# mdangschat/ctc-asr

Measured on AMD Instinct MI355X. Metric: audio-seconds/s training throughput (DS2, 10 s utterances), higher is better.
Workload: dtype f32 tensors / accumulate / own kernels; projection GEMMs: fp16x3 split (22 significand bits) where the layer input is bounded or, behind a ReLU cell, scaled per row / per column on the device - forward projections and their gradient GEMMs - bf16x6 split (24 bits) elsewhere; forward and backward recu

## Files before the change

ctc_asr_amd/csrc/conv16.hip:

```cpp
#include "common.h"

namespace {

constexpr int C16_CIN = 32, C16_KT = 11, C16_KF = 21;
constexpr int C16_CELL = 144;

typedef unsigned int u32x4 __attribute__((ext_vector_type(4)));
typedef unsigned int u32x2 __attribute__((ext_vector_type(2)));
typedef _Float16 f16x8 __attribute__((ext_vector_type(8)));
union Frag16 {
    u32x4 u;
    f16x8 h;
};

__device__ __forceinline__ unsigned f16_pieces(float s) {
    const _Float16 h1 = (_Float16)s;
    const _Float16 h2 = (_Float16)(s - (float)h1);
    return (unsigned)__builtin_bit_cast(unsigned short, h1) |
           ((unsigned)__builtin_bit_cast(unsigned short, h2) << 16);
}

__device__ __forceinline__ float scale_below_f16_max(unsigned max_bits) {
    const int e = (int)((max_bits >> 23) & 0xFF) - 127;
    const int se = max_bits == 0u ? 0 : min(max(14 - e, -60), 60);
// ... 547 lines not shown
    if (tile < tiles) fetch(tile);
    while (tile < tiles) {
        __syncthreads();
        stage();
        __syncthreads();
        const int next = next_valid(tile + nsplit);
        if (next < tiles) fetch(next);
#pragma unroll 1
        for (int q = 0; q < G::KS; ++q) {
            const int slot = 4 * q + g;
            Frag16 a1[2], a2[2];
#pragma unroll
            for (int c = 0; c < 2; ++c) {
                a1[c].u = dzs[(slot * 2 + 0) * 32 + c * 16 + n];
                a2[c].u = dzs[(slot * 2 + 1) * 32 + c * 16 + n];
            }
            const u32x4 *xb = xs + ((2 * slot + kf0) * 2) * 32 + ci_tile * 16 + n;
#pragma unroll
            for (int k = 0; k < TAPS; ++k) {
                if (k < TAPS - 1 || !half) {
                    Frag16 b1, b2;
                    b1.u = xb[k * 64];
                    b2.u = xb[k * 64 + 32];
#pragma unroll
                    for (int c = 0; c < 2; ++c) {
                        acc[k][c] = __builtin_amdgcn_mfma_f32_16x16x32_f16(a1[c].h, b1.h, acc[k][c], 0, 0, 0);
                        acc[k][c] = __builtin_amdgcn_mfma_f32_16x16x32_f16(a1[c].h, b2.h, acc[k][c], 0, 0, 0);
                        acc[k][c] = __builtin_amdgcn_mfma_f32_16x16x32_f16(a2[c].h, b1.h, acc[k][c], 0, 0, 0);
                    }
                }
            }
        }
        tile = next;
    }
    float *out = partial + (((size_t)split * gridDim.z + cg) * C16_KT + kt) * C16_KF * 1024;
#pragma unroll
    for (int k = 0; k < TAPS; ++k) {
        if (k < TAPS - 1 || !half) {
#pragma unroll
            for (int c = 0; c < 2; ++c)
#pragma unroll
                for (int r = 0; r < 4; ++r)
                    out[(size_t)(kf0 + k) * 1024 + (c * 16 + 4 * g + r) * C16_CIN + ci_tile * 16 +
                        n] = acc[k][c][r];
        }
    }
}

__global__ void wrw16_reduce_kernel(const float *__restrict__ partial,
                                    const unsigned *__restrict__ max_bits, float inv_x_scale,
                                    float *__restrict__ dw, int nsplit, int cout) {
    const int j = blockIdx.x * blockDim.x + threadIdx.x;
    const int total = cout * C16_CIN * C16_KT * C16_KF;
    if (j >= total) return;
    const int ci = j & 31, co32 = (j >> 5) & 31, tap = (j >> 10) % (C16_KT * C16_KF);
    const int co = (j >> 10) / (C16_KT * C16_KF) * 32 + co32;
    float sum = 0.f;
#pragma unroll 4
    for (int sp = 0; sp < nsplit; ++sp) sum += partial[(size_t)sp * total + j];
    dw[((size_t)co * C16_CIN + ci) * (C16_KT * C16_KF) + tap] =
        sum * (inv_x_scale / scale_below_f16_max(max_bits[co]));
}

int wrw16_splits(int B, int T, int cout) {
    const int tiles = ((B + 7) / 8) * T;
    const int want = 512 / (C16_KT * (cout / 32));
    return tiles < want ? tiles : want;
}

struct Wrw16Workspace {
    size_t max_bits, x16, dz16, partial, total;
};
Wrw16Workspace wrw16_workspace(int B, int T, int freq_in, int cout) {
    const size_t nblk = (size_t)(B + 7) / 8;
    Wrw16Workspace w;
    w.max_bits = 0;
    w.x16 = 512;
    w.dz16 = w.x16 + nblk * T * freq_in * 1024;
    w.partial = w.dz16 + nblk * T * (freq_in / 2) * 2 * cout * 16;
    w.total = w.partial + (size_t)wrw16_splits(B, T, cout) * cout * C16_CIN * C16_KT * C16_KF * 4;
    return w;
}

bool covered16(int freq_in, int cout) {
    return (freq_in == 40 && cout == 32) || (freq_in == 20 && cout == 96);
}

}

static size_t pack16_order_bytes(int cout) {
    return (size_t)C16_KT * C16_KF * C16_CIN * cout * 4;
}
extern "C" size_t ctcasr_conv_s12_pack16_bytes(int cout) {
    if (cout != 32 && cout != 96) return 0;
    return 16 + 2 * pack16_order_bytes(cout);
}

extern "C" int ctcasr_conv_s12_pack_weights16(const float *w, void *packed, int cout,
                                              ctcasr_stream_t stream) {
    if (!w || !packed || (cout != 32 && cout != 96)) return CTCASR_ERR_BAD_ARGUMENT;
    hipStream_t s = (hipStream_t)stream;
    unsigned *max_bits = reinterpret_cast<unsigned *>(packed);
    if (hipMemsetAsync(max_bits, 0, 16, s) != hipSuccess) return CTCASR_ERR_LAUNCH;
    const int n = cout * C16_CIN * C16_KT * C16_KF;
    conv16_absmax_kernel<<<64, 256, 0, s>>>(w, n, max_bits);
    const int threads = C16_KT * C16_KF * (cout / 16) * 64;
    conv16_pack_fwd_kernel<<<(threads + 255) / 256, 256, 0, s>>>(
        w, max_bits, reinterpret_cast<u32x4 *>(reinterpret_cast<char *>(packed) + 16), cout);
    const int threads_b = C16_KT * C16_KF * (cout / 32) * 2 * 64;
    conv16_pack_bwd_kernel<<<(threads_b + 255) / 256, 256, 0, s>>>(
        w, max_bits,
        reinterpret_cast<u32x4 *>(reinterpret_cast<char *>(packed) + 16 + pack16_order_bytes(cout)),
        cout);
    return ctcasr_launch_status();
}

extern "C" int ctcasr_conv_s12_bwd_data16(const float *dz, const void *packed, float *dx, int B,
                                          int T, int freq_in, int cout, int dz_time_major,
                                          const float *act, float relu_cutoff,
                                          ctcasr_stream_t stream) {
    if (!dz || !packed || !dx || B <= 0 || T <= 0 || (act && relu_cutoff <= 0.f))
        return CTCASR_ERR_BAD_ARGUMENT;
    if (!covered16(freq_in, cout) || B > 65535) return CTCASR_ERR_UNSUPPORTED;
    hipStream_t s = (hipStream_t)stream;
    const unsigned *max_bits = reinterpret_cast<const unsigned *>(packed);
    const void *pieces = reinterpret_cast<const char *>(packed) + 16 + pack16_order_bytes(cout);
    if (cout == 32)
        return launch_bwd16<32, 40>(dz, pieces, max_bits, dx, B, T, dz_time_major, act,
                                    relu_cutoff, s);
    return launch_bwd16<96, 20>(dz, pieces, max_bits, dx, B, T, dz_time_major, act, relu_cutoff, s);
}

extern "C" int ctcasr_conv_s12_fwd16(const float *x, float x_scale, const void *packed,
                                     const float *bias, float *y, int B, int T, int freq_in,
                                     int cout, float relu_cutoff, int y_time_major,
                                     ctcasr_stream_t stream) {
    if (!x || !packed || !y || B <= 0 || T <= 0 || !(x_scale > 0.f)) return CTCASR_ERR_BAD_ARGUMENT;
    if (!covered16(freq_in, cout) || B > 65535) return CTCASR_ERR_UNSUPPORTED;
    hipStream_t s = (hipStream_t)stream;
    const unsigned *max_bits = reinterpret_cast<const unsigned *>(packed);
    const void *pieces = reinterpret_cast<const char *>(packed) + 16;
    if (cout == 32)
        return launch_fwd16<32, 40>(x, x_scale, pieces, max_bits, bias, y, B, T, relu_cutoff,
                                    y_time_major, s);
    return launch_fwd16<96, 20>(x, x_scale, pieces, max_bits, bias, y, B, T, relu_cutoff,
                                y_time_major, s);
}

extern "C" size_t ctcasr_conv_s12_wrw16_workspace_bytes(int B, int T, int freq_in, int cout) {
    if (B <= 0 || T <= 0 || !covered16(freq_in, cout)) return 0;
    return wrw16_workspace(B, T, freq_in, cout).total;
}

extern "C" int ctcasr_conv_s12_wrw16(const float *dz, const float *x, float x_scale, float *dw,
                                     int B, int T, int freq_in, int cout, int dz_time_major,
                                     const float *act, float relu_cutoff, float *dbias,
                                     void *workspace, size_t workspace_bytes,
                                     ctcasr_stream_t stream) {
    if (!dz || !x || !dw || B <= 0 || T <= 0 || (act && relu_cutoff <= 0.f) || !(x_scale > 0.f))
        return CTCASR_ERR_BAD_ARGUMENT;
    if (!covered16(freq_in, cout)) return CTCASR_ERR_UNSUPPORTED;
    const Wrw16Workspace w = wrw16_workspace(B, T, freq_in, cout);
    if (!workspace || workspace_bytes < w.total) return CTCASR_ERR_WORKSPACE;
    hipStream_t s = (hipStream_t)stream;
    char *base = reinterpret_cast<char *>(workspace);
    unsigned *max_bits = reinterpret_cast<unsigned *>(base + w.max_bits);
    u32x4 *x16 = reinterpret_cast<u32x4 *>(base + w.x16);
    u32x4 *dz16 = reinterpret_cast<u32x4 *>(base + w.dz16);
    float *partial = reinterpret_cast<float *>(base + w.partial);
    const int fo = freq_in / 2, nblk = (B + 7) / 8;
    if (hipMemsetAsync(max_bits, 0, 512, s) != hipSuccess) return CTCASR_ERR_LAUNCH;
    const long cells4 = (long)B * T * fo * cout / 4;
    wrw16_colmax_kernel<<<240, 256, 0, s>>>(dz, act, relu_cutoff, cells4, cout, max_bits, dbias);
    const long per_utt = (long)T * freq_in * C16_CIN, xcells = (long)nblk * per_utt;
    wrw16_pack_x_kernel<<<(unsigned)((xcells + 255) / 256), 256, 0, s>>>(x, x_scale, x16, B,
                                                                        per_utt, xcells);
    const long dcells = (long)nblk * T * fo * cout;
    wrw16_pack_dz_kernel<<<(unsigned)((dcells + 255) / 256), 256, 0, s>>>(
        dz, act, relu_cutoff, max_bits, dz16, B, T, fo * cout, cout, dz_time_major, dcells);
    const int nsplit = wrw16_splits(B, T, cout);
    dim3 grid(nsplit, C16_KT, cout / 32);
    if (freq_in == 40) {
        if (hipFuncSetAttribute(reinterpret_cast<const void *>(&wrw16_kernel<40>),
                                hipFuncAttributeMaxDynamicSharedMemorySize,
                                (int)Wrw16Geometry<40>::LDS) != hipSuccess)
            return CTCASR_ERR_LAUNCH;
        wrw16_kernel<40><<<grid, 256, Wrw16Geometry<40>::LDS, s>>>(x16, dz16, partial, nblk, T, cout);
    } else {
        if (hipFuncSetAttribute(reinterpret_cast<const void *>(&wrw16_kernel<20>),
                                hipFuncAttributeMaxDynamicSharedMemorySize,
                                (int)Wrw16Geometry<20>::LDS) != hipSuccess)
            return CTCASR_ERR_LAUNCH;
        wrw16_kernel<20><<<grid, 256, Wrw16Geometry<20>::LDS, s>>>(x16, dz16, partial, nblk, T, cout);
    }
    const int total = cout * C16_CIN * C16_KT * C16_KF;
    wrw16_reduce_kernel<<<(total + 255) / 256, 256, 0, s>>>(partial, max_bits, 1.0f / x_scale, dw,
                                                            nsplit, cout);
    return ctcasr_launch_status();
}

namespace {

constexpr int Z0_KT = 11, Z0_KF = 41, Z0_FI = 80, Z0_FO = 40, Z0_TT = 16;
constexpr int Z0_PW = 128;
constexpr int Z0_PT = 2 * Z0_TT + Z0_KT - 2;
constexpr int Z0_GROUPS = Z0_KT * 6;
constexpr int Z0_QS = (Z0_GROUPS + 3) / 4;
constexpr int Z0_W_CELLS = Z0_QS * 2 * 2 * 64;
constexpr int Z0_DW = 32 * Z0_KT * Z0_KF;
constexpr size_t Z0_FWD_LDS = (size_t)2 * 2 * Z0_PT * Z0_PW * 2 + (size_t)Z0_W_CELLS * 16 + 16;
constexpr size_t Z0_WRW_LDS = ((size_t)Z0_KT * 2 * Z0_PW + (size_t)Z0_FO * 2 * 32) * 16;
constexpr int Z0_WRW_GRID = 256;

__global__ void __launch_bounds__(256)
conv0_pack_w16_kernel(const float *__restrict__ w, const unsigned *__restrict__ max_bits,
                      u32x4 *__restrict__ packed) {
    const int i = blockIdx.x * blockDim.x + threadIdx.x;
    if (i >= Z0_QS * 2 * 64) return;
    const int lane = i & 63, nt = (i >> 6) & 1, q = i >> 7;
    const int n = lane & 15, g = lane >> 4, gi = 4 * q + g, kt = gi / 6, kb = gi % 6;
    const float s_w = scale_below_f16_max(*max_bits);
    unsigned p[8];
#pragma unroll
    for (int e = 0; e < 8; ++e) {
        const int kf = 8 * kb + e;
        p[e] = (gi < Z0_GROUPS && kf < Z0_KF)
                   ? f16_pieces(w[((16 * nt + n) * Z0_KT + kt) * Z0_KF + kf] * s_w) : 0u;
    }
    store_pieces8(packed + ((size_t)(q * 2 + nt) * 2) * 64 + lane, 64, p);
}

__global__ void __launch_bounds__(256)
conv0_fwd16_kernel(const float *__restrict__ x, const u32x4 *__restrict__ packed,
                   const unsigned *__restrict__ w_max_bits, const float *__restrict__ bias,
                   float *__restrict__ y, int T, int t_out, int pt0, float cutoff) {
    extern __shared__ __attribute__((aligned(16))) unsigned char zsm[];
    _Float16 *copies = reinterpret_cast<_Float16 *>(zsm);
    u32x4 *wl = reinterpret_cast<u32x4 *>(zsm + (size_t)2 * 2 * Z0_PT * Z0_PW * 2);
    unsigned *pmax = reinterpret_cast<unsigned *>(wl + Z0_W_CELLS);
    const int tid = threadIdx.x, lane = tid & 63, wave = tid >> 6;
    const int t0 = blockIdx.x * Z0_TT, b = blockIdx.y;
    const int g = lane >> 4, n = lane & 15;
    constexpr int PLANE = Z0_PT * Z0_PW;

    if (tid == 0) *pmax = 0u;
    __syncthreads();
    constexpr int PER = (PLANE + 255) / 256;
    float v[PER];
    float m = 0.f;
#pragma unroll
    for (int j = 0; j < PER; ++j) {
        const int i = tid + j * 256, col = i % Z0_PW, pr = i / Z0_PW;
        const int ts = 2 * t0 - pt0 + pr, fi = col - 19;
        v[j] = (i < PLANE && ts >= 0 && ts < T && fi >= 0 && fi < Z0_FI)
                   ? x[((size_t)b * T + ts) * Z0_FI + fi] : 0.f;
        m = fmaxf(m, fabsf(v[j]));
    }
    m = wave_max(m);
    if (lane == 0) atomicMax(pmax, __float_as_uint(m));
    for (int i = tid; i < Z0_W_CELLS; i += 256) wl[i] = packed[i];
    __syncthreads();
    const float s_x = scale_below_f16_max(*pmax);
    for (int i = tid; i < 2 * Z0_PT; i += 256) {
        _Float16 *tail = copies + (size_t)(2 + i / Z0_PT) * PLANE + (i % Z0_PT) * Z0_PW + Z0_PW - 2;
        tail[0] = (_Float16)0.f;
        tail[1] = (_Float16)0.f;
    }
#pragma unroll
    for (int j = 0; j < PER; ++j) {
        const int i = tid + j * 256, col = i % Z0_PW;
        if (i < PLANE) {
            const unsigned p = f16_pieces(v[j] * s_x);
            const _Float16 h1 = __builtin_bit_cast(_Float16, (unsigned short)(p & 0xFFFFu));
            const _Float16 h2 = __builtin_bit_cast(_Float16, (unsigned short)(p >> 16));
            copies[i] = h1;
            copies[PLANE + i] = h2;
            if (col >= 2) {
                copies[2 * PLANE + i - 2] = h1;
                copies[3 * PLANE + i - 2] = h2;
            }
        }
    }
    __syncthreads();

    int base_a[10];
#pragma unroll
    for (int ti = 0; ti < 10; ++ti) {
        const int rho = ti / 5, mrow = (ti % 5) * 16 + n, tt = mrow / 20, i = mrow % 20;
        base_a[ti] = rho * 2 * PLANE + 2 * (4 * wave + tt) * Z0_PW + 4 * i;
    }
    f32x4 acc[10][2];
#pragma unroll
    for (int ti = 0; ti < 10; ++ti) {
        acc[ti][0] = (f32x4){0.f, 0.f, 0.f, 0.f};
        acc[ti][1] = (f32x4){0.f, 0.f, 0.f, 0.f};
    }
#pragma unroll 1
    for (int q = 0; q < Z0_QS; ++q) {
        const int gi = 4 * q + g, kt = gi / 6, kb = gi - 6 * kt;
        const int off = gi < Z0_GROUPS ? kt * Z0_PW + 8 * kb : 0;
        const unsigned keep0 = kb == 5 ? 0x0000FFFFu : 0xFFFFFFFFu, keep = kb == 5 ? 0u : 0xFFFFFFFFu;
        Frag16 b1[2], b2[2];
#pragma unroll
        for (int nt = 0; nt < 2; ++nt) {
            b1[nt].u = wl[((q * 2 + nt) * 2 + 0) * 64 + lane];
            b2[nt].u = wl[((q * 2 + nt) * 2 + 1) * 64 + lane];
        }
#pragma unroll
        for (int ti = 0; ti < 10; ++ti) {
            const u32x2 *p1 = reinterpret_cast<const u32x2 *>(copies + base_a[ti] + off);
            const u32x2 *p2 = reinterpret_cast<const u32x2 *>(copies + base_a[ti] + off + PLANE);
            const u32x2 lo1 = p1[0], hi1 = p1[1], lo2 = p2[0], hi2 = p2[1];
            Frag16 a1, a2;
            a1.u = (u32x4){lo1.x & keep0, lo1.y & keep, hi1.x & keep, hi1.y & keep};
            a2.u = (u32x4){lo2.x & keep0, lo2.y & keep, hi2.x & keep, hi2.y & keep};
#pragma unroll
            for (int nt = 0; nt < 2; ++nt) {
                acc[ti][nt] = __builtin_amdgcn_mfma_f32_16x16x32_f16(a1.h, b1[nt].h, acc[ti][nt], 0, 0, 0);
                acc[ti][nt] = __builtin_amdgcn_mfma_f32_16x16x32_f16(a1.h, b2[nt].h, acc[ti][nt], 0, 0, 0);
                acc[ti][nt] = __builtin_amdgcn_mfma_f32_16x16x32_f16(a2.h, b1[nt].h, acc[ti][nt], 0, 0, 0);
            }
        }
    }

    const float inv = 1.0f / (s_x * scale_below_f16_max(*w_max_bits));
    const float bias0 = bias ? bias[n] : 0.f, bias1 = bias ? bias[16 + n] : 0.f;
#pragma unroll
    for (int ti = 0; ti < 10; ++ti)
#pragma unroll
        for (int r = 0; r < 4; ++r) {
            const int rho = ti / 5, mrow = (ti % 5) * 16 + 4 * g + r, tt = mrow / 20;
            const int fo = 2 * (mrow % 20) + rho, t = t0 + 4 * wave + tt;
            if (t < t_out) {
                float *out = y + ((size_t)(b * t_out + t) * Z0_FO + fo) * 32 + n;
                float v0 = acc[ti][0][r] * inv + bias0, v1 = acc[ti][1][r] * inv + bias1;
                if (cutoff > 0.f) {
                    v0 = relu_clip(v0, cutoff);
                    v1 = relu_clip(v1, cutoff);
                }
                out[0] = v0;
                out[16] = v1;
            }
        }
}

__global__ void __launch_bounds__(256)
conv0_pack_x_kernel(const float *__restrict__ x, const unsigned *__restrict__ max_bits,
                    u32x4 *__restrict__ x16, int B, long per_utt , long cells) {
    const long i = (long)blockIdx.x * 256 + threadIdx.x;
    if (i >= cells) return;
    const long within = i % per_utt;
    const int b0 = (int)(i / per_utt) * 8;
    const float s = scale_below_f16_max(*max_bits);
// ... 42 lines not shown
        const u32x4 *dsrc = dz16 + ((size_t)bblk * t_out + t) * Z0_FO * 64;
#pragma unroll
        for (int j = 0; j < DZ_PER; ++j) rdz[j] = dsrc[tid + j * 256];
    };
    auto stage = [&]() {
#pragma unroll
        for (int j = 0; j < X_PER; ++j) {
            const int i = tid + j * 256, kt = i / (2 * Z0_FI), rest = i % (2 * Z0_FI);
            if (i < X_CELLS)
                xl[(kt * 2 + rest / Z0_FI) * Z0_PW + 19 + rest % Z0_FI] = rx[j];
        }
#pragma unroll
        for (int j = 0; j < DZ_PER; ++j) dzs[tid + j * 256] = rdz[j];
    };

    int tile = blockIdx.x;
    if (tile < tiles) fetch(tile);
    while (tile < tiles) {
        __syncthreads();
        stage();
        __syncthreads();
        const int next = tile + gridDim.x;
        if (next < tiles) fetch(next);
#pragma unroll 1
        for (int q = 0; q < Z0_FO / 4; ++q) {
            const int slot = 4 * q + g;
            Frag16 a1[2], a2[2];
#pragma unroll
            for (int mt = 0; mt < 2; ++mt) {
                a1[mt].u = dzs[(slot * 2 + 0) * 32 + mt * 16 + n];
                a2[mt].u = dzs[(slot * 2 + 1) * 32 + mt * 16 + n];
            }
#pragma unroll
            for (int k = 0; k < 3; ++k) {
                const int kt = wave + 4 * k;
                if (kt < Z0_KT) {
                    const u32x4 *xb = xl + (kt * 2) * Z0_PW + 2 * slot + n;
#pragma unroll
                    for (int nt = 0; nt < 3; ++nt) {
                        Frag16 b1, b2;
                        b1.u = xb[16 * nt];
                        b2.u = xb[16 * nt + Z0_PW];
#pragma unroll
                        for (int mt = 0; mt < 2; ++mt) {
                            acc[k][nt][mt] = __builtin_amdgcn_mfma_f32_16x16x32_f16(
                                a1[mt].h, b1.h, acc[k][nt][mt], 0, 0, 0);
                            acc[k][nt][mt] = __builtin_amdgcn_mfma_f32_16x16x32_f16(
                                a1[mt].h, b2.h, acc[k][nt][mt], 0, 0, 0);
                            acc[k][nt][mt] = __builtin_amdgcn_mfma_f32_16x16x32_f16(
                                a2[mt].h, b1.h, acc[k][nt][mt], 0, 0, 0);
                        }
                    }
                }
            }
        }
        tile = next;
    }
    float *out = partial + (size_t)blockIdx.x * Z0_DW;
#pragma unroll
    for (int k = 0; k < 3; ++k) {
        const int kt = wave + 4 * k;
        if (kt < Z0_KT) {
#pragma unroll
            for (int nt = 0; nt < 3; ++nt) {
                const int kf = 16 * nt + n;
                if (kf < Z0_KF) {
#pragma unroll
                    for (int mt = 0; mt < 2; ++mt)
#pragma unroll
                        for (int r = 0; r < 4; ++r)
                            out[((16 * mt + 4 * g + r) * Z0_KT + kt) * Z0_KF + kf] =
                                acc[k][nt][mt][r];
                }
            }
        }
    }
}

__global__ void __launch_bounds__(256)
conv0_wrw16_reduce_kernel(const float *__restrict__ partial, const unsigned *__restrict__ ch_bits,
                          const unsigned *__restrict__ x_bits, float *__restrict__ dw, int parts) {
    __shared__ float band_sum[4][64];
    const int e = threadIdx.x & 63, band = threadIdx.x >> 6, i = blockIdx.x * 64 + e;
    float sum = 0.f;
    if (i < Z0_DW) {
#pragma unroll 8
        for (int part = band; part < parts; part += 4) sum += partial[(size_t)part * Z0_DW + i];
    }
    band_sum[band][e] = sum;
    __syncthreads();
    if (band == 0 && i < Z0_DW)
        dw[i] = (band_sum[0][e] + band_sum[1][e] + (band_sum[2][e] + band_sum[3][e])) /
                (scale_below_f16_max(ch_bits[i / (Z0_KT * Z0_KF)]) * scale_below_f16_max(*x_bits));
}

struct Z0Workspace {
    size_t x16, dz16, partial, total;
    int parts;
};
Z0Workspace z0_workspace(int B, int T) {
    const size_t nblk = (size_t)(B + 7) / 8, t_out = (size_t)(T + 1) / 2;
    Z0Workspace w;
    w.x16 = 512;
    w.dz16 = w.x16 + nblk * T * 2 * Z0_FI * 16;
    w.partial = w.dz16 + nblk * t_out * Z0_FO * 64 * 16;
    const size_t tiles = nblk * t_out;
    w.parts = (int)(tiles < (size_t)Z0_WRW_GRID ? tiles : (size_t)Z0_WRW_GRID);
    w.total = w.partial + (size_t)w.parts * Z0_DW * 4;
    return w;
}

int conv0_pt0(int T) {
    const int t_out = (T + 1) / 2;
    const int total = (t_out - 1) * 2 + Z0_KT - T;
    return total > 0 ? total / 2 : 0;
}

}

extern "C" size_t ctcasr_conv0_pack16_bytes(void) { return 16 + (size_t)Z0_W_CELLS * 16; }

extern "C" int ctcasr_conv0_pack_weights16(const float *w, void *packed16, ctcasr_stream_t stream) {
    if (!w || !packed16) return CTCASR_ERR_BAD_ARGUMENT;
    hipStream_t s = (hipStream_t)stream;
    unsigned *max_bits = reinterpret_cast<unsigned *>(packed16);
    if (hipMemsetAsync(max_bits, 0, 16, s) != hipSuccess) return CTCASR_ERR_LAUNCH;
    conv16_absmax_kernel<<<8, 256, 0, s>>>(w, Z0_DW, max_bits);
    conv0_pack_w16_kernel<<<(Z0_QS * 2 * 64 + 255) / 256, 256, 0, s>>>(
        w, max_bits, reinterpret_cast<u32x4 *>(reinterpret_cast<char *>(packed16) + 16));
    return ctcasr_launch_status();
}

extern "C" int ctcasr_conv0_fwd16(const float *x, const void *packed16, const float *bias, float *y,
                                  int B, int T, float relu_cutoff, ctcasr_stream_t stream) {
    if (!x || !packed16 || !y || B <= 0 || T <= 0) return CTCASR_ERR_BAD_ARGUMENT;
    if (B > 65535) return CTCASR_ERR_UNSUPPORTED;
    const int t_out = (T + 1) / 2;
    if (hipFuncSetAttribute(reinterpret_cast<const void *>(&conv0_fwd16_kernel),
                            hipFuncAttributeMaxDynamicSharedMemorySize,
                            (int)Z0_FWD_LDS) != hipSuccess)
        return CTCASR_ERR_LAUNCH;
    dim3 grid((t_out + Z0_TT - 1) / Z0_TT, B);
    conv0_fwd16_kernel<<<grid, 256, Z0_FWD_LDS, (hipStream_t)stream>>>(
        x, reinterpret_cast<const u32x4 *>(reinterpret_cast<const char *>(packed16) + 16),
        reinterpret_cast<const unsigned *>(packed16), bias, y, T, t_out, conv0_pt0(T), relu_cutoff);
    return ctcasr_launch_status();
}

extern "C" size_t ctcasr_conv0_wrw16_workspace_bytes(int B, int T) {
    if (B <= 0 || T <= 0) return 0;
    return z0_workspace(B, T).total;
}

extern "C" int ctcasr_conv0_wrw16(const float *dz, const float *x, float *dw, int B, int T,
                                  const float *act, float relu_cutoff, float *dbias,
                                  void *workspace, size_t workspace_bytes,
                                  ctcasr_stream_t stream) {
    if (!dz || !x || !dw || B <= 0 || T <= 0 || (act && relu_cutoff <= 0.f))
        return CTCASR_ERR_BAD_ARGUMENT;
    const Z0Workspace w = z0_workspace(B, T);
    if (!workspace || workspace_bytes < w.total) return CTCASR_ERR_WORKSPACE;
    hipStream_t s = (hipStream_t)stream;
    char *base = reinterpret_cast<char *>(workspace);
    unsigned *ch_bits = reinterpret_cast<unsigned *>(base);
    unsigned *x_bits = reinterpret_cast<unsigned *>(base + 256);
    u32x4 *x16 = reinterpret_cast<u32x4 *>(base + w.x16);
    u32x4 *dz16 = reinterpret_cast<u32x4 *>(base + w.dz16);
    float *partial = reinterpret_cast<float *>(base + w.partial);
    const int t_out = (T + 1) / 2, nblk = (B + 7) / 8;
    if (hipMemsetAsync(base, 0, 512, s) != hipSuccess) return CTCASR_ERR_LAUNCH;
    const long cells4 = (long)B * t_out * Z0_FO * 32 / 4;
    wrw16_colmax_kernel<<<240, 256, 0, s>>>(dz, act, relu_cutoff, cells4, 32, ch_bits, dbias);
    const long n_x = (long)B * T * Z0_FI;
    conv16_absmax_kernel<<<512, 256, 0, s>>>(x, (int)n_x, x_bits);
    const long per_utt = (long)T * Z0_FI, xcells = (long)nblk * per_utt;
    conv0_pack_x_kernel<<<(unsigned)((xcells + 255) / 256), 256, 0, s>>>(x, x_bits, x16, B, per_utt,
                                                                        xcells);
    const long dcells = (long)nblk * t_out * Z0_FO * 32;
    wrw16_pack_dz_kernel<<<(unsigned)((dcells + 255) / 256), 256, 0, s>>>(
        dz, act, relu_cutoff, ch_bits, dz16, B, t_out, Z0_FO * 32, 32, 0, dcells);
    if (hipFuncSetAttribute(reinterpret_cast<const void *>(&conv0_wrw16_kernel),
                            hipFuncAttributeMaxDynamicSharedMemorySize,
                            (int)Z0_WRW_LDS) != hipSuccess)
        return CTCASR_ERR_LAUNCH;
    conv0_wrw16_kernel<<<w.parts, 256, Z0_WRW_LDS, s>>>(x16, dz16, partial, nblk, T, t_out,
                                                        conv0_pt0(T));
    conv0_wrw16_reduce_kernel<<<(Z0_DW + 63) / 64, 256, 0, s>>>(partial, ch_bits, x_bits, dw,
                                                                  w.parts);
    return ctcasr_launch_status();
}
```

ctc_asr_amd/csrc/elementwise.hip:

```cpp
#include "common.h"

namespace {

__device__ __forceinline__ float uniform01(uint64_t seed, uint64_t idx) {
    return (float)splitmix64_r24(seed, idx) * (1.0f / 16777216.0f);
}

__global__ void __launch_bounds__(256)
bias_act_fwd_kernel(float *__restrict__ y, const float *__restrict__ bias, int64_t n, int cols,
                    float cutoff, float rate, float inv_keep, uint64_t seed) {
    const int64_t stride = (int64_t)gridDim.x * blockDim.x;
    for (int64_t i = (int64_t)blockIdx.x * blockDim.x + threadIdx.x; i < n; i += stride) {
        float v = y[i];
        if (bias) v += bias[i % cols];
        if (cutoff > 0.f) {
            v = relu_clip(v, cutoff);
            if (rate > 0.f) v = uniform01(seed, (uint64_t)i) >= rate ? v * inv_keep : 0.f;
        }
        y[i] = v;
    }
}

__global__ void __launch_bounds__(256)
bias_act_fwd_kernel_v4(float4 *__restrict__ y, const float4 *__restrict__ bias, int64_t n4,
                       int cols4, float cutoff, float rate, float inv_keep, uint64_t seed) {
    const int64_t stride = (int64_t)gridDim.x * blockDim.x;
    for (int64_t i = (int64_t)blockIdx.x * blockDim.x + threadIdx.x; i < n4; i += stride) {
        float4 v = y[i];
        if (bias) {
            float4 bb = bias[i % cols4];
            v.x += bb.x; v.y += bb.y; v.z += bb.z; v.w += bb.w;
        }
        if (cutoff > 0.f) {
            v.x = relu_clip(v.x, cutoff); v.y = relu_clip(v.y, cutoff);
            v.z = relu_clip(v.z, cutoff); v.w = relu_clip(v.w, cutoff);
            if (rate > 0.f) {
                const uint64_t e = (uint64_t)i * 4;
                v.x = uniform01(seed, e + 0) >= rate ? v.x * inv_keep : 0.f;
                v.y = uniform01(seed, e + 1) >= rate ? v.y * inv_keep : 0.f;
                v.z = uniform01(seed, e + 2) >= rate ? v.z * inv_keep : 0.f;
                v.w = uniform01(seed, e + 3) >= rate ? v.w * inv_keep : 0.f;
            }
        }
        y[i] = v;
    }
}

__global__ void __launch_bounds__(256)
dropout_kernel(const float *__restrict__ in, float *__restrict__ out, int64_t n, float rate,
               float inv_keep, uint64_t seed) {
    const int64_t stride = (int64_t)gridDim.x * blockDim.x;
    for (int64_t i = (int64_t)blockIdx.x * blockDim.x + threadIdx.x; i < n; i += stride)
        out[i] = uniform01(seed, (uint64_t)i) >= rate ? in[i] * inv_keep : 0.f;
}

__global__ void __launch_bounds__(256)
bias_act_bwd_kernel(const float *__restrict__ y, const float *__restrict__ dy,
                    float *__restrict__ dz, float *__restrict__ dbias, int64_t rows, int cols,
                    float upper, float inv_keep, int64_t rows_per_block) {
    __shared__ float part[4][64];
    const int lane = threadIdx.x & 63, wave = threadIdx.x >> 6;
    const bool narrow = cols < 64 && 64 % cols == 0;
    const int rpw = narrow ? 64 / cols : 1;
    const int c = narrow ? lane % cols : blockIdx.x * 64 + lane;
    const int64_t r0 = (int64_t)blockIdx.y * rows_per_block;
    const int64_t r1 = r0 + rows_per_block < rows ? r0 + rows_per_block : rows;
    float sum = 0.f;
    if (c < cols) {
        for (int64_t r = r0 + wave * rpw + (narrow ? lane / cols : 0); r < r1; r += 4 * rpw) {
            const int64_t i = r * cols + c;
            float g = dy[i];
            if (y) {
                const float v = y[i];
                g = (v > 0.f && v < upper) ? g * inv_keep : 0.f;
            }
            if (dz) dz[i] = g;
            sum += g;
        }
    }
    if (!dbias) return;
    part[wave][lane] = sum;
    __syncthreads();
    if (wave == 0 && lane < (narrow ? cols : 64) && c < cols) {
        float total = 0.f;
        for (int j = lane; j < 64; j += narrow ? cols : 64)
            total += part[0][j] + part[1][j] + part[2][j] + part[3][j];
        atomicAdd(&dbias[c], total);
    }
}

__global__ void __launch_bounds__(256)
transpose_kernel(const float *__restrict__ in, float *__restrict__ out, int rows, int cols) {
    __shared__ float tile[32][33];
    const size_t base = (size_t)blockIdx.z * rows * cols;
    const int tx = threadIdx.x & 31, ty = threadIdx.x >> 5;
    const int c0 = blockIdx.x * 32, r0 = blockIdx.y * 32;
    for (int j = ty; j < 32; j += 8) {
        int r = r0 + j, c = c0 + tx;
        if (r < rows && c < cols) tile[j][tx] = in[base + (size_t)r * cols + c];
    }
    __syncthreads();
    for (int j = ty; j < 32; j += 8) {
        int c = c0 + j, r = r0 + tx;
        if (r < rows && c < cols) out[base + (size_t)c * rows + r] = tile[tx][j];
    }
}

#define ADAM_LANE(f)                                                      \
        {                                                                 \
            float gr = gg.f * gscale;                                     \
            mm.f = b1 * mm.f + (1.f - b1) * gr;                           \
            vv.f = b2 * vv.f + (1.f - b2) * gr * gr;                      \
            pp.f -= lr_t * mm.f / (sqrtf(vv.f) + eps);                    \
        }

__global__ void __launch_bounds__(256)
adam_kernel(float *__restrict__ p, const float *__restrict__ g, float *__restrict__ m,
            float *__restrict__ v, int64_t n, float lr_t, float b1, float b2, float eps,
            float gscale, const int32_t *__restrict__ skip,
            const float *__restrict__ gfactor) {
    if (skip && *skip) return;
    if (gfactor) gscale *= *gfactor;
    const int64_t stride = (int64_t)gridDim.x * blockDim.x;
    const int64_t n4 = n >> 2;
    float4 *p4 = reinterpret_cast<float4 *>(p);
    const float4 *g4 = reinterpret_cast<const float4 *>(g);
    float4 *m4 = reinterpret_cast<float4 *>(m);
    float4 *v4 = reinterpret_cast<float4 *>(v);
    for (int64_t i = (int64_t)blockIdx.x * blockDim.x + threadIdx.x; i < n4; i += stride) {
        float4 pp = p4[i], gg = g4[i], mm = m4[i], vv = v4[i];
        ADAM_LANE(x) ADAM_LANE(y) ADAM_LANE(z) ADAM_LANE(w)
        p4[i] = pp; m4[i] = mm; v4[i] = vv;
    }
    for (int64_t i = (n4 << 2) + (int64_t)blockIdx.x * blockDim.x + threadIdx.x; i < n;
         i += stride) {
        float gr = g[i] * gscale;
        float mm = b1 * m[i] + (1.f - b1) * gr;
        float vv = b2 * v[i] + (1.f - b2) * gr * gr;
        m[i] = mm; v[i] = vv;
        p[i] -= lr_t * mm / (sqrtf(vv) + eps);
    }
}

__global__ void __launch_bounds__(256)
adam_ema_kernel(float *__restrict__ p, const float *__restrict__ g, float *__restrict__ m,
                float *__restrict__ v, float *__restrict__ e, int64_t n, float lr_t, float b1,
                float b2, float eps, float gscale, const int32_t *__restrict__ skip,
                const float *__restrict__ gfactor, float alpha) {
    if (skip && *skip) return;
    if (gfactor) gscale *= *gfactor;
    const int64_t stride = (int64_t)gridDim.x * blockDim.x;
    const int64_t n4 = n >> 2;
    float4 *p4 = reinterpret_cast<float4 *>(p);
    const float4 *g4 = reinterpret_cast<const float4 *>(g);
    float4 *m4 = reinterpret_cast<float4 *>(m);
    float4 *v4 = reinterpret_cast<float4 *>(v);
    float4 *e4 = reinterpret_cast<float4 *>(e);
#define EMA_LANE(f) ee.f = ee.f + alpha * (pp.f - ee.f);
    for (int64_t i = (int64_t)blockIdx.x * blockDim.x + threadIdx.x; i < n4; i += stride) {
        float4 pp = p4[i], gg = g4[i], mm = m4[i], vv = v4[i], ee = e4[i];
        ADAM_LANE(x) ADAM_LANE(y) ADAM_LANE(z) ADAM_LANE(w)
        EMA_LANE(x) EMA_LANE(y) EMA_LANE(z) EMA_LANE(w)
        p4[i] = pp; m4[i] = mm; v4[i] = vv; e4[i] = ee;
    }
    struct One { float x; };
    for (int64_t i = (n4 << 2) + (int64_t)blockIdx.x * blockDim.x + threadIdx.x; i < n;
         i += stride) {
        One pp{p[i]}, gg{g[i]}, mm{m[i]}, vv{v[i]}, ee{e[i]};
        ADAM_LANE(x)
        EMA_LANE(x)
        m[i] = mm.x; v[i] = vv.x; p[i] = pp.x; e[i] = ee.x;
    }
#undef EMA_LANE
}
#undef ADAM_LANE

__global__ void step_guard_kernel(const int32_t *__restrict__ status,
                                  const float *__restrict__ loss, int batch,
                                  const unsigned *err0, const unsigned *err1,
                                  const int32_t *wgrad, int32_t *__restrict__ skip) {
    int bad = 0;
    for (int b = threadIdx.x; b < batch; b += blockDim.x) {
        if (status && status[b] != 0) bad = 1;
        if (loss && !isfinite(loss[b])) bad = 1;
    }
    bad = __any(bad) ? 1 : 0;
    __shared__ int any_bad[4];
    if ((threadIdx.x & 63) == 0) any_bad[threadIdx.x >> 6] = bad;
    __syncthreads();
    if (threadIdx.x == 0) {
        const unsigned err = (err0 ? *err0 : 0u) | (err1 ? *err1 : 0u) |
                             (wgrad && *wgrad != 0 ? 1u << 30 : 0u);
        skip[0] = (any_bad[0] | any_bad[1] | any_bad[2] | any_bad[3] | (err != 0u)) ? 1 : 0;
        skip[1] = (int32_t)err;
    }
}

__global__ void __launch_bounds__(256)
absmax_kernel(const float *__restrict__ x, int64_t n, unsigned *__restrict__ out) {
    const int64_t stride = (int64_t)gridDim.x * blockDim.x;
    float m = 0.f;
    const float4 *x4 = reinterpret_cast<const float4 *>(x);
    for (int64_t i = (int64_t)blockIdx.x * blockDim.x + threadIdx.x; i < (n >> 2); i += stride) {
        const float4 v = x4[i];
        m = fmaxf(fmaxf(m, fmaxf(fabsf(v.x), fabsf(v.y))), fmaxf(fabsf(v.z), fabsf(v.w)));
    }
    for (int64_t i = ((n >> 2) << 2) + (int64_t)blockIdx.x * blockDim.x + threadIdx.x; i < n;
         i += stride)
        m = fmaxf(m, fabsf(x[i]));
    m = wave_max(m);
    __shared__ float wmax[4];
    if ((threadIdx.x & 63) == 0) wmax[threadIdx.x >> 6] = m;
    __syncthreads();
    if (threadIdx.x == 0)
        atomicMax(out, __float_as_uint(fmaxf(fmaxf(wmax[0], wmax[1]), fmaxf(wmax[2], wmax[3]))));
}

__global__ void __launch_bounds__(256) occupy_kernel(unsigned long long busy_ticks) {
    const unsigned long long start = wall_clock64();
    while (wall_clock64() - start < busy_ticks) __builtin_amdgcn_s_sleep(32);
}

__global__ void __launch_bounds__(256) collective_traffic_kernel(float4 *a, const float4 *b,
                                                                 long long n4, long long total4,
                                                                 unsigned long long busy_ticks) {
    const unsigned long long start = wall_clock64();
    const long long share = total4 / gridDim.x;
    const long long first = (long long)blockIdx.x * share;
    constexpr long long SLAB = 256 * 16;
    for (long long base = 0; base < share; base += SLAB) {
#pragma unroll 4
        for (long long i = base + threadIdx.x; i < min(base + SLAB, share); i += 256) {
            const long long idx = (first + i) % n4;
            const float4 x = a[idx], y = b[idx];
            a[idx] = make_float4(x.x + y.x, x.y + y.y, x.z + y.z, x.w + y.w);
        }
        const unsigned long long due = (unsigned long long)(
            (double)busy_ticks * (double)(base + SLAB) / (double)share);
        while (wall_clock64() - start < due) __builtin_amdgcn_s_sleep(8);
    }
    while (wall_clock64() - start < busy_ticks) __builtin_amdgcn_s_sleep(32);
}

int grid_for(int64_t work_items) {
    int64_t blocks = (work_items + 255) / 256;
    if (blocks > 2048) blocks = 2048;
    if (blocks < 1) blocks = 1;
    return (int)blocks;
}

}

extern "C" int ctcasr_bias_act_fwd(float *y, const float *bias, int64_t rows, int cols,
                                   float cutoff, float dropout_rate, uint64_t seed,
                                   ctcasr_stream_t stream) {
    if (!y || rows < 0 || cols <= 0 || dropout_rate < 0.f || dropout_rate >= 1.f)
        return CTCASR_ERR_BAD_ARGUMENT;
    if (rows == 0) return CTCASR_OK;
    const int64_t n = rows * cols;
    const float inv_keep = 1.f / (1.f - dropout_rate);
    hipStream_t s = (hipStream_t)stream;
    const bool aligned = (reinterpret_cast<uintptr_t>(y) % 16 == 0) &&
                         (!bias || reinterpret_cast<uintptr_t>(bias) % 16 == 0);
    if (cols % 4 == 0 && aligned) {
        bias_act_fwd_kernel_v4<<<grid_for(n / 4), 256, 0, s>>>(
            reinterpret_cast<float4 *>(y), reinterpret_cast<const float4 *>(bias), n / 4,
            cols / 4, cutoff, dropout_rate, inv_keep, seed);
    } else {
        bias_act_fwd_kernel<<<grid_for(n), 256, 0, s>>>(y, bias, n, cols, cutoff, dropout_rate,
                                                        inv_keep, seed);
    }
    return ctcasr_launch_status();
}

static int launch_bwd(const float *y, const float *dy, float *dz, float *dbias, int64_t rows,
                      int cols, float upper, float inv_keep, hipStream_t s) {
    const int col_blocks = (cols + 63) / 64;
    int64_t row_blocks = (2048 + col_blocks - 1) / col_blocks;
    if (row_blocks > (rows + 15) / 16) row_blocks = (rows + 15) / 16;
    if (row_blocks < 1) row_blocks = 1;
    if (row_blocks > 65535) row_blocks = 65535;
    const int64_t rows_per_block = (rows + row_blocks - 1) / row_blocks;
    dim3 grid(col_blocks, (unsigned)((rows + rows_per_block - 1) / rows_per_block));
    bias_act_bwd_kernel<<<grid, 256, 0, s>>>(y, dy, dz, dbias, rows, cols, upper, inv_keep,
                                            rows_per_block);
    return ctcasr_launch_status();
}

extern "C" int ctcasr_bias_act_bwd(const float *y, const float *dy, float *dz, float *dbias,
                                   int64_t rows, int cols, float cutoff, float dropout_rate,
                                   ctcasr_stream_t stream) {
    if (!y || !dy || !dz || rows < 0 || cols <= 0 || cutoff <= 0.f || dropout_rate < 0.f ||
        dropout_rate >= 1.f)
        return CTCASR_ERR_BAD_ARGUMENT;
    if (rows == 0) return CTCASR_OK;
    const float inv_keep = 1.f / (1.f - dropout_rate);
    return launch_bwd(y, dy, dz, dbias, rows, cols, cutoff * inv_keep, inv_keep,
                      (hipStream_t)stream);
}

extern "C" int ctcasr_colsum_accumulate(const float *dz, float *dbias, int64_t rows, int cols,
                                        ctcasr_stream_t stream) {
    if (!dz || !dbias || rows < 0 || cols <= 0) return CTCASR_ERR_BAD_ARGUMENT;
    if (rows == 0) return CTCASR_OK;
    return launch_bwd(nullptr, dz, nullptr, dbias, rows, cols, 0.f, 1.f, (hipStream_t)stream);
}

extern "C" int ctcasr_dropout(const float *in, float *out, int64_t n, float dropout_rate,
                              uint64_t seed, ctcasr_stream_t stream) {
    if (!in || !out || n < 0 || dropout_rate < 0.f || dropout_rate >= 1.f)
        return CTCASR_ERR_BAD_ARGUMENT;
    if (n == 0) return CTCASR_OK;
    dropout_kernel<<<grid_for(n), 256, 0, (hipStream_t)stream>>>(
        in, out, n, dropout_rate, 1.f / (1.f - dropout_rate), seed);
    return ctcasr_launch_status();
}

extern "C" int ctcasr_transpose_batched(const float *in, float *out, int batch, int rows, int cols,
                                        ctcasr_stream_t stream) {
    if (!in || !out || batch <= 0 || rows <= 0 || cols <= 0) return CTCASR_ERR_BAD_ARGUMENT;
    dim3 grid((cols + 31) / 32, (rows + 31) / 32, batch);
    transpose_kernel<<<grid, 256, 0, (hipStream_t)stream>>>(in, out, rows, cols);
    return ctcasr_launch_status();
}

extern "C" int ctcasr_adam_step_clipped(float *param, const float *grad, float *m, float *v,
                                        int64_t n, float lr, float beta1, float beta2,
                                        float epsilon, int64_t step, float grad_scale,
                                        const int32_t *skip, const float *grad_factor,
                                        ctcasr_stream_t stream) {
    if (!param || !grad || !m || !v || n < 0 || step < 1) return CTCASR_ERR_BAD_ARGUMENT;
    if (n == 0) return CTCASR_OK;
    if ((reinterpret_cast<uintptr_t>(param) | reinterpret_cast<uintptr_t>(grad) |
         reinterpret_cast<uintptr_t>(m) | reinterpret_cast<uintptr_t>(v)) % 16 != 0)
        return CTCASR_ERR_BAD_ARGUMENT;
    const double lr_t = (double)lr * sqrt(1.0 - pow((double)beta2, (double)step)) /
                        (1.0 - pow((double)beta1, (double)step));
#ifndef ADAM_BLOCKS
#define ADAM_BLOCKS 65536
#endif
    int64_t want = (n / 4 + 1 + 255) / 256;
    const int blocks = (int)(want > ADAM_BLOCKS ? ADAM_BLOCKS : want < 1 ? 1 : want);
    adam_kernel<<<blocks, 256, 0, (hipStream_t)stream>>>(
        param, grad, m, v, n, (float)lr_t, beta1, beta2, epsilon, grad_scale, skip, grad_factor);
    return ctcasr_launch_status();
}

extern "C" int ctcasr_adam_step_ema(float *param, const float *grad, float *m, float *v,
                                    float *ema, int64_t n, float lr, float beta1, float beta2,
                                    float epsilon, int64_t step, float grad_scale,
                                    const int32_t *skip, const float *grad_factor,
                                    float ema_alpha, ctcasr_stream_t stream) {
    if (!param || !grad || !m || !v || !ema || n < 0 || step < 1) return CTCASR_ERR_BAD_ARGUMENT;
    if (!(ema_alpha >= 0.f && ema_alpha <= 1.f)) return CTCASR_ERR_BAD_ARGUMENT;
    if (n == 0) return CTCASR_OK;
    if ((reinterpret_cast<uintptr_t>(param) | reinterpret_cast<uintptr_t>(grad) |
         reinterpret_cast<uintptr_t>(m) | reinterpret_cast<uintptr_t>(v) |
         reinterpret_cast<uintptr_t>(ema)) % 16 != 0)
        return CTCASR_ERR_BAD_ARGUMENT;
    const double lr_t = (double)lr * sqrt(1.0 - pow((double)beta2, (double)step)) /
                        (1.0 - pow((double)beta1, (double)step));
    int64_t want = (n / 4 + 1 + 255) / 256;
    const int blocks = (int)(want > ADAM_BLOCKS ? ADAM_BLOCKS : want < 1 ? 1 : want);
    adam_ema_kernel<<<blocks, 256, 0, (hipStream_t)stream>>>(
        param, grad, m, v, ema, n, (float)lr_t, beta1, beta2, epsilon, grad_scale, skip,
        grad_factor, ema_alpha);
    return ctcasr_launch_status();
}

extern "C" int ctcasr_adam_step(float *param, const float *grad, float *m, float *v, int64_t n,
                                float lr, float beta1, float beta2, float epsilon, int64_t step,
                                float grad_scale, const int32_t *skip, ctcasr_stream_t stream) {
    return ctcasr_adam_step_clipped(param, grad, m, v, n, lr, beta1, beta2, epsilon, step,
                                    grad_scale, skip, nullptr, stream);
}

extern "C" int ctcasr_step_guard(const int32_t *ctc_status, const float *per_utterance_loss,
                                 int batch, const uint32_t *timeout_word0,
                                 const uint32_t *timeout_word1, const int32_t *wgrad_word,
                                 int32_t *skip, ctcasr_stream_t stream) {
    if (!skip || batch < 0) return CTCASR_ERR_BAD_ARGUMENT;
    step_guard_kernel<<<1, 256, 0, (hipStream_t)stream>>>(ctc_status, per_utterance_loss, batch,
                                                          timeout_word0, timeout_word1, wgrad_word,
                                                          skip);
    return ctcasr_launch_status();
}

extern "C" int ctcasr_occupy_cus(int workgroups, int busy_us, ctcasr_stream_t stream) {
    if (workgroups < 1 || workgroups > 256 || busy_us < 0 || busy_us > 100000)
        return CTCASR_ERR_BAD_ARGUMENT;
    occupy_kernel<<<workgroups, 256, 0, (hipStream_t)stream>>>((unsigned long long)busy_us * 100ull);
    return ctcasr_launch_status();
}

extern "C" int ctcasr_collective_traffic(int workgroups, int busy_us, float *a, const float *b,
                                         int64_t scratch_floats, int64_t payload_bytes,
                                         ctcasr_stream_t stream) {
    if (workgroups < 1 || workgroups > 256 || busy_us < 0 || busy_us > 100000 || !a || !b ||
        scratch_floats < 1024 || scratch_floats % 4 != 0 || payload_bytes < 0 ||
        (reinterpret_cast<uintptr_t>(a) | reinterpret_cast<uintptr_t>(b)) % 16 != 0)
        return CTCASR_ERR_BAD_ARGUMENT;
    const long long total4 = 2 * (payload_bytes / 16);
    collective_traffic_kernel<<<workgroups, 256, 0, (hipStream_t)stream>>>(
        reinterpret_cast<float4 *>(a), reinterpret_cast<const float4 *>(b), scratch_floats / 4,
        total4, (unsigned long long)busy_us * 100ull);
    return ctcasr_launch_status();
}

extern "C" int ctcasr_absmax(const float *x, int64_t n, uint32_t *max_bits,
                             ctcasr_stream_t stream) {
    if (!x || !max_bits || n < 0 || reinterpret_cast<uintptr_t>(x) % 16 != 0)
        return CTCASR_ERR_BAD_ARGUMENT;
    if (n == 0) return CTCASR_OK;
    const int blocks = grid_for(n / 4 + 1);
    absmax_kernel<<<blocks < 1024 ? blocks : 1024, 256, 0, (hipStream_t)stream>>>(x, n, max_bits);
    return ctcasr_launch_status();
}
```

ctc_asr_amd/hip.py:

```python

import ctypes
import functools
import os

import torch

_PKG_DIR = os.path.dirname(os.path.abspath(__file__))
LIB_PATH = os.path.join(_PKG_DIR, 'libctcasr.so')

ABI_VERSION = 8
BUILD_PROBE_WRONG_RESULTS, BUILD_NONDEFAULT_TUNING = 1, 2
RNN_DEFAULT, RNN_HALF_CHIP, RNN_WHOLE_CHIP, RNN_ONE_BARRIER = 0, 1, 2, 4
RNN_F16 = 16
RNN_XCD_SPLIT = 32
RNN_STAGGER = 64
RNN_KPAIR = 128
RESIDENT_GATE_MAX_US = 100000
GRAD_NORM_CHUNK = 8192
GRAD_NORM_MAX_SEGMENTS = 64
SPEC_AUGMENT_MAX_MASKS = 16
NOISE_MIX_CHUNK = 8192
NOISE_MIX_SNR_DB = (-20, 60)
REVERB_CHUNK = 2048
REVERB_TAP_BLOCK = 32
REVERB_TAP_ALIGN = 8
REVERB_MAX_TAPS = 8192
VAD_HOP = 160
VAD_LEVELS = 160
VAD_CHUNK = 40960
RESAMPLE_MAX_TABLE = 16640
RESAMPLE_RATES = (4000, 192000)
RESAMPLE_MAX_CHANNELS = 8
SEQ_BN_ROWS = 64
ALIGN_LONG_TILE_STATES = 1024
ALIGN_LONG_TILE_FRAMES = 256
ALIGN_LONG_MAX = (1 << 22, 1 << 20, 64)
SEARCH_MAX_LABEL_LEN = 576
SEARCH_MAX_HITS = 1024
SEARCH_WAVES = 4
CELL_IDS = {'rnn_relu': 0, 'rnn_tanh': 1, 'lstm': 2, 'gru': 3}
CELL_GATES = {'rnn_relu': 1, 'rnn_tanh': 1, 'lstm': 4, 'gru': 3}

_c_int, _c_i64, _c_u64 = ctypes.c_int, ctypes.c_int64, ctypes.c_uint64
_c_f, _c_p, _c_sz = ctypes.c_float, ctypes.c_void_p, ctypes.c_size_t
_c_d = ctypes.c_double

SIGNATURES = {
    'ctcasr_abi_version': (_c_int, []),
    'ctcasr_build_flags': (ctypes.c_uint, []),
    'ctcasr_error_string': (ctypes.c_char_p, [_c_int]),
    'ctcasr_set_option': (_c_int, [ctypes.c_char_p, _c_int]),
    'ctcasr_rnn_kernel_events': (_c_int, [_c_p, _c_p]),
    'ctcasr_log_softmax_fwd': (_c_int, [_c_p, _c_p, _c_int, _c_int, _c_p]),
    'ctcasr_log_softmax_bwd': (_c_int, [_c_p, _c_p, _c_p, _c_int, _c_int, _c_p]),
    'ctcasr_ctc_loss_workspace_bytes': (_c_sz, [_c_int] * 4),
    'ctcasr_ctc_loss_fwd_bwd': (_c_int, [_c_p] * 4 + [_c_int] * 5 + [_c_f] + [_c_p] * 4 +
                                [_c_sz, _c_p]),
    'ctcasr_ctc_greedy_decode': (_c_int, [_c_p, _c_p] + [_c_int] * 4 + [_c_p, _c_p, _c_p]),
    'ctcasr_ctc_beam_workspace_bytes': (_c_sz, [_c_int] * 4),
    'ctcasr_ctc_beam_decode': (_c_int, [_c_p, _c_p] + [_c_int] * 6 + [_c_p] * 4 + [_c_sz, _c_p]),
    'ctcasr_ctc_beam_lm_workspace_bytes': (_c_sz, [_c_int] * 4),
    'ctcasr_ctc_beam_decode_lm': (_c_int, [_c_p, _c_p] + [_c_int] * 6 + [_c_p] * 3 + [_c_int] +
                                  [_c_p] * 4 + [_c_sz, _c_p]),
    'ctcasr_ctc_beam_nbest_workspace_bytes': (_c_sz, [_c_int] * 4),
    'ctcasr_ctc_beam_decode_nbest': (_c_int, [_c_p, _c_p] + [_c_int] * 7 + [_c_p] * 3 + [_c_int] +
                                     [_c_p] * 5 + [_c_sz, _c_p]),
    'ctcasr_ctc_score_workspace_bytes': (_c_sz, [_c_int] * 5),
    'ctcasr_ctc_score': (_c_int, [_c_p, _c_p] + [_c_int] * 4 + [_c_p] * 3 + [_c_int] * 2 +
                         [_c_p] * 3 + [_c_sz, _c_p]),
    'ctcasr_ctc_mwer_workspace_bytes': (_c_sz, [_c_int] * 5),
    'ctcasr_ctc_mwer': (_c_int, [_c_p, _c_p] + [_c_int] * 4 + [_c_p] * 4 + [_c_int, _c_int, _c_f,
                                                                              _c_int] +
                        [_c_p] * 6 + [_c_sz, _c_p]),
    'ctcasr_ctc_align_workspace_bytes': (_c_sz, [_c_int] * 4),
    'ctcasr_ctc_align': (_c_int, [_c_p] * 4 + [_c_int] * 5 + [_c_p] * 5 + [_c_sz, _c_p]),
    'ctcasr_ctc_align_long_workspace_bytes': (_c_sz, [_c_i64, _c_int, _c_i64, _c_int]),
    'ctcasr_ctc_align_long': (_c_int, [_c_p, _c_p, _c_i64, _c_int, _c_int, _c_i64, _c_int] +
                              [_c_p] * 6 + [_c_sz, _c_p]),
    'ctcasr_ctc_search_workspace_bytes': (_c_sz, [_c_int] * 3),
    'ctcasr_ctc_search': (_c_int, [_c_p, _c_p] + [_c_int] * 4 + [_c_p, _c_p, _c_int, _c_int] +
                          [_c_p] * 3 + [_c_int, _c_int] + [_c_p] * 9 + [_c_sz, _c_p]),
    'ctcasr_edit_distance_workspace_bytes': (_c_sz, [_c_int] * 3),
    'ctcasr_edit_distance': (_c_int, [_c_p] * 6 + [_c_int] * 3 + [_c_p] * 6 + [_c_sz, _c_p]),
    'ctcasr_rnn_reserve_bytes': (_c_sz, [_c_int] * 4),
    'ctcasr_rnn_workspace_bytes': (_c_sz, [_c_int] * 4),
    'ctcasr_rnn_persistent_supported': (_c_int, [_c_int] * 4),
    'ctcasr_rnn_poll_error': (_c_int, [_c_p, _c_sz] + [_c_int] * 4 + [_c_p]),
    'ctcasr_rnn_resident_gate': (_c_int, [_c_p, _c_sz] + [_c_int] * 4 + [ctypes.c_uint, _c_int,
                                                                          _c_p]),
    'ctcasr_rnn_gru_drec_offset': (_c_sz, [_c_int] * 3),
    'ctcasr_rnn_fwd': (_c_int, [_c_int] + [_c_p] * 5 + [_c_int] * 3 + [_c_p] * 3 + [_c_sz, _c_p]),
    'ctcasr_rnn_bwd': (_c_int, [_c_int] + [_c_p] * 5 + [_c_int] * 3 + [_c_p] * 4 + [_c_sz, _c_p]),
    'ctcasr_rnn_fwd_steps': (_c_int, [_c_int] + [_c_p] * 5 + [_c_int] * 3 + [_c_p] * 4 +
                             [_c_sz, _c_int, _c_int, _c_int, _c_p]),
    'ctcasr_rnn_fwd_f16_supported': (_c_int, [_c_int] * 5),
    'ctcasr_rnn_bwd_steps': (_c_int, [_c_int] + [_c_p] * 5 + [_c_int] * 3 + [_c_p] * 5 +
                             [_c_sz, _c_int, _c_int, _c_int, _c_p]),
    'ctcasr_rnn_bwd_f16_supported': (_c_int, [_c_int] * 5),
    'ctcasr_bias_act_fwd': (_c_int, [_c_p, _c_p, _c_i64, _c_int, _c_f, _c_f, _c_u64, _c_p]),
    'ctcasr_bias_act_bwd': (_c_int, [_c_p] * 4 + [_c_i64, _c_int, _c_f, _c_f, _c_p]),
    'ctcasr_dropout': (_c_int, [_c_p, _c_p, _c_i64, _c_f, _c_u64, _c_p]),
    'ctcasr_colsum_accumulate': (_c_int, [_c_p, _c_p, _c_i64, _c_int, _c_p]),
    'ctcasr_conv_s12_supported': (_c_int, [_c_int, _c_int]),
    'ctcasr_conv_s12_pack_weights': (_c_int, [_c_p, _c_p, _c_int, _c_p]),
    'ctcasr_conv_s12_fwd': (_c_int, [_c_p, _c_p, _c_p, _c_p] + [_c_int] * 4 + [_c_f, _c_int, _c_p]),
    'ctcasr_conv_s12_pack16_bytes': (_c_sz, [_c_int]),
    'ctcasr_conv_s12_pack_weights16': (_c_int, [_c_p, _c_p, _c_int, _c_p]),
    'ctcasr_conv_s12_fwd16': (_c_int, [_c_p, _c_f, _c_p, _c_p, _c_p] + [_c_int] * 4 +
                              [_c_f, _c_int, _c_p]),
    'ctcasr_conv_s12_bwd_data16': (_c_int, [_c_p, _c_p, _c_p] + [_c_int] * 5 + [_c_p, _c_f, _c_p]),
    'ctcasr_conv0_pack16_bytes': (_c_sz, []),
    'ctcasr_conv0_pack_weights16': (_c_int, [_c_p, _c_p, _c_p]),
    'ctcasr_conv0_fwd16': (_c_int, [_c_p] * 4 + [_c_int, _c_int, _c_f, _c_p]),
    'ctcasr_conv0_wrw16_workspace_bytes': (_c_sz, [_c_int, _c_int]),
    'ctcasr_conv0_wrw16': (_c_int, [_c_p] * 3 + [_c_int, _c_int, _c_p, _c_f, _c_p, _c_p, _c_sz,
                                                 _c_p]),
    'ctcasr_conv_s12_wrw16_workspace_bytes': (_c_sz, [_c_int] * 4),
    'ctcasr_conv_s12_wrw16': (_c_int, [_c_p, _c_p, _c_f, _c_p] + [_c_int] * 5 +
                              [_c_p, _c_f, _c_p, _c_p, _c_sz, _c_p]),
    'ctcasr_conv_s12_bwd_data': (_c_int, [_c_p, _c_p, _c_p] + [_c_int] * 5 + [_c_p, _c_f, _c_p]),
    'ctcasr_conv_s12_wrw_workspace_bytes': (_c_sz, [_c_int] * 4),
    'ctcasr_conv_s12_wrw': (_c_int, [_c_p] * 3 + [_c_int] * 5 + [_c_p, _c_f, _c_p] +
                            [_c_p, _c_sz, _c_p]),
    'ctcasr_conv0_fwd': (_c_int, [_c_p, _c_p, _c_p, _c_p, _c_int, _c_int, _c_f, _c_p]),
    'ctcasr_conv0_wrw_workspace_bytes': (_c_sz, [_c_int, _c_int]),
    'ctcasr_conv0_wrw': (_c_int, [_c_p, _c_p, _c_p, _c_int, _c_int, _c_p, _c_f, _c_p, _c_p, _c_sz,
                                  _c_p]),
    'ctcasr_transpose_batched': (_c_int, [_c_p, _c_p, _c_int, _c_int, _c_int, _c_p]),
    'ctcasr_split_bf16': (_c_int, [_c_p, _c_i64, _c_int, _c_i64, _c_p, _c_int, _c_p, _c_i64, _c_i64,
                                   _c_p]),
    'ctcasr_split_f16': (_c_int, [_c_p, _c_i64, _c_int, _c_i64, _c_f, _c_p, _c_int, _c_p, _c_i64,
                                  _c_i64, _c_p]),
    'ctcasr_colmax_scale': (_c_int, [_c_p, _c_i64, _c_int, _c_i64, _c_p, _c_p, _c_p, _c_p]),
    'ctcasr_colscale_from_max': (_c_int, [_c_p, _c_int, _c_p, _c_p, _c_p]),
    'ctcasr_split_f16_cols': (_c_int, [_c_p, _c_i64, _c_int, _c_i64, _c_p, _c_f, _c_p, _c_int, _c_p,
                                       _c_i64, _c_i64, _c_p]),
    'ctcasr_split_f16_rows': (_c_int, [_c_p, _c_i64, _c_int, _c_i64, _c_p, _c_int, _c_p, _c_i64,
                                       _c_i64, _c_p, _c_p]),
    'ctcasr_rescale_rows': (_c_int, [_c_p, _c_i64, _c_p, _c_f, _c_p, _c_i64, _c_i64, _c_int, _c_int,
                                     _c_p]),
    'ctcasr_gemm_split_nt': (_c_int, [_c_p, _c_i64, _c_p, _c_i64, _c_p, _c_i64, _c_int, _c_int, _c_int,
                                      _c_int, _c_p]),
    'ctcasr_gemm_split_tn': (_c_int, [_c_p, _c_i64, _c_p, _c_i64, _c_p, _c_i64, _c_int, _c_int, _c_int,
                                      _c_int, _c_p]),
    'ctcasr_rnn_f16_recurrence': (_c_int, [_c_int] * 7),
    'ctcasr_collective_traffic': (_c_int, [_c_int, _c_int, _c_p, _c_p, _c_i64, _c_i64, _c_p]),
    'ctcasr_wgrad16_packed_bytes': (_c_sz, [_c_int, _c_int]),
    'ctcasr_wgrad16_pack': (_c_int, [_c_p, _c_i64, _c_i64, _c_int, _c_i64, _c_int, _c_p, _c_f, _c_p,
                                     _c_p]),
    'ctcasr_wgrad16_gemm': (_c_int, [_c_p, _c_int, _c_int, _c_p, _c_p, _c_int, _c_int, _c_f, _c_p,
                                     _c_i64, _c_p, _c_int, _c_int, _c_f, _c_p, _c_i64, _c_int, _c_p,
                                     _c_p]),
    'ctcasr_wgrad16_sync_ints': (_c_sz, [_c_int, _c_int, _c_int]),
    'ctcasr_dgrad16_packed_bytes': (_c_sz, [_c_int]),
    'ctcasr_dgrad16_pack_weights': (_c_int, [_c_p, _c_i64, _c_int, _c_int, _c_f, _c_p, _c_p]),
    'ctcasr_dgrad16_supported': (_c_int, [_c_int] * 4),
    'ctcasr_dgrad16_published_offsets': (_c_int, [_c_int, _c_int, _c_int, _c_p, _c_p]),
    'ctcasr_dgrad16_blockscaled': (_c_int, [_c_p, _c_int, _c_int, _c_int, _c_p, _c_f, _c_int, _c_p,
                                            _c_i64] + [_c_int] * 5 + [_c_p]),
    'ctcasr_features_num_frames': (_c_int, [_c_int]),
    'ctcasr_features_tables_bytes': (_c_sz, []),
    'ctcasr_features_init_tables': (_c_int, [_c_p, _c_int, _c_p]),
    'ctcasr_features_workspace_bytes': (_c_sz, [_c_int, _c_int]),
    'ctcasr_features': (_c_int, [_c_p, _c_p] + [_c_int] * 5 + [_c_p, _c_p, _c_int, _c_p, _c_p,
                                 _c_sz, _c_p]),
    'ctcasr_spec_augment': (_c_int, [_c_p, _c_p, _c_int, _c_int, _c_u64] + [_c_int] * 5 +
                            [_c_p, _c_p]),
    'ctcasr_resample_num_samples': (_c_int, [_c_int, _c_int]),
    'ctcasr_speed_perturb': (_c_int, [_c_p, _c_p, _c_p, _c_int, _c_int, _c_p, _c_int, _c_p, _c_p]),
    'ctcasr_noise_mix_workspace_bytes': (_c_sz, [_c_int]),
    'ctcasr_noise_mix': (_c_int, [_c_p, _c_p, _c_int, _c_int, _c_p, _c_p, _c_int, _c_u64] +
                         [_c_int] * 3 + [_c_p] * 5 + [_c_sz, _c_p]),
    'ctcasr_reverb': (_c_int, [_c_p, _c_p, _c_int, _c_int] + [_c_p] * 4 + [_c_int, _c_u64, _c_int] +
                      [_c_p] * 3),
    'ctcasr_vad_energy': (_c_int, [_c_p, _c_i64, _c_p, _c_p, _c_p]),
    'ctcasr_gather_segments': (_c_int, [_c_p, _c_i64, _c_p, _c_p, _c_int, _c_int] + [_c_p] * 3),
    'ctcasr_resample_plan': (_c_int, [_c_int, _c_int] + [_c_p] * 4),
    'ctcasr_resample_chunk': (_c_int, [_c_int, _c_int]),
    'ctcasr_resample_out_samples': (_c_i64, [_c_i64, _c_int, _c_int]),
    'ctcasr_resample_table_bytes': (_c_sz, [_c_int, _c_int]),
    'ctcasr_resample_table': (_c_int, [_c_int, _c_int, _c_p, _c_p]),
    'ctcasr_resample': (_c_int, [_c_p, _c_int, _c_int, _c_i64, _c_int, _c_int, _c_p, _c_p, _c_i64,
                                 _c_p, _c_p]),
    'ctcasr_adam_step': (_c_int, [_c_p] * 4 + [_c_i64] + [_c_f] * 4 + [_c_i64, _c_f, _c_p, _c_p]),
    'ctcasr_adam_step_clipped': (_c_int, [_c_p] * 4 + [_c_i64] + [_c_f] * 4 +
                                 [_c_i64, _c_f, _c_p, _c_p, _c_p]),
    'ctcasr_adam_step_ema': (_c_int, [_c_p] * 5 + [_c_i64] + [_c_f] * 4 +
                             [_c_i64, _c_f, _c_p, _c_p, _c_f, _c_p]),
    'ctcasr_grad_norm_workspace_bytes': (_c_sz, [_c_i64, _c_int]),
    'ctcasr_grad_norm': (_c_int, [_c_p, _c_i64, _c_p, _c_int, _c_f, _c_f] + [_c_p] * 4 +
                         [_c_sz, _c_p]),
    'ctcasr_seq_bn_workspace_bytes': (_c_sz, [_c_i64, _c_int]),
    'ctcasr_seq_bn_fwd': (_c_int, [_c_p, _c_p, _c_int, _c_int, _c_int] + [_c_p] * 4 +
                          [_c_d, _c_d] + [_c_p] * 4 + [_c_sz, _c_p]),
    'ctcasr_seq_bn_infer': (_c_int, [_c_p, _c_p, _c_int, _c_int, _c_int] + [_c_p] * 4 +
                            [_c_d, _c_p, _c_p]),
    'ctcasr_seq_bn_bwd': (_c_int, [_c_p, _c_p, _c_p, _c_int, _c_int, _c_int] + [_c_p] * 7 +
                          [_c_sz, _c_p]),
    'ctcasr_step_guard': (_c_int, [_c_p, _c_p, _c_int, _c_p, _c_p, _c_p, _c_p, _c_p]),
    'ctcasr_rnn_timeout_word_offset': (_c_sz, [_c_int] * 5),
    'ctcasr_absmax': (_c_int, [_c_p, _c_i64, _c_p, _c_p]),
    'ctcasr_occupy_cus': (_c_int, [_c_int, _c_int, _c_p]),
}

_lib = None

EVENTS = None
TIMED = ('rnn_fwd', 'rnn_bwd', 'ctc_loss_fwd_bwd', 'dgrad16')


class _Timed:
    def __init__(self, name):
        self.name = name

    def __enter__(self):
        if EVENTS is not None and self.name in TIMED:
            self.start = torch.cuda.Event(enable_timing=True)
            self.stop = torch.cuda.Event(enable_timing=True)
            self.start.record()
        return self

    def __exit__(self, *exc):
        if EVENTS is not None and self.name in TIMED:
            self.stop.record()
            EVENTS.setdefault(self.name, []).append((self.start, self.stop))
        return False


def drain_events():
    global EVENTS
    out = {}
    for name, pairs in (EVENTS or {}).items():
        out[name] = (len(pairs), sum(a.elapsed_time(b) for a, b in pairs))
    if EVENTS is not None:
        EVENTS = {}
    return out


class CtcAsrError(RuntimeError):
    """Non-zero status from the C ABI."""


def load(path=None):
    global _lib
    if _lib is not None and path is None:
        return _lib
    path = path or os.environ.get('CTCASR_LIB') or LIB_PATH
    if not os.path.exists(path):
        raise CtcAsrError('{} is missing - build it with `python -m ctc_asr_amd.build`; the '
                          'MI355X path has no CPU fallback.'.format(path))
    lib = ctypes.CDLL(path)
    for name, (restype, argtypes) in SIGNATURES.items():
        fn = getattr(lib, name)
        fn.restype, fn.argtypes = restype, argtypes
    if lib.ctcasr_abi_version() != ABI_VERSION:
        raise CtcAsrError('libctcasr ABI version mismatch')
    if lib.ctcasr_build_flags() & BUILD_PROBE_WRONG_RESULTS and \
            os.environ.get('CTCASR_ALLOW_PROBE_BUILD') != '1':
        raise CtcAsrError('{} is a timing-probe build (ctcasr_build_flags() = {:#x}: results are '
                          'wrong on purpose); set CTCASR_ALLOW_PROBE_BUILD=1 to load it anyway.'
                          .format(path, lib.ctcasr_build_flags()))
    _lib = lib
    return lib


def _check(code, what):
    if code != 0:
        raise CtcAsrError('{} failed: {} ({})'.format(
            what, load().ctcasr_error_string(code).decode(), code))


def _dev(tensor, dtype=torch.float32, name='tensor'):
# ... 1028 lines not shown
        raise CtcAsrError('{}: x_scale must be a positive finite number (got {}).'
                          .format(what, x_scale))
    return x_scale


def _conv_mask(what, dz, act, relu_cutoff, dbias, cout):
    if act is not None:
        if tuple(act.shape) != tuple(dz.shape):
            raise CtcAsrError('{}: act must be shaped like dz {} (got {}).'
                              .format(what, tuple(dz.shape), tuple(act.shape)))
        if not float(relu_cutoff) > 0.0:
            raise CtcAsrError('{}: act needs relu_cutoff > 0 (got {}).'.format(what, relu_cutoff))
    _expect_numel(what, 'dbias', dbias, cout)


@_on_tensor_device
def conv_s12_pack_weights(weight, packed=None):
    cout = weight.shape[0] if weight.dim() == 4 else 0
    if tuple(weight.shape[1:]) != (32, 11, 21) or cout not in (32, 96):
        raise CtcAsrError('the conv_s12 kernels cover w [32|96, 32, 11, 21] only.')
    _expect_numel('conv_s12_pack_weights', 'packed', packed, conv_s12_packed_floats(cout))
    packed = torch.empty(conv_s12_packed_floats(cout), dtype=torch.float32,
                         device=weight.device) if packed is None else packed
    _check(load().ctcasr_conv_s12_pack_weights(_dev(weight, name='weight'),
                                               _dev(packed, name='packed'), cout, _stream()),
           'conv_s12_pack_weights')
    return packed


@_on_tensor_device
def conv_s12_fwd(x, packed, cout, bias=None, out=None, relu_cutoff=0.0, time_major=False):
    batch, frames, freq, cin = _conv_dims('conv_s12_fwd', 'x', x, 4)
    if cin != 32 or not conv_s12_supported(freq, cout):
        raise CtcAsrError('conv_s12_fwd: unsupported layer shape {} -> {} channels'.format(
            tuple(x.shape), cout))
    _expect_numel('conv_s12_fwd', 'packed', packed, conv_s12_packed_floats(cout))
    _expect_numel('conv_s12_fwd', 'bias', bias, cout)
    _expect_numel('conv_s12_fwd', 'out', out, batch * frames * (freq // 2) * cout)
    shape = (frames, batch, freq // 2, cout) if time_major else (batch, frames, freq // 2, cout)
    out = torch.empty(shape, dtype=torch.float32, device=x.device) if out is None else out
    with _Timed('conv_s12_fwd'):
        _check(load().ctcasr_conv_s12_fwd(_dev(x, name='x'), _dev(packed, name='packed'),
                                          _dev(bias, name='bias'), _dev(out, name='y'), batch,
                                          frames, freq, cout, float(relu_cutoff),
                                          1 if time_major else 0, _stream()), 'conv_s12_fwd')
    return out


@_on_tensor_device
def conv_s12_pack_weights16(weight, packed=None):
    cout = weight.shape[0] if weight.dim() == 4 else 0
    nbytes = load().ctcasr_conv_s12_pack16_bytes(int(cout))
    if nbytes == 0 or tuple(weight.shape[1:]) != (32, 11, 21):
        raise CtcAsrError('conv_s12_pack_weights16: unsupported kernel shape {}'.format(
            tuple(weight.shape)))
    if packed is None or packed.numel() != nbytes:
        packed = torch.empty(nbytes, dtype=torch.uint8, device=weight.device)
    _check(load().ctcasr_conv_s12_pack_weights16(_dev(weight, name='weight'),
                                                 _dev(packed, torch.uint8, 'packed'), int(cout),
                                                 _stream()), 'conv_s12_pack_weights16')
    return packed


@_on_tensor_device
def conv_s12_fwd16(x, x_scale, packed16, cout, bias=None, out=None, relu_cutoff=0.0,
                   time_major=False):
    batch, frames, freq, cin = _conv_dims('conv_s12_fwd16', 'x', x, 4)
    if cin != 32 or not conv_s12_supported(freq, cout):
        raise CtcAsrError('conv_s12_fwd16: unsupported layer shape {} -> {} channels'.format(
            tuple(x.shape), cout))
    x_scale = _conv_scale('conv_s12_fwd16', x_scale)
    _expect_numel('conv_s12_fwd16', 'packed16', packed16,
                  load().ctcasr_conv_s12_pack16_bytes(int(cout)))
    _expect_numel('conv_s12_fwd16', 'bias', bias, cout)
    _expect_numel('conv_s12_fwd16', 'out', out, batch * frames * (freq // 2) * cout)
    shape = (frames, batch, freq // 2, cout) if time_major else (batch, frames, freq // 2, cout)
    out = torch.empty(shape, dtype=torch.float32, device=x.device) if out is None else out
    with _Timed('conv_s12_fwd'):
        _check(load().ctcasr_conv_s12_fwd16(_dev(x, name='x'), x_scale,
                                            _dev(packed16, torch.uint8, 'packed16'),
                                            _dev(bias, name='bias'), _dev(out, name='y'), batch,
                                            frames, freq, cout, float(relu_cutoff),
                                            1 if time_major else 0, _stream()), 'conv_s12_fwd16')
    return out


def _conv_s12_dz(what, dz, time_major):
    dims = _conv_dims(what, 'dz', dz, 4)
    frames, batch = (dims[0], dims[1]) if time_major else (dims[1], dims[0])
    if not conv_s12_supported(2 * dims[2], dims[3]):
        raise CtcAsrError('{}: unsupported layer shape {}'.format(what, tuple(dz.shape)))
    return batch, frames, dims[2], dims[3]


@_on_tensor_device
def conv_s12_bwd_data(dz, packed, out=None, time_major=False, act=None, relu_cutoff=0.0):
    batch, frames, freq_out, cout = _conv_s12_dz('conv_s12_bwd_data', dz, time_major)
    _conv_mask('conv_s12_bwd_data', dz, act, relu_cutoff, None, cout)
    _expect_numel('conv_s12_bwd_data', 'packed', packed, conv_s12_packed_floats(cout))
    _expect_numel('conv_s12_bwd_data', 'out', out, batch * frames * 2 * freq_out * 32)
    out = torch.empty((batch, frames, 2 * freq_out, 32), dtype=torch.float32, device=dz.device) \
        if out is None else out
    with _Timed('conv_s12_bwd_data'):
        _check(load().ctcasr_conv_s12_bwd_data(_dev(dz, name='dz'), _dev(packed, name='packed'),
                                               _dev(out, name='dx'), batch, frames,
                                               2 * freq_out, cout, 1 if time_major else 0,
                                               _dev(act, name='act'), float(relu_cutoff),
                                               _stream()), 'conv_s12_bwd_data')
    return out


@_on_tensor_device
def conv_s12_bwd_data16(dz, packed16, out=None, time_major=False, act=None, relu_cutoff=0.0):
    batch, frames, freq_out, cout = _conv_s12_dz('conv_s12_bwd_data16', dz, time_major)
    _conv_mask('conv_s12_bwd_data16', dz, act, relu_cutoff, None, cout)
    _expect_numel('conv_s12_bwd_data16', 'packed16', packed16,
                  load().ctcasr_conv_s12_pack16_bytes(int(cout)))
    _expect_numel('conv_s12_bwd_data16', 'out', out, batch * frames * 2 * freq_out * 32)
    out = torch.empty((batch, frames, 2 * freq_out, 32), dtype=torch.float32, device=dz.device) \
        if out is None else out
    with _Timed('conv_s12_bwd_data'):
        _check(load().ctcasr_conv_s12_bwd_data16(_dev(dz, name='dz'),
                                                 _dev(packed16, torch.uint8, 'packed16'),
                                                 _dev(out, name='dx'), batch, frames,
                                                 2 * freq_out, cout, 1 if time_major else 0,
                                                 _dev(act, name='act'), float(relu_cutoff),
                                                 _stream()), 'conv_s12_bwd_data16')
    return out


@_on_tensor_device
def conv_s12_wrw(dz, x, out=None, time_major=False, act=None, relu_cutoff=0.0, dbias=None):
    batch, frames, freq_out, cout = _conv_s12_dz('conv_s12_wrw', dz, time_major)
    if tuple(x.shape) != (batch, frames, 2 * freq_out, 32):
        raise CtcAsrError('conv_s12_wrw: unsupported layer shape {} / {}'.format(
            tuple(dz.shape), tuple(x.shape)))
    _conv_mask('conv_s12_wrw', dz, act, relu_cutoff, dbias, cout)
    _expect_numel('conv_s12_wrw', 'out', out, cout * 32 * 11 * 21)
    out = torch.empty((cout, 32, 11, 21), dtype=torch.float32, device=x.device) if out is None \
        else out
    workspace = _workspace(load().ctcasr_conv_s12_wrw_workspace_bytes(batch, frames,
                                                                      2 * freq_out, cout),
                           x.device)
    with _Timed('conv_s12_wrw'):
        _check(load().ctcasr_conv_s12_wrw(_dev(dz, name='dz'), _dev(x, name='x'),
                                          _dev(out, name='dw'), batch, frames, 2 * freq_out, cout,
                                          1 if time_major else 0, _dev(act, name='act'),
                                          float(relu_cutoff), _dev(dbias, name='dbias'),
                                          _dev(workspace, torch.uint8, 'workspace'),
                                          workspace.numel(), _stream()), 'conv_s12_wrw')
    return out


@_on_tensor_device
def conv_s12_wrw16(dz, x, x_scale, out=None, time_major=False, act=None, relu_cutoff=0.0,
                   dbias=None):
    batch, frames, freq_out, cout = _conv_s12_dz('conv_s12_wrw16', dz, time_major)
    if tuple(x.shape) != (batch, frames, 2 * freq_out, 32):
        raise CtcAsrError('conv_s12_wrw16: unsupported layer shape {} / {}'.format(
            tuple(dz.shape), tuple(x.shape)))
    x_scale = _conv_scale('conv_s12_wrw16', x_scale)
    _conv_mask('conv_s12_wrw16', dz, act, relu_cutoff, dbias, cout)
    _expect_numel('conv_s12_wrw16', 'out', out, cout * 32 * 11 * 21)
    out = torch.empty((cout, 32, 11, 21), dtype=torch.float32, device=x.device) if out is None \
        else out
    workspace = _workspace(load().ctcasr_conv_s12_wrw16_workspace_bytes(batch, frames,
                                                                        2 * freq_out, cout),
                           x.device)
    with _Timed('conv_s12_wrw'):
        _check(load().ctcasr_conv_s12_wrw16(_dev(dz, name='dz'), _dev(x, name='x'),
                                            x_scale, _dev(out, name='dw'), batch, frames,
                                            2 * freq_out, cout, 1 if time_major else 0,
                                            _dev(act, name='act'), float(relu_cutoff),
                                            _dev(dbias, name='dbias'),
                                            _dev(workspace, torch.uint8, 'workspace'),
                                            workspace.numel(), _stream()), 'conv_s12_wrw16')
    return out


def _conv0_x(what, x):
    batch, frames, freq = _conv_dims(what, 'x', x, 3)
    if freq != 80:
        raise CtcAsrError('{} covers x [B,T,80] only (got {}).'.format(what, tuple(x.shape)))
    return batch, frames


@_on_tensor_device
def conv0_fwd(x, weight, bias=None, out=None, relu_cutoff=0.0):
    batch, frames = _conv0_x('conv0_fwd', x)
    if tuple(weight.shape) != (32, 1, 11, 41):
        raise CtcAsrError('conv0_fwd covers x [B,T,80] and w [32,1,11,41] only.')
    _expect_numel('conv0_fwd', 'bias', bias, 32)
    _expect_numel('conv0_fwd', 'out', out, batch * ((frames + 1) // 2) * 40 * 32)
    out = torch.empty((batch, (frames + 1) // 2, 40, 32), dtype=torch.float32,
                      device=x.device) if out is None else out
    with _Timed('conv0_fwd'):
        _check(load().ctcasr_conv0_fwd(_dev(x, name='x'), _dev(weight, name='weight'),
                                       _dev(bias, name='bias'), _dev(out, name='y'), batch,
                                       frames, float(relu_cutoff), _stream()), 'conv0_fwd')
    return out


@_on_tensor_device
def conv0_pack_weights16(weight, out=None):
    if tuple(weight.shape) != (32, 1, 11, 41):
        raise CtcAsrError('conv0_pack_weights16 covers w [32,1,11,41] only.')
    nbytes = load().ctcasr_conv0_pack16_bytes()
    _expect_numel('conv0_pack_weights16', 'out', out, nbytes)
    out = torch.empty(nbytes, dtype=torch.uint8, device=weight.device) if out is None else out
    _check(load().ctcasr_conv0_pack_weights16(_dev(weight, name='weight'),
                                              _dev(out, torch.uint8, 'packed16'), _stream()),
           'conv0_pack_weights16')
    return out


@_on_tensor_device
def conv0_fwd16(x, packed16, bias=None, out=None, relu_cutoff=0.0):
    batch, frames = _conv0_x('conv0_fwd16', x)
    _expect_numel('conv0_fwd16', 'packed16', packed16, load().ctcasr_conv0_pack16_bytes())
    _expect_numel('conv0_fwd16', 'bias', bias, 32)
    _expect_numel('conv0_fwd16', 'out', out, batch * ((frames + 1) // 2) * 40 * 32)
    out = torch.empty((batch, (frames + 1) // 2, 40, 32), dtype=torch.float32,
                      device=x.device) if out is None else out
    with _Timed('conv0_fwd'):
        _check(load().ctcasr_conv0_fwd16(_dev(x, name='x'), _dev(packed16, torch.uint8, 'packed16'),
                                         _dev(bias, name='bias'), _dev(out, name='y'), batch,
                                         frames, float(relu_cutoff), _stream()), 'conv0_fwd16')
    return out


@_on_tensor_device
def conv0_wrw16(dz, x, out=None, act=None, relu_cutoff=0.0, dbias=None):
    batch, frames = _conv0_x('conv0_wrw16', x)
    if tuple(dz.shape) != (batch, (frames + 1) // 2, 40, 32):
        raise CtcAsrError('conv0_wrw16 covers x [B,T,80], dz [B,ceil(T/2),40,32] only.')
    _conv_mask('conv0_wrw16', dz, act, relu_cutoff, dbias, 32)
    _expect_numel('conv0_wrw16', 'out', out, 32 * 11 * 41)
    out = torch.empty((32, 1, 11, 41), dtype=torch.float32, device=x.device) if out is None \
        else out
    workspace = _workspace(load().ctcasr_conv0_wrw16_workspace_bytes(batch, frames), x.device)
    with _Timed('conv0_wrw'):
        _check(load().ctcasr_conv0_wrw16(_dev(dz, name='dz'), _dev(x, name='x'),
                                         _dev(out, name='dw'), batch, frames,
                                         _dev(act, name='act'), float(relu_cutoff),
                                         _dev(dbias, name='dbias'),
                                         _dev(workspace, torch.uint8, 'workspace'),
                                         workspace.numel(), _stream()), 'conv0_wrw16')
    return out


@_on_tensor_device
def conv0_wrw(dz, x, out=None, act=None, relu_cutoff=0.0, dbias=None):
    batch, frames = _conv0_x('conv0_wrw', x)
    if tuple(dz.shape) != (batch, (frames + 1) // 2, 40, 32):
        raise CtcAsrError('conv0_wrw covers x [B,T,80], dz [B,ceil(T/2),40,32] only.')
    _conv_mask('conv0_wrw', dz, act, relu_cutoff, dbias, 32)
    _expect_numel('conv0_wrw', 'out', out, 32 * 11 * 41)
    out = torch.empty((32, 1, 11, 41), dtype=torch.float32, device=x.device) if out is None \
        else out
    workspace = _workspace(load().ctcasr_conv0_wrw_workspace_bytes(batch, frames), x.device)
    with _Timed('conv0_wrw'):
        _check(load().ctcasr_conv0_wrw(_dev(dz, name='dz'), _dev(x, name='x'),
                                       _dev(out, name='dw'), batch, frames, _dev(act, name='act'),
                                       float(relu_cutoff), _dev(dbias, name='dbias'),
                                       _dev(workspace, torch.uint8, 'workspace'),
                                       workspace.numel(), _stream()), 'conv0_wrw')
    return out


@_on_tensor_device
def transpose_batched(src, out=None):
    if src.dim() != 3:
        raise CtcAsrError('transpose_batched: src must be [N, R, C] (got {} dimensions).'
                          .format(src.dim()))
    batch, rows, cols = src.shape
    out = torch.empty((batch, cols, rows), dtype=torch.float32, device=src.device) \
        if out is None else out
    if tuple(out.shape) != (batch, cols, rows):
        raise CtcAsrError('transpose_batched: out must be [N, C, R] = {} (got {}).'
                          .format((batch, cols, rows), tuple(out.shape)))
    _check(load().ctcasr_transpose_batched(_dev(src, name='src'), _dev(out, name='out'), batch,
                                           rows, cols, _stream()), 'transpose_batched')
    return out


@_on_tensor_device
def adam_step(param, grad, m, v, step, lr=1e-5, beta1=0.9, beta2=0.999, epsilon=1e-8,
              grad_scale=1.0, skip=None, grad_factor=None, ema=None, ema_alpha=None):
    for name, tensor in (('grad', grad), ('m', m), ('v', v)):
        _expect_numel('adam_step', name, tensor, param.numel())
    if skip is not None and skip.numel() < 1:
        raise CtcAsrError('adam_step: skip holds no word.')
    if ema is not None:
        _expect_numel('adam_step', 'ema', ema, param.numel())
        if ema_alpha is None:
            raise CtcAsrError('adam_step: ema needs ema_alpha.')
        if grad_factor is not None:
            _expect_numel('adam_step', 'grad_factor', grad_factor, 1)
        _check(load().ctcasr_adam_step_ema(
            _dev(param, name='param'), _dev(grad, name='grad'), _dev(m, name='m'),
            _dev(v, name='v'), _dev(ema, name='ema'), param.numel(), float(lr), float(beta1),
            float(beta2), float(epsilon), int(step), float(grad_scale),
            _dev(skip, torch.int32, 'skip'), _dev(grad_factor, name='grad_factor'),
            float(ema_alpha), _stream()), 'adam_step')
        return
    if ema_alpha is not None:
        raise CtcAsrError('adam_step: ema_alpha without ema.')
    if grad_factor is not None:
        _expect_numel('adam_step', 'grad_factor', grad_factor, 1)
        _check(load().ctcasr_adam_step_clipped(
            _dev(param, name='param'), _dev(grad, name='grad'), _dev(m, name='m'),
            _dev(v, name='v'), param.numel(), float(lr), float(beta1), float(beta2),
            float(epsilon), int(step), float(grad_scale), _dev(skip, torch.int32, 'skip'),
            _dev(grad_factor, name='grad_factor'), _stream()), 'adam_step')
        return
    _check(load().ctcasr_adam_step(_dev(param, name='param'), _dev(grad, name='grad'),
                                   _dev(m, name='m'), _dev(v, name='v'), param.numel(), float(lr),
                                   float(beta1), float(beta2), float(epsilon), int(step),
                                   float(grad_scale), _dev(skip, torch.int32, 'skip'), _stream()),
           'adam_step')


def grad_norm_workspace_bytes(n, segments):
    return load().ctcasr_grad_norm_workspace_bytes(int(n), int(segments))


@_on_tensor_device
def grad_norm(grad, seg_offsets, grad_scale=1.0, max_norm=0.0, skip=None, out=None,
              workspace=None):
    segments = seg_offsets.numel() - 1
    if segments < 1:
        raise CtcAsrError('grad_norm: seg_offsets holds {} offsets, at least 2 needed.'
                          .format(seg_offsets.numel()))
    if segments > GRAD_NORM_MAX_SEGMENTS:
        raise CtcAsrError('grad_norm: {} segments, at most {} supported.'
                          .format(segments, GRAD_NORM_MAX_SEGMENTS))
    if skip is not None and skip.numel() < 1:
        raise CtcAsrError('grad_norm: skip holds no word.')
    if out is None:
        out = torch.empty(segments + 2, dtype=torch.float32, device=grad.device)
    _expect_numel('grad_norm', 'out', out, segments + 2)
    need = grad_norm_workspace_bytes(grad.numel(), segments)
    if workspace is None:
        workspace = _workspace(need, grad.device)
    elif workspace.numel() < need:
        raise CtcAsrError('grad_norm: workspace holds {} bytes, {} needed.'
                          .format(workspace.numel(), need))
    out_ptr = _dev(out, name='out')
    _check(load().ctcasr_grad_norm(_dev(grad, name='grad'), grad.numel(),
                                   _dev(seg_offsets, torch.int64, 'seg_offsets'), segments,
                                   float(grad_scale), float(max_norm), out_ptr,
                                   out_ptr + 4 * (segments + 1), _dev(skip, torch.int32, 'skip'),
                                   _dev(workspace, torch.uint8, 'workspace'), workspace.numel(),
                                   _stream()), 'grad_norm')
    return out[:segments + 1], out[segments + 1:]


def seq_bn_workspace_bytes(rows, channels):
    return load().ctcasr_seq_bn_workspace_bytes(int(rows), int(channels))


def _seq_bn_shape(what, x, lengths, per_channel):
    if x.dim() != 3:
        raise CtcAsrError('{}: x must be [T, B, C] (got {} dimensions).'.format(what, x.dim()))
    steps, batch, channels = x.shape
    if channels < 4 or channels % 4 != 0:
        raise CtcAsrError('{}: {} channels; a multiple of 4 is needed.'.format(what, channels))
    if steps < 1 or batch < 1:
        raise CtcAsrError('{}: x is empty (shape {}).'.format(what, tuple(x.shape)))
    if lengths is not None:
        _expect_numel(what, 'lengths', lengths, batch)
    for name, tensor in per_channel:
        _expect_numel(what, name, tensor, channels)
    return steps, batch, channels


def _seq_bn_workspace(what, workspace, rows, channels, device):
    need = seq_bn_workspace_bytes(rows, channels)
    if workspace is None:
        return _workspace(need, device)
    if workspace.numel() < need:
        raise CtcAsrError('{}: workspace holds {} bytes, {} needed.'
                          .format(what, workspace.numel(), need))
    return workspace


@_on_tensor_device
def seq_bn_fwd(x, lengths, gamma, beta, running_mean, running_var, decay, eps, workspace=None):
    steps, batch, channels = _seq_bn_shape(
        'seq_bn_fwd', x, lengths, (('gamma', gamma), ('beta', beta),
                                   ('running_mean', running_mean), ('running_var', running_var)))
    workspace = _seq_bn_workspace('seq_bn_fwd', workspace, steps * batch, channels, x.device)
    y = torch.empty_like(x)
    mean = torch.empty(channels, dtype=torch.float32, device=x.device)
    rstd = torch.empty(channels, dtype=torch.float32, device=x.device)
    _check(load().ctcasr_seq_bn_fwd(
        _dev(x, name='x'), _dev(lengths, torch.int32, 'lengths'), steps, batch, channels,
        _dev(gamma, name='gamma'), _dev(beta, name='beta'),
        _dev(running_mean, name='running_mean'), _dev(running_var, name='running_var'),
        float(decay), float(eps), _dev(y, name='y'), _dev(mean, name='mean'),
# ... 397 lines not shown
```

ctc_asr_amd/model.py:

```python

import contextlib
import math
import os

import numpy as np
import torch

from ctc_asr_amd import hip, metrics, split_gemm
from ctc_asr_amd.labels import num_classes
from ctc_asr_amd.params import check_mwer_settings, ema_alpha_at

CONV_KERNEL_SIZES = ((11, 41), (11, 21), (11, 21))
CONV_STRIDES = ((2, 2), (1, 2), (1, 2))
GATES = {'lstm': 4, 'gru': 3, 'rnn_relu': 1, 'rnn_tanh': 1}
BN_EPS = 1e-5


class InfeasibleAlignmentError(ValueError):
    """Raised where ``tf.nn.ctc_loss`` raises InvalidArgumentError ("Not enough time for target
    transition sequence"), ``ignore_longer_outputs_than_inputs=False`` (``asr/model.py:259``)."""


class ModelConfig:

# ... 214 lines not shown

    def touch(self):
        self.version += 1

    def load(self, flat_params):
        for name in self.offsets:
            value = torch.as_tensor(np.asarray(flat_params[name]), dtype=torch.float32)
            if name.startswith('conv') and name.endswith('kernel'):
                value = value.permute(3, 2, 0, 1)
            self.p[name].copy_(value.contiguous().to(self.device))
        self.version += 1
        self.seed_ema()

    def seed_ema(self):
        if self.ema is not None:
            self.ema.copy_(self.param)

    def export(self, which='param'):
        if which == 'ema':
            if self.ema is None:
                raise ValueError('export: this arena keeps no averaged parameters.')
            views = {n: self._view(self.ema, n) for n in self.offsets}
        else:
            views = self.p if which == 'param' else self.g
        out = {}
        for name, view in views.items():
            value = view.detach().cpu()
            if name.startswith('conv') and name.endswith('kernel'):
                value = value.permute(2, 3, 1, 0)
            out[name] = value.contiguous().numpy().copy()
        return out


def predicted_input_bounds(cfg, training):
    if cfg.used_model == 'ds2':
        bound = cfg.relu_cutoff / (1.0 - cfg.conv_dropout_rate)
    else:
        bound = cfg.relu_cutoff / (1.0 - (cfg.dense_dropout_rate if training else 0.0))
    rate = cfg.rnn_dropout_rate if training else 0.0
    bounds = []
    for i in range(cfg.num_layers_rnn):
        if cfg.rnn_batch_norm and i > 0:
            bound = None
        if rate > 0.0 and (i > 0 or not cfg.cudnn) and bound is not None:
            bound = bound / (1.0 - rate)
        bounds.append(bound)
        bound = None if cfg.cell == 'rnn_relu' else 1.0
        if rate > 0.0 and not cfg.cudnn and bound is not None:
            bound = bound / (1.0 - rate)
    return bounds + [bound]


class _WeightPieces:

    def __init__(self, model, name, matrix, training):
        self.model, self.name, self.matrix, self.training = model, name, matrix, training
        self.fwd16 = self.tr16 = None
        self.dg16 = None
        self.rows_form = False
        self._fwd = self._tr = None

    def make_fwd(self, out=None):
        if self.name == 'dense4':
            stacked = split_gemm.split_rows_stacked(self.matrix, split_gemm.B_ORDER, out=out)
            self._fwd = stacked.view(-1, self.matrix.shape[1])
        else:
            self._fwd = split_gemm.split(self.matrix, split_gemm.B_ORDER, out=out)
        return self._fwd

    def make_tr(self, out=None, scratch=None):
        if self.name == 'dense4':
            self._tr = split_gemm.split(self.matrix, split_gemm.A_ORDER, out=out)
        else:
            rows, cols = self.matrix.shape
            if scratch is None:
                scratch = torch.empty((cols, rows), dtype=torch.float32,
                                      device=self.matrix.device)
            hip.transpose_batched(self.matrix.view(1, rows, cols), out=scratch.view(1, cols, rows))
            self._tr = split_gemm.split(scratch, split_gemm.A_ORDER, out=out)
        return self._tr

    def make_tr16(self, out=None, scratch=None):
        rows, cols = self.matrix.shape
        if scratch is None:
            scratch = torch.empty((cols, rows), dtype=torch.float32, device=self.matrix.device)
        hip.transpose_batched(self.matrix.view(1, rows, cols), out=scratch.view(1, cols, rows))
        self.tr16 = split_gemm.split16(scratch, split_gemm.W_SCALE, split_gemm.H_B, out=out)
        return self.tr16

    def __getitem__(self, index):
        if index == 0:
            return self._fwd if self._fwd is not None else self.make_fwd()
        if index == 1:
            return self._tr if self._tr is not None else self.make_tr()
        return (self.fwd16, self.tr16)[index - 2]


class CTCModel:

    def __init__(self, cfg, device='cuda', seed=0, params=None, conv_autotune=None, ema=False):
        side_gate_max_us = int(os.environ.get('CTCASR_SIDE_GATE_US', '300'))
        if side_gate_max_us > hip.RESIDENT_GATE_MAX_US:
            raise ValueError('CTCASR_SIDE_GATE_US={}: a residency gate waits {} us at the most '
                             '(0 disables the gates).'.format(side_gate_max_us,
                                                              hip.RESIDENT_GATE_MAX_US))
        hip.load()
        if conv_autotune is None:
            conv_autotune = os.environ.get('CTCASR_CONV_AUTOTUNE', '0') == '1'
        if conv_autotune:
            torch.backends.cudnn.benchmark = True
        else:
            os.environ.setdefault('MIOPEN_FIND_MODE', 'FAST')
            torch.backends.cudnn.benchmark = False
        self.cfg = cfg
        self.device = torch.device(device)
        if self.device.type != 'cuda':
            raise hip.CtcAsrError('CTCModel runs on the MI355X only; there is no CPU path.')
        self.arena = ParamArena(cfg, self.device, ema=ema)
        self._grad_norm_state = None
        self.arena.load(params if params is not None else init_params(cfg, seed))
        self.step_count = 0
        self.overlap_wgrad = os.environ.get('CTCASR_OVERLAP_WGRAD', '1') == '1'
        self.own_conv = os.environ.get('CTCASR_OWN_CONV', '1') == '1'
        self._conv_packed = {}
        self._conv_packed16 = {}
        self.conv_f16 = os.environ.get('CTCASR_CONV_F16', '1') == '1'
        self.conv_wrw_f16 = os.environ.get('CTCASR_CONV_WRW_F16', '1') == '1'
        self.conv_fused_bwd = os.environ.get('CTCASR_CONV_FUSED_BWD', '1') == '1'
        self.side_gate_max_us = side_gate_max_us
        self._ticket = 0
        self.bwd_chunks = max(0, int(os.environ.get('CTCASR_BWD_CHUNKS', '0')))
        self.fwd_chunks = max(1, int(os.environ.get('CTCASR_FWD_CHUNKS', '4')))
        self.fwd_pipeline_max_batch = int(os.environ.get('CTCASR_FWD_PIPELINE_MAX_BATCH', '16'))
        self.split_gemm = os.environ.get('CTCASR_SPLIT_GEMM', '1') == '1'
        self.split_dense4 = os.environ.get('CTCASR_SPLIT_DENSE4', '1') == '1'
        self.fwd_f16 = os.environ.get('CTCASR_FWD_F16', '1') == '1'
        self.bwd_f16 = os.environ.get('CTCASR_BWD_F16', '1') == '1'
        self.split_wgrad = os.environ.get('CTCASR_SPLIT_WGRAD', '1') == '1'
        self.own_dgrad = os.environ.get('CTCASR_OWN_DGRAD', '1') == '1'
        self.own_wgrad = os.environ.get('CTCASR_OWN_WGRAD', '1') == '1'
        self.own_wgrad_parts = int(os.environ.get('CTCASR_WGRAD_PARTS', '2'))
        self.unbounded_f16 = os.environ.get('CTCASR_UNBOUNDED_F16', '1') == '1'
        self.rnn_fwd_f16 = os.environ.get('CTCASR_RNN_FWD_F16', '1') == '1'
        self.rnn_bwd_f16 = os.environ.get('CTCASR_RNN_BWD_F16', '1') == '1'
        self.rnn_xcd_flag = hip.RNN_XCD_SPLIT \
            if os.environ.get('CTCASR_RNN_XCD_SPLIT', '1') == '1' else 0
        self.rnn_stagger_flag = hip.RNN_STAGGER \
            if os.environ.get('CTCASR_RNN_STAGGER', '1') == '1' else 0
        self.rnn_kpair_wide = os.environ.get('CTCASR_RNN_KPAIR_2048', '1') == '1'
        self.rnn_fwd_pieces = os.environ.get('CTCASR_RNN_FWD_PIECES', '1') == '1'
        self._w_split, self._w_split_ready, self._w_split_bufs = {}, None, {}
        self._w_guard = None
        self._side_stream = None
        self.early_hooks = False
        self.rnn_bwd_flags = int(os.environ.get('CTCASR_RNN_BWD_FLAGS', str(hip.RNN_DEFAULT)))
        self.gpu_metrics = os.environ.get('CTCASR_GPU_METRICS', '1') == '1'
        self._rnn_ws = {}
        self.dropout_seed = int(seed) * 0x9E3779B1 + 1
        self.bn_state = None
        if cfg.rnn_batch_norm and cfg.num_layers_rnn > 1:
            self.bn_state = torch.zeros((cfg.num_layers_rnn - 1, 2, 2 * cfg.num_units_rnn),
                                        dtype=torch.float32, device=self.device)
            self.bn_state[:, 1].fill_(1.0)
        self._bn_ws = None
        self._acts = None
        self._w_hh_t = [torch.empty((2, cfg.num_units_rnn, GATES[cfg.cell] * cfg.num_units_rnn),
                                    dtype=torch.float32, device=self.device)
                        for _ in range(cfg.num_layers_rnn)]

    def _upcoming_ticket(self):
        return self._ticket % 0xFFFFFF + 1

    def _take_ticket(self):
        self._ticket = self._upcoming_ticket()
        return self._ticket

    def _gate_side_stream(self, cell, workspace, t_out, batch, hidden):
        if self.side_gate_max_us > 0:
            hip.rnn_resident_gate(cell, workspace, t_out, batch, hidden, self._upcoming_ticket(),
                                  self.side_gate_max_us)

    def _predicted_bounds(self, training):
        return predicted_input_bounds(self.cfg, training)

    def _weights_in_f16_range(self, names, views, side):
        fresh = self._w_guard is None or self._w_guard['version'] != self.arena.version or \
            self._w_guard['names'] != names
        if fresh:
            self._w_guard = {
                'version': self.arena.version, 'names': names, 'event': None,
                'dev': torch.zeros(len(names), dtype=torch.int32, device=self.device),
                'host': torch.zeros(len(names), dtype=torch.int32).pin_memory(),
                'max': None}
        guard = self._w_guard

        def measure():
            with torch.cuda.stream(side):
                guard['dev'].zero_()
                for k, view in enumerate(views):
                    hip.absmax(view, guard['dev'][k:k + 1])
                guard['host'].copy_(guard['dev'], non_blocking=True)
                guard['event'] = torch.cuda.Event()
                guard['event'].record(side)

        if fresh:
            measure()
            guard['event'].synchronize()
        if guard['event'] is not None and guard['event'].query():
            guard['max'] = guard['host'].view(torch.float32).clone().numpy()
            guard['event'] = None
        if guard['event'] is None:
            measure()
        limit = 0.5 * split_gemm.F16_MAX / split_gemm.W_SCALE
        return {name: bool(guard['max'][k] <= limit) for k, name in enumerate(names)}

    def _prepare_weight_splits(self, rows, training, batch=None):
        cfg, p = self.cfg, self.arena.p
        self._w_split, self._w_split_ready = {}, None
        if not self.split_gemm:
            return
        gh2 = 2 * GATES[cfg.cell] * cfg.num_units_rnn
        jobs = []
        for i in range(cfg.num_layers_rnn):
            w_ih = p['rnn{}/w_ih'.format(i)].view(gh2, -1)
            if split_gemm.worthwhile(rows, w_ih.shape[1], gh2):
                jobs.append((i, 'rnn{}'.format(i), w_ih))
        k4 = p['dense4/kernel']
        dense4 = self.split_dense4 and split_gemm.worthwhile(rows, k4.shape[0], k4.shape[1])
        if not jobs and not dense4:
            return
        main = torch.cuda.current_stream(self.device)
        if self._side_stream is None:
            self._side_stream = torch.cuda.Stream(self.device)
        side = self._side_stream
        bufs = self._w_split_bufs
        start = torch.cuda.Event()
        start.record(main)
        side.wait_event(start)
        bounds = self._predicted_bounds(training)
        in_range = {}
        if self.fwd_f16:
            names = tuple(name for _, name, _ in jobs) + (('dense4',) if dense4 else ())
            views = [w for _, _, w in jobs] + ([k4] if dense4 else [])
            in_range = self._weights_in_f16_range(names, views, side)

        def rows_form(layer, name):
            return (self.fwd_f16 and self.unbounded_f16 and in_range.get(name, False) and
                    bounds[layer] is None)

        def f16_form(layer, name):
            return (self.fwd_f16 and in_range.get(name, False) and
                    split_gemm.f16_scale(bounds[layer]) is not None) or rows_form(layer, name)

        def buf(key, make):
            if key not in bufs:
                bufs[key] = make()
            return bufs[key]

        dense4_f16 = dense4 and f16_form(cfg.num_layers_rnn, 'dense4')
        hidden = cfg.num_units_rnn
        own_dgrad = bool(
            training and batch and self.own_dgrad and self.bwd_f16 and self.rnn_bwd_f16 and
            cfg.cell == 'lstm' and cfg.cudnn and rows % batch == 0 and
            hip.dgrad16_supported(cfg.cell, rows // batch, batch, hidden) and
            hip.rnn_bwd_f16_supported(cfg.cell, rows // batch, batch, hidden,
                                      self.rnn_bwd_flags | hip.RNN_F16))
        with torch.cuda.stream(side):
            for i, name, w_ih in jobs:
                cols = w_ih.shape[1]
                pieces = _WeightPieces(self, name, w_ih, training)
                pieces.rows_form = rows_form(i, name)
                if f16_form(i, name):
                    pieces.fwd16 = split_gemm.split16(
                        w_ih, split_gemm.W_SCALE, split_gemm.H_B,
                        out=buf(name + '/f16', lambda: split_gemm.empty16(
                            gh2, cols, split_gemm.H_B, self.device)))
                    above_f16 = f16_form(i + 1, 'rnn{}'.format(i + 1)) \
                        if i + 1 < cfg.num_layers_rnn else dense4_f16
                    bn_above = self.bn_state is not None and i + 1 < cfg.num_layers_rnn
                    above_f16 = above_f16 and not bn_above
                    if training and self.bwd_f16 and above_f16 and own_dgrad:
                        pieces.dg16 = hip.dgrad16_pack_weights(
                            w_ih, hidden, split_gemm.W_SCALE,
                            out=buf(name + '/dg16', lambda: torch.empty(
                                hip.dgrad16_packed_bytes(cols), dtype=torch.uint8,
                                device=self.device)))
                    elif training and self.bwd_f16 and above_f16:
                        pieces.make_tr16(
                            buf(name + '/t16', lambda: split_gemm.empty16(
                                cols, gh2, split_gemm.H_B, self.device)),
                            buf(name + '/t', lambda: torch.empty(
                                (cols, gh2), dtype=torch.float32, device=self.device)))
                    elif training and bn_above:
                        pieces.make_tr(
                            buf(name + '/tbf16', lambda: split_gemm.empty(
                                cols, gh2, split_gemm.A_ORDER, self.device)),
                            buf(name + '/t', lambda: torch.empty(
                                (cols, gh2), dtype=torch.float32, device=self.device)))
                else:
                    pieces.make_fwd(buf(name + '/bf16', lambda: split_gemm.empty(
                        gh2, cols, split_gemm.B_ORDER, self.device)))
                    if training:
                        pieces.make_tr(
                            buf(name + '/tbf16', lambda: split_gemm.empty(
                                cols, gh2, split_gemm.A_ORDER, self.device)),
                            buf(name + '/t', lambda: torch.empty(
                                (cols, gh2), dtype=torch.float32, device=self.device)))
                self._w_split[name] = pieces
            if dense4:
                pieces = _WeightPieces(self, 'dense4', k4, training)
                pieces.rows_form = rows_form(cfg.num_layers_rnn, 'dense4')
                if dense4_f16:
                    stacked16 = buf('dense4/f16', lambda: torch.empty(
                        (3,) + tuple(k4.shape), dtype=torch.float16, device=self.device))
                    split_gemm.split16_rows_stacked(k4, split_gemm.W_SCALE, split_gemm.H_B,
                                                    out=stacked16)
                    pieces.fwd16 = stacked16.view(-1, k4.shape[1])
                else:
                    pieces.make_fwd(buf('dense4/bf16', lambda: torch.empty(
                        (6,) + tuple(k4.shape), dtype=torch.bfloat16, device=self.device)))
                if training and dense4_f16 and self.bwd_f16:
                    pieces.tr16 = split_gemm.split16(
                        k4, split_gemm.W_SCALE, split_gemm.H_B,
                        out=buf('dense4/t16', lambda: split_gemm.empty16(
                            k4.shape[0], k4.shape[1], split_gemm.H_B, self.device)))
                elif training:
                    pieces.make_tr(buf('dense4/tbf16', lambda: split_gemm.empty(
                        k4.shape[0], k4.shape[1], split_gemm.A_ORDER, self.device)), None)
                self._w_split['dense4'] = pieces
            self._w_split_ready = torch.cuda.Event()
            self._w_split_ready.record(side)

    def _weight_split(self, name, backward=False, acts=None):
        pieces, ready = (self._w_split, self._w_split_ready) if acts is None else \
            (acts['w_split'], acts['w_split_ready'])
        got = pieces.get(name)
        if got is None:
            return None
        if ready is not None:
            torch.cuda.current_stream(self.device).wait_event(ready)
        return got

    def _next_seed(self):
        self.dropout_seed = (self.dropout_seed * 6364136223846793005 + 1442695040888963407) \
            & 0xFFFFFFFFFFFFFFFF
        return self.dropout_seed

    def _dense_act(self, x2d, name, rate, training, xs=None):
        p = self.arena.p
        if xs is not None:
            out = split_gemm.mm_nn_stacked(xs, self._weight_split(name)[0])
        else:
            out = torch.mm(x2d, p[name + '/kernel'])
        hip.bias_act_fwd(out, p[name + '/bias'], self.cfg.relu_cutoff,
                         rate if training else 0.0, self._next_seed())
        return out

    def inference_fn(self, sequences, seq_length, training=True):
        cfg, p = self.cfg, self.arena.p
        sequences = sequences.to(self.device, torch.float32).contiguous()
        batch, frames, _ = sequences.shape
        acts = {'training': training, 'batch': batch, 'conv_f16': {}}
        acts['input_poison'] = torch.where(
            torch.isfinite(sequences).view(batch, -1).all(dim=1), 0.0, float('nan')).to(torch.float32)
        self._prepare_weight_splits(cfg.output_time(frames) * batch, training, batch)
        if cfg.used_model == 'ds2':
            x = sequences.unsqueeze(1).contiguous(memory_format=torch.channels_last)
            conv_in, conv_out, pads, own_kind = [], [], [], []
            layers = len(cfg.conv_filters)
            fused = cfg.conv_dropout_rate == 0.0
            last_time_major = False
            for i in range(layers):
                k_t, k_f = CONV_KERNEL_SIZES[i]
                s_t, s_f = CONV_STRIDES[i]
                _, pt0, pt1 = same_padding(x.shape[2], k_t, s_t)
                _, pf0, pf1 = same_padding(x.shape[3], k_f, s_f)
                own_kind.append('conv0' if self._own_conv0_layer(i, x.shape[3]) else
                                's12' if self._own_conv_layer(i, x.shape[3]) else None)
                cutoff = cfg.relu_cutoff if fused else 0.0
                if own_kind[i] == 'conv0':
                    if self.conv_f16:
                        self._conv_packed16[0] = hip.conv0_pack_weights16(
                            p['conv0/kernel'], self._conv_packed16.get(0))
                        y = hip.conv0_fwd16(sequences, self._conv_packed16[0], p['conv0/bias'],
                                            relu_cutoff=cutoff).permute(0, 3, 1, 2)
                    else:
                        y = hip.conv0_fwd(sequences, p['conv0/kernel'], p['conv0/bias'],
                                          relu_cutoff=cutoff).permute(0, 3, 1, 2)
                    acts.setdefault('arithmetic_front', {})['conv0/forward'] = \
                        'fp16x3' if self.conv_f16 else 'fp32'
                    conv_in.append(None)
                    acts['features'] = sequences
                elif own_kind[i] == 's12':
                    kernel = p['conv{}/kernel'.format(i)]
                    last_time_major = fused and i == layers - 1
                    x_scale = split_gemm.f16_scale(cfg.relu_cutoff) \
                        if (self.conv_f16 and fused and i > 0) else None
                    if x_scale is not None:
                        self._conv_packed16[i] = hip.conv_s12_pack_weights16(
                            kernel, self._conv_packed16.get(i))
                        y = hip.conv_s12_fwd16(x.permute(0, 2, 3, 1), x_scale,
                                               self._conv_packed16[i], kernel.shape[0],
                                               p['conv{}/bias'.format(i)], relu_cutoff=cutoff,
                                               time_major=last_time_major)
                    else:
                        self._conv_packed[i] = hip.conv_s12_pack_weights(
                            kernel, self._conv_packed.get(i))
                        y = hip.conv_s12_fwd(x.permute(0, 2, 3, 1), self._conv_packed[i],
                                             kernel.shape[0], p['conv{}/bias'.format(i)],
                                             relu_cutoff=cutoff, time_major=last_time_major)
                    acts.setdefault('arithmetic_front', {})['conv{}/forward'.format(i)] = \
                        'fp16x3' if x_scale is not None else 'fp32'
                    acts.setdefault('conv_f16', {})[i] = x_scale
                    if not last_time_major:
                        y = y.permute(0, 3, 1, 2)
                    conv_in.append(x)
                else:
                    xp = torch.nn.functional.pad(x, (pf0, pf1, pt0, pt1)) \
                        .contiguous(memory_format=torch.channels_last)
                    y = torch.ops.aten.convolution(xp, self._conv_kernel_cl(i),
                                                   p['conv{}/bias'.format(i)], [s_t, s_f],
                                                   [0, 0], [1, 1], False, [0, 0], 1)
                    y = y.contiguous(memory_format=torch.channels_last)
                    conv_in.append(xp)
                if own_kind[i] is None or not fused:
                    hip.bias_act_fwd(y.permute(0, 2, 3, 1), None, cfg.relu_cutoff,
                                     cfg.conv_dropout_rate, self._next_seed())
                conv_out.append(y)
                pads.append((pt0, pt1, pf0, pf1))
                x = y
            if last_time_major:
                t_out = x.shape[0]
                rnn_in = x.view(t_out, batch, -1)
            else:
                t_out = x.shape[2]
                rnn_in = x.permute(2, 0, 3, 1).reshape(t_out, batch, -1)
            acts.update(conv_in=conv_in, conv_out=conv_out, pads=pads, conv_own=own_kind,
                        last_time_major=last_time_major)
            seq_length = torch.full((batch,), t_out, dtype=torch.int32, device=self.device)
            in_bound = cfg.relu_cutoff / (1.0 - cfg.conv_dropout_rate)
        else:
            t_out = frames
            x2d = sequences.transpose(0, 1).reshape(t_out * batch, -1)
            dense_in, dense_out = [], []
            for i in range(3):
                dense_in.append(x2d)
                x2d = self._dense_act(x2d, 'dense{}'.format(i), cfg.dense_dropout_rate, training)
                dense_out.append(x2d)
            rnn_in = x2d.view(t_out, batch, -1)
            in_bound = cfg.relu_cutoff / (1.0 - (cfg.dense_dropout_rate if training else 0.0))
            acts.update(dense_in=dense_in, dense_out=dense_out)
            seq_length = torch.as_tensor(seq_length).to(self.device, torch.int32).contiguous()

        cell, hidden, gates = cfg.cell, cfg.num_units_rnn, GATES[cfg.cell]
        rnn_len = None if cfg.cudnn else seq_length
        layer_in, layer_out, reserves, drop_seeds = [], [], [], []
        arithmetic = acts['arithmetic'] = dict(acts.get('arithmetic_front', {}))
        f16_rec = (self.rnn_fwd_f16 and cell in ('lstm', 'gru') and
                   hip.rnn_persistent_supported(cell, t_out, batch, hidden))
        rnn_flags = (hip.RNN_F16 | self.rnn_xcd_flag) if f16_rec else hip.RNN_DEFAULT
        rnn_form = 'fp16x3' if f16_rec else 'fp32'
        in_split = []
        in_split16 = []
        pipelined_xw = None
        y16_of = None
        x = rnn_in.contiguous()
        workspace = self._rnn_workspace(cell, t_out, batch, hidden)
        rnn_rate = cfg.rnn_dropout_rate if training else 0.0
        bn_on = self.bn_state is not None
        bn_saved = []
        for i in range(cfg.num_layers_rnn):
            seeds = [None, None]
            bn_saved.append(None)
            if bn_on and i > 0:
                bn_name = 'rnn{}/bn_'.format(i)
                state = self.bn_state[i - 1]
                if training:
                    x_bn, bn_mean, bn_rstd = hip.seq_bn_fwd(
                        x, rnn_len, p[bn_name + 'gamma'], p[bn_name + 'beta'], state[0],
                        state[1], cfg.rnn_bn_decay, BN_EPS,
                        workspace=self._bn_workspace(t_out * batch, 2 * hidden))
                    bn_saved[i] = (x, bn_mean, bn_rstd)
                else:
                    x_bn = hip.seq_bn_infer(x, rnn_len, p[bn_name + 'gamma'],
                                            p[bn_name + 'beta'], state[0], state[1], BN_EPS)
                x, in_bound = x_bn, None
            if rnn_rate > 0.0 and (i > 0 or not cfg.cudnn):
                seeds[0] = self._next_seed()
                x = hip.dropout(x, rnn_rate, seeds[0])
                in_bound = in_bound / (1.0 - rnn_rate) if in_bound is not None else None
            w_ih = p['rnn{}/w_ih'.format(i)].view(2 * gates * hidden, -1)
            xs = ws = pieces16 = None
            form = 'fp32'
            if pipelined_xw is not None:
                xw, pipelined_xw = pipelined_xw, None
            elif self._weight_split('rnn{}'.format(i)) is not None:
                w_pieces = self._weight_split('rnn{}'.format(i))
                scale = split_gemm.f16_scale(in_bound) if w_pieces[2] is not None else None
                if scale is None and w_pieces[2] is not None and w_pieces.rows_form:
                    x2d = x.view(t_out * batch, -1)
                    xw = split_gemm.mm_rows16(x2d, w_pieces[2], split_gemm.W_SCALE)
                    pieces16 = split_gemm.ColScaled(x2d)
                    form = 'fp16x3 (row / column scales)'
                elif scale is not None:
                    if y16_of is not None and y16_of[0] is x and y16_of[2] == scale:
                        x16 = y16_of[1]
                    else:
                        x16 = split_gemm.split16(x.view(t_out * batch, -1), scale, split_gemm.H_A)
                    xw = split_gemm.mm_nt16(x16, w_pieces[2], scale * split_gemm.W_SCALE)
                    pieces16 = (x16, scale)
                    form = 'fp16x3'
                else:
                    xs = split_gemm.split(x.view(t_out * batch, -1), split_gemm.A_ORDER)
                    xw = split_gemm.mm_nt(xs, w_pieces[0])
                    form = 'bf16x6'
            else:
                xw = torch.mm(x.view(t_out * batch, -1), w_ih.t())
            in_split.append(xs)
            in_split16.append(pieces16)
            arithmetic['rnn{}/input_projection'.format(i)] = form
            if self._pipeline_forward(i, cell, t_out, batch, hidden, rnn_len, rnn_rate):
                y16_of = None
                y, reserve, workspace, pipelined_xw = self._rnn_fwd_pipelined(
                    i, xw, t_out, batch, hidden, gates, workspace)
            else:
                y16 = None
                consumer = 'rnn{}'.format(i + 1) if i + 1 < cfg.num_layers_rnn else 'dense4'
                if (f16_rec and self.rnn_fwd_pieces and rnn_len is None and
                        not (rnn_rate > 0.0 and (not cfg.cudnn or i + 1 < cfg.num_layers_rnn)) and
                        not (bn_on and i + 1 < cfg.num_layers_rnn) and
                        hip.rnn_fwd_f16_supported(cell, t_out, batch, hidden, rnn_flags)):
                    pieces = self._weight_split(consumer)
                    if pieces is not None and pieces[2] is not None:
                        y16 = split_gemm.empty16(t_out * batch, 2 * hidden, split_gemm.H_A,
                                                 self.device)
                y, reserve, workspace = hip.rnn_fwd(
                    cell, xw.view(t_out, batch, 2, gates * hidden), p['rnn{}/w_hh'.format(i)],
                    rnn_len, b_hh_n=p['rnn{}/b_hh'.format(i)] if cell == 'gru' else None,
                    workspace=workspace, xw_bias=self._rnn_bias(i), flags=rnn_flags,
                    y16=None if y16 is None else y16.buf)
                y16_of = None if y16 is None else (y, y16, split_gemm.RNN_F16_H_SCALE)
            arithmetic['rnn{}/recurrence_fwd'.format(i)] = rnn_form
            layer_in.append(x)
            layer_out.append(y)
            reserves.append(reserve)
            x = y
            in_bound = None if cell == 'rnn_relu' else 1.0
            if rnn_rate > 0.0 and not cfg.cudnn:
                seeds[1] = self._next_seed()
                x = hip.dropout(x, rnn_rate, seeds[1])
                in_bound = in_bound / (1.0 - rnn_rate) if in_bound is not None else None
            drop_seeds.append(seeds)
        acts.update(layer_in=layer_in, layer_out=layer_out, reserves=reserves, rnn_ws=workspace,
# ... 174 lines not shown
        else:
            flat, offsets, max_len, _ = self.pack_labels(labels, self.device)
        batch = logits.shape[1]
        per_utt, grad, status = hip.ctc_loss_fwd_bwd(logits, flat, offsets, seq_length, max_len,
                                                     grad_scale=1.0 / batch)
        if self._acts is not None:
            self._acts['dlogits'] = grad
            if self._acts.get('input_poison') is not None and \
                    self._acts['input_poison'].shape == per_utt.shape:
                per_utt = per_utt + self._acts['input_poison']
        self.last_status, self.last_per_utterance_loss = status, per_utt
        if check:
            self.check_status(status)
        return per_utt.mean()

    def mwer_loss_fn(self, logits, seq_length, labels, originals=None, nbest=4, beam_width=64,
                     ctc_weight=0.01, risk='word', check=True):
        from ctc_asr_amd.labels import decode
        check_mwer_settings(nbest, beam_width, ctc_weight, risk)
        nbest = int(nbest)
        if nbest < 2:
            raise ValueError('mwer_loss_fn(): nbest={} is not in 2..64.'.format(nbest))
        if isinstance(labels, tuple) and len(labels) == 4 and torch.is_tensor(labels[0]):
            flat, offsets, max_len, rows = labels
        else:
            flat, offsets, max_len, rows = self.pack_labels(labels, self.device)
        num_steps, batch = int(logits.shape[0]), int(logits.shape[1])
        per_utt, grad, status = hip.ctc_loss_fwd_bwd(logits, flat, offsets, seq_length, max_len,
                                                     grad_scale=float(ctc_weight) / batch)
        out, out_len, _, n_paths = hip.ctc_beam_decode_nbest(logits, seq_length, beam_width,
                                                            nbest)
        dev = out.device
        lengths = out_len.reshape(-1).clamp(0, num_steps)
        hyp_flat, hyp_offsets = self._pack_rows(out, lengths)
        if risk == 'label':
            ref_len = (offsets[1:] - offsets[:-1]).repeat_interleave(nbest).contiguous()
            distance = hip.edit_distance(
                out, torch.arange(batch * nbest, device=dev, dtype=torch.int32) * num_steps,
                lengths, flat, offsets[:-1].repeat_interleave(nbest).contiguous(), ref_len)[0]
            risks = distance.to(torch.float32)
            longest = int(lengths.max())
        else:
            host = torch.cat([out.reshape(-1), lengths, n_paths]).cpu().numpy()
            host_out = host[:batch * nbest * num_steps].reshape(batch, nbest, num_steps)
            host_len = host[batch * nbest * num_steps:-batch].reshape(batch, nbest)
            if originals is None or len(originals) == 0:
                originals = [decode(row) for row in rows]
            if len(originals) != batch:
                raise ValueError('mwer_loss_fn(): {} transcripts for a batch of {}.'.format(
                    len(originals), batch))
            used = [(b, k) for b in range(batch) for k in range(int(host[-batch + b]))]
            texts = [decode(host_out[b, k, :host_len[b, k]].tolist()) for b, k in used]
            ref_words, hyp_words = metrics.word_ids([originals[b] for b, _ in used], texts)
            counts = metrics.error_counts(hyp_words, ref_words, self.device)
            host_risk = np.zeros((batch, nbest), dtype=np.float32)
            for (b, k), count in zip(used, counts[:, 0]):
                host_risk[b, k] = count
            risks = torch.from_numpy(host_risk.reshape(-1)).to(dev)
            longest = int(host_len.max())
        grad, expected, score, posterior, hyp_status = hip.ctc_mwer(
            logits, seq_length, hyp_flat, hyp_offsets, n_paths, risks,
            max_label_len=max(longest, 0), scale=1.0 / batch, accumulate=True, grad=grad)
        total = expected + float(ctc_weight) * per_utt
        if self._acts is not None:
            self._acts['dlogits'] = grad
            if self._acts.get('input_poison') is not None and \
                    self._acts['input_poison'].shape == total.shape:
                total = total + self._acts['input_poison']
        self.last_status, self.last_per_utterance_loss = status, total
        self.last_mwer = {'labels': hyp_flat, 'label_offsets': hyp_offsets, 'n_hyps': n_paths,
                          'risk': risks, 'expected_risk': expected, 'score': score,
                          'posterior': posterior, 'status': hyp_status, 'out': out,
                          'out_len': out_len, 'ctc_loss': per_utt}
        if check:
            self.check_status(status)
        return total.mean()

    def align_fn(self, logits, seq_len, labels):
        if isinstance(labels, tuple) and len(labels) == 4 and torch.is_tensor(labels[0]):
            flat, offsets, max_len, _ = labels
        else:
            flat, offsets, max_len, _ = self.pack_labels(labels, self.device)
        return hip.ctc_align(logits, flat, offsets, seq_len, max_len)

    def align_long_fn(self, logits, labels):
        if not torch.is_tensor(labels):
            labels = torch.tensor([int(v) for v in labels], dtype=torch.int32,
                                  device=self.device)
        return hip.ctc_align_long(logits, labels)

    def search_fn(self, logits, seq_len, phrases, min_score_per_label, max_hits=16, pairs=None):
        rows = [[int(v) for v in phrase] for phrase in phrases]
        batch = int(logits.shape[1])
        if pairs is None:
            pairs = [(b, p) for b in range(batch) for p in range(len(rows))]
        pairs = [(int(b), int(p)) for b, p in pairs]
        count, max_hits = len(pairs), int(max_hits)
        offsets = np.zeros(len(rows) + 1, dtype=np.int32)
        offsets[1:] = np.cumsum([len(r) for r in rows])
        flat = np.array([v for r in rows for v in r] or [0], dtype=np.int32)
        lengths = np.array([len(r) for r in rows], dtype=np.float64)
        min_score = np.float64(min_score_per_label) * lengths
        dev = logits.device
        host = [torch.as_tensor(flat), torch.as_tensor(offsets), torch.as_tensor(min_score),
                torch.tensor([b for b, _ in pairs], dtype=torch.int32),
                torch.tensor([p for _, p in pairs], dtype=torch.int32)]
        flat_d, offsets_d, min_score_d, utt_d, phrase_d = (t.to(dev) for t in host)
        hits, hit_score, n_hits, best_score, best_span, _, _, status = hip.ctc_search(
            logits, seq_len, flat_d, offsets_d, utt_d, phrase_d, min_score_d, max_hits=max_hits)
        packed = torch.cat([hits.reshape(count, 2 * max_hits).double(), hit_score,
                            n_hits[:, None].double(), best_score[:, None], best_span.double(),
                            status[:, None].double()], dim=1).cpu().numpy()
        spans = packed[:, :2 * max_hits].astype(np.int32).reshape(count, max_hits, 2)
        scores = packed[:, 2 * max_hits:3 * max_hits]
        tail = packed[:, 3 * max_hits:]
        per_pair = {'utt': np.array([b for b, _ in pairs], dtype=np.int32),
                    'phrase': np.array([p for _, p in pairs], dtype=np.int32),
                    'n_hits': tail[:, 0].astype(np.int32), 'best_score': tail[:, 1].copy(),
                    'best_span': tail[:, 2:4].astype(np.int32),
                    'status': tail[:, 4].astype(np.int32)}
        found = []
        for h, (b, p) in enumerate(pairs):
            for k in range(min(int(per_pair['n_hits'][h]), max_hits)):
                score = float(scores[h, k])
                found.append({'phrase': p, 'utt': b, 'start': int(spans[h, k, 0]),
                              'end': int(spans[h, k, 1]), 'score': score,
                              'score_per_label': score / len(rows[p])})
        return found, per_pair

    @staticmethod
    def check_status(status):
        bad = status.cpu().numpy()
        if (bad == 1).any():
            raise InfeasibleAlignmentError(
                'Not enough time for target transition sequence (batch rows {})'
                .format(np.nonzero(bad == 1)[0].tolist()))
        if (bad == 2).any():
            raise ValueError('CTC labels out of range or sequence_length > max_time (rows {})'
                             .format(np.nonzero(bad == 2)[0].tolist()))

    def backward(self, reduce_hook=None, accumulate=False):
        cfg, p, g, acts = self.cfg, self.arena.p, self.arena.g, self._acts
        if acts is None or 'dlogits' not in acts:
            raise RuntimeError('backward() needs inference_fn() and loss_fn() first.')
        if self.bn_state is not None and not acts['training']:
            raise RuntimeError('backward() through rnn_batch_norm needs a training-mode forward '
                               'pass: the batch statistics it normalised with.')
        slices = {name: (start, stop) for name, start, stop in self.arena.layer_slices}

        def done(layer):
            if reduce_hook is not None:
                reduce_hook(layer, *slices[layer])

        if not accumulate:
            self.arena.grad.zero_()

        def write(view, fn):
            if not accumulate:
                fn(view)
                return
            scratch = torch.empty_like(view)
            fn(scratch)
            view.add_(scratch)

        arith = acts.setdefault('arithmetic', {})
        training = acts['training']
        t_out, batch = acts['t_out'], acts['batch']
        hidden, gates, cell = cfg.num_units_rnn, GATES[cfg.cell], cfg.cell
        rows = t_out * batch
        dlogits = acts['dlogits'].view(rows, cfg.num_classes)
        main = torch.cuda.current_stream(self.device)
        side = main
        if self.overlap_wgrad:
            if self._side_stream is None:
                self._side_stream = torch.cuda.Stream(self.device)
            side = self._side_stream
        deferred = []

        whole_chip_rnn = (cfg.cell in ('lstm', 'gru') and cfg.num_units_rnn == 2048 and
                          hip.rnn_persistent_supported(cfg.cell, acts['t_out'], acts['batch'],
                                                       cfg.num_units_rnn))

        persistent = hip.rnn_persistent_supported(cfg.cell, acts['t_out'], acts['batch'],
                                                  cfg.num_units_rnn)

        def on_side(tensors, fn, gate=False, beside_recurrence=True):
            if side is main or (whole_chip_rnn and beside_recurrence):
                fn()
                return
            ready = torch.cuda.Event()
            ready.record(main)
            with torch.cuda.stream(side):
                side.wait_event(ready)
                if gate and persistent:
                    self._gate_side_stream(cfg.cell, acts['rnn_ws'], acts['t_out'], acts['batch'],
                                           cfg.num_units_rnn)
                fn()
            for tensor in tensors:
                tensor.record_stream(side)

        for i in range(cfg.num_layers_rnn):
            hip.transpose_batched(p['rnn{}/w_hh'.format(i)], out=self._w_hh_t[i])

        write(g['logits/kernel'], lambda out: torch.mm(acts['dense4'].t(), dlogits, out=out))
        hip.colsum_accumulate(dlogits, g['logits/bias'])
        d_dense4 = torch.mm(dlogits, p['logits/kernel'].t())
        done('logits')
        dz = hip.bias_act_bwd(acts['dense4'], d_dense4, cfg.relu_cutoff,
                              cfg.dense_dropout_rate if training else 0.0, g['dense4/bias'])
        k4_split = self._weight_split('dense4', True, acts) if acts['flat_uses_split'] else None
        dz_split = None
        if k4_split is not None and k4_split[3] is not None:
            dy = split_gemm.dgrad16(dz, k4_split[3], split_gemm.W_SCALE) \
                .view(t_out, batch, 2 * hidden)
            acts['arithmetic']['dense4/data_gradient'] = 'fp16x3'
        elif k4_split is not None:
            dz_split = split_gemm.split(dz, split_gemm.B_ORDER)
            dy = split_gemm.mm_nt(dz_split, k4_split[1]).view(t_out, batch, 2 * hidden)
        else:
            dy = torch.mm(dz, p['dense4/kernel'].t()).view(t_out, batch, 2 * hidden)
        early = self.early_hooks

        flat16 = acts.get('flat16')
        k4_f16 = (self.bwd_f16 and k4_split is not None and flat16 is not None and
                  self.split_wgrad and os.environ.get('CTCASR_DENSE4_WGRAD_F16', '1') == '1')
        acts['arithmetic']['dense4/kernel_gradient'] = \
            'fp16x3' if k4_f16 else ('bf16x6' if k4_split is not None else 'fp32')

        def dense4_weight_grad(dz_split=dz_split):
            if k4_f16:
                dz16, dz_inv = split_gemm.wgrad16_operand(dz)
                pieces, scale = flat16[0], flat16[1]
                inv = getattr(flat16, 'col_inv', None)
                if inv is None:
                    inv = torch.ones(pieces.cols, dtype=torch.float32, device=dz.device)
                if not accumulate:
                    g['dense4/kernel'].zero_()
                split_gemm.wgrad16(g['dense4/kernel'], pieces.buf, inv,
                                   split_gemm.Split(dz16, split_gemm.H_B), scale, 0,
                                   x_col_inv=dz_inv)
            elif k4_split is not None:
                if dz_split is None:
                    dz_split = split_gemm.split(dz, split_gemm.B_ORDER)
                if acts['flat_split'] is None:
                    acts['flat_split'] = split_gemm.split(acts['rnn_flat'], split_gemm.A_ORDER)
                split_gemm.mm_tn_rows(g['dense4/kernel'], acts['flat_split'], dz_split, 0, rows,
                                      accumulate=accumulate)
            else:
                write(g['dense4/kernel'], lambda out: torch.mm(acts['rnn_flat'].t(), dz, out=out))
            if early:
                done('dense4')

        on_side([dz] + ([dz_split.buf] if dz_split is not None else []) +
                ([acts['flat_split'].buf] if acts['flat_split'] is not None else []),
                dense4_weight_grad, gate=True)
        if not early:
            deferred.append('dense4')

        need_dx_first = True
        rnn_rate = acts['rnn_rate']
        for i in range(cfg.num_layers_rnn - 1, -1, -1):
            name = 'rnn{}'.format(i)
            x, y = acts['layer_in'][i], acts['layer_out'][i]
            seeds = acts['drop_seeds'][i]
            if seeds[1] is not None:
                dy = hip.dropout(dy.contiguous(), rnn_rate, seeds[1])
            gh = gates * hidden
            chunks = 1
            if (side is not main and acts['rnn_len'] is None and not whole_chip_rnn and
                    persistent):
                chunks = self.bwd_chunks or 2
                if t_out < 8 * chunks:
                    chunks = 1
            dy = dy.contiguous()
            dxw = torch.empty((t_out, batch, 2, gh), dtype=torch.float32, device=dy.device)

            drec = hip.rnn_gru_drec(acts['reserves'][i], t_out, batch, hidden) if cell == 'gru' \
                else dxw
            dxw2d = dxw.view(rows, 2 * gh)
            w_ih = p[name + '/w_ih'].view(2 * gh, -1)

            w_pieces = self._weight_split(name, True, acts)
            use_split = w_pieces is not None
            x16 = acts['in_split16'][i]
            if i + 1 < cfg.num_layers_rnn:
                y16 = acts['in_split16'][i + 1] if acts['layer_in'][i + 1] is y else None
            else:
                y16 = acts['flat16'] if acts['flat_of'] is y else None
            g16 = (self.bwd_f16 and use_split and x16 is not None and y16 is not None and
                   (w_pieces[3] is not None or w_pieces.dg16 is not None) and
                   2 * gh <= 16384 and self.split_wgrad)
            ds = drs = None
            if use_split and not g16:
                ds = split_gemm.empty(rows, 2 * gh, split_gemm.B_ORDER, dy.device)
                drs = ds if cell != 'gru' else \
                    split_gemm.empty(rows, 2 * gh, split_gemm.B_ORDER, dy.device)

            def input_pieces(layer=i, x=x):
                if acts['in_split'][layer] is None:
                    acts['in_split'][layer] = split_gemm.split(x.view(rows, -1),
                                                               split_gemm.A_ORDER)
                return acts['in_split'][layer]

            def output_pieces(layer=i, y=y):
                if layer + 1 < cfg.num_layers_rnn and acts['layer_in'][layer + 1] is y and \
                        acts['in_split'][layer + 1] is not None:
                    return acts['in_split'][layer + 1]
                if layer + 1 == cfg.num_layers_rnn and acts['flat_of'] is y and \
                        acts['flat_split'] is not None:
                    return acts['flat_split']
                if acts['out_split'][layer] is None:
                    acts['out_split'][layer] = split_gemm.split(y.view(rows, 2 * hidden),
                                                                split_gemm.A_ORDER)
                return acts['out_split'][layer]

            side_tensors = [dxw] + [t.buf for t in (ds, drs, acts['in_split'][i],
                                                    acts['flat_split']) if t is not None] + \
                [t[0].buf for t in (x16, y16)
                 if t is not None and not isinstance(t, split_gemm.ColScaled)]

            def split_steps(lo, hi, ds=ds, drs=drs, dxw2d=dxw2d, drec=drec):
                for d, (a, b) in enumerate(((lo, hi), (t_out - hi, t_out - lo))):
                    rng, cols = slice(a * batch, b * batch), slice(d * gh, (d + 1) * gh)
                    hip.split_bf16(dxw2d[rng, cols], split_gemm.B_ORDER, out=ds.buf[rng, :, cols])
                    if drs is not ds:
                        hip.split_bf16(drec.view(rows, 2 * gh)[rng, cols], split_gemm.B_ORDER,
                                       out=drs.buf[rng, :, cols])

            x_packs = {}

            def partial_weight_grads_f16(lo, hi, name=name, dxw2d=dxw2d, drec=drec, x16=x16,
                                         y16=y16, x=x, y=y, colmax=None, x_packs=x_packs):
                own = (self.own_wgrad and cell != 'gru' and
                       not isinstance(x16, split_gemm.ColScaled) and
                       not isinstance(y16, split_gemm.ColScaled))
                for d, (a, b) in enumerate(((lo, hi), (t_out - hi, t_out - lo))):
                    cols = slice(d * gh, (d + 1) * gh)
                    if own:
                        n_rows = (b - a) * batch
                        stages = (n_rows + 31) // 32
                        d_rows = dxw2d[a * batch:b * batch, cols]
                        scale, inv = hip.colmax_scale(d_rows) if colmax is None else \
                            hip.colscale_from_max(colmax[d * gh:(d + 1) * gh])
                        d_pk = hip.wgrad16_pack(d_rows, n_rows, 0, stages, 1.0, col_scale=scale)
                        x_pk = x_packs.pop((a, n_rows), None)
                        if x_pk is None:
                            x_pk = hip.wgrad16_pack(x.view(rows, -1), rows, a * batch, stages,
                                                    x16[1])
                            x_packs[(a, n_rows)] = x_pk
                        y_pk = hip.wgrad16_pack(
                            y.view(rows, 2 * hidden)[:, d * hidden:(d + 1) * hidden], rows,
                            (a + (1 if d else -1)) * batch, stages, y16[1])
                        hip.wgrad16_gemm(d_pk, gh, stages, inv, x_pk, 0, x16[1],
                                         g[name + '/w_ih'][d], y_packed=y_pk, y_scale=y16[1],
                                         dw_y=g[name + '/w_hh'][d], parts=self.own_wgrad_parts)
# ... 42 lines not shown
                    if b <= a:
                        continue
                    if ds is not None:
                        split_gemm.mm_tn_rows(g[name + '/w_hh'][d], drs, ys, a * batch, b * batch,
                                              a_cols=cols, b_cols=hcols, b_shift=shift * batch)
                    else:
                        g[name + '/w_hh'][d].addmm_(
                            drec[a:b, :, d, :].reshape((b - a) * batch, gh).t(),
                            y[a + shift:b + shift, :, hcols].reshape((b - a) * batch, hidden))

            b_start = self.arena.offsets[name + '/b_ih']
            b_count = 2 * gh * (2 if cell == 'gru' else 1)
            assert self.arena.offsets[name + '/b_hh'] == b_start + 2 * gh
            dbias = self.arena.grad[b_start:b_start + b_count]
            bounds = [t_out * (chunks - c) // chunks for c in range(chunks + 1)]
            split_done = []
            bwd_flags = self.rnn_bwd_flags | ((hip.RNN_F16 | self.rnn_xcd_flag |
                                               self.rnn_stagger_flag |
                                               (hip.RNN_KPAIR if hidden == 2048 and
                                                self.rnn_kpair_wide else 0))
                                              if self.rnn_bwd_f16 else 0)
            f16_rec = hip.rnn_f16_recurrence(cell, t_out, batch, hidden, bwd_flags, backward=True,
                                             ragged=acts['rnn_len'] is not None)
            arith['rnn{}/recurrence_bwd'.format(i)] = 'fp16x3' if f16_rec else 'fp32'
            colmax = torch.zeros((chunks, 2 * gh), dtype=torch.int32, device=dy.device) \
                if f16_rec and g16 else None
            if colmax is not None:
                side_tensors.append(colmax)
            need_dx = i > 0 or need_dx_first
            own_dg = (need_dx and g16 and w_pieces.dg16 is not None and f16_rec and
                      acts['rnn_len'] is None and
                      hip.dgrad16_supported(cell, t_out, batch, hidden))
            for c in range(chunks):
                hip.rnn_bwd(cell, dy, y, self._w_hh_t[i], acts['reserves'][i], acts['rnn_len'],
                            dxw=dxw, dbias=dbias, workspace=acts['rnn_ws'],
                            steps=(bounds[c + 1], bounds[c]), flags=bwd_flags,
                            ticket=self._take_ticket() if persistent and not whole_chip_rnn
                            else 0, colmax=None if colmax is None else colmax[c])
                if c + 1 < chunks:
                    def finished_steps(lo=bounds[c + 1], hi=bounds[c],
                                       colmax=None if colmax is None else colmax[c]):
                        if ds is not None:
                            split_steps(lo, hi)
                            split_done.append(torch.cuda.Event())
                            split_done[-1].record(torch.cuda.current_stream(self.device))
                        partial_weight_grads(lo, hi, colmax=colmax)
                    on_side(side_tensors, finished_steps, gate=True)
            if ds is not None:
                split_steps(0, bounds[-2])
                for event in split_done:
                    main.wait_event(event)
            dy_below = None
            if need_dx:
                arith['rnn{}/data_gradient'.format(i)] = \
                    'fp16x3 block-scaled (own kernel)' if own_dg else \
                    'fp16x3' if g16 else 'bf16x6' if use_split else 'fp32'
                if own_dg:
                    dy_below = hip.dgrad16_blockscaled(
                        acts['rnn_ws'], t_out, batch, hidden, w_pieces.dg16, split_gemm.W_SCALE,
                        w_ih.shape[1]).view(t_out, batch, -1)
                elif g16:
                    if w_pieces[3] is None:
                        w_pieces.make_tr16()
                    dy_below = split_gemm.dgrad16(
                        dxw2d, w_pieces[3], split_gemm.W_SCALE,
                        before_gemm=(lambda: main.wait_stream(side)) if side is not main
                        else None).view(t_out, batch, -1)
                elif side is not main:
                    main.wait_stream(side)
                if g16:
                    pass
                elif use_split:
                    dy_below = torch.empty((rows, x.shape[-1]), dtype=torch.float32,
                                           device=dy.device)
                    split_gemm.mm_nt_by_order(dy_below, ds, w_pieces[1])
                    dy_below = dy_below.view(t_out, batch, -1)
                else:
                    dy_below = torch.mm(dxw2d, w_ih).view(t_out, batch, -1)
                if seeds[0] is not None:
                    dy_below = hip.dropout(dy_below, rnn_rate, seeds[0])
                if acts['bn_saved'][i] is not None:
                    bn_in, bn_mean, bn_rstd = acts['bn_saved'][i]
                    dy_below = hip.seq_bn_bwd(
                        dy_below.contiguous(), bn_in, acts['rnn_len'], bn_mean, bn_rstd,
                        p[name + '/bn_gamma'], g[name + '/bn_gamma'], g[name + '/bn_beta'],
                        workspace=self._bn_workspace(rows, 2 * hidden))

            def weight_grads(name=name, x=x, y=y, dxw=dxw, dxw2d=dxw2d, i=i, chunks=chunks,
                             last=bounds[-2], partial_weight_grads=partial_weight_grads,
                             drec=drec, use_split=use_split,
                             colmax=None if colmax is None else colmax[chunks - 1]):
                if cell != 'gru':
                    g[name + '/b_hh'].copy_(g[name + '/b_ih'])
                if chunks > 1 or use_split:
                    partial_weight_grads(0, last, colmax=colmax)
                    return
                write(g[name + '/w_ih'].view(2 * gates * hidden, -1),
                      lambda out: torch.mm(dxw2d.t(), x.view(rows, -1), out=out))
                if t_out > 1:
                    gh = gates * hidden
                    write(g[name + '/w_hh'][0], lambda out: torch.mm(
                        drec[1:, :, 0, :].reshape((t_out - 1) * batch, gh).t(),
                        y[:-1, :, :hidden].reshape((t_out - 1) * batch, hidden), out=out))
                    write(g[name + '/w_hh'][1], lambda out: torch.mm(
                        drec[:-1, :, 1, :].reshape((t_out - 1) * batch, gh).t(),
                        y[1:, :, hidden:].reshape((t_out - 1) * batch, hidden), out=out))

            def layer_weight_grads(name=name, weight_grads=weight_grads):
                weight_grads()
                if early:
                    done(name)

            on_side(side_tensors, layer_weight_grads, gate=i > 0, beside_recurrence=i > 0)
            if not early:
                deferred.append(name)
            if dy_below is not None:
                dy = dy_below
        with torch.cuda.stream(side):
            for name in deferred:
                done(name)
            if hasattr(reduce_hook, 'flush'):
                reduce_hook.flush()

        if cfg.used_model == 'ds2':
            conv_out = acts['conv_out']
            last = conv_out[-1]
            if acts['last_time_major']:
                dact = dy.contiguous().view(last.shape)
            else:
                b_, c_, tt, ff = last.shape
                dact = dy.view(tt, b_, ff, c_).permute(1, 0, 2, 3).contiguous()
            if side is not main and any(kind is None for kind in acts['conv_own']):
                main.wait_stream(side)
            for i in range(len(cfg.conv_filters) - 1, -1, -1):
                name = 'conv{}'.format(i)
                tm = acts['last_time_major'] and i == len(cfg.conv_filters) - 1
                out_phys = conv_out[i] if tm else conv_out[i].permute(0, 2, 3, 1)
                own = acts['conv_own'][i]
                fused_bwd = (self.conv_fused_bwd and own is not None and
                             cfg.conv_dropout_rate == 0.0)
                if fused_bwd:
                    dz = dact if tm else dact.permute(0, 3, 1, 2)
                    mask = dict(act=out_phys, relu_cutoff=cfg.relu_cutoff)
                else:
                    dz = hip.bias_act_bwd(out_phys, dact, cfg.relu_cutoff,
                                          cfg.conv_dropout_rate, g[name + '/bias'])
                    if not tm:
                        dz = dz.permute(0, 3, 1, 2)
                    mask = {}
                pt0, pt1, pf0, pf1 = acts['pads'][i]
                if own == 'conv0':
                    wrw0 = hip.conv0_wrw16 if (self.conv_f16 and self.conv_wrw_f16) \
                        else hip.conv0_wrw
                    write(g[name + '/kernel'], lambda out: wrw0(
                        dz.permute(0, 2, 3, 1), acts['features'], out=out,
                        dbias=g[name + '/bias'] if fused_bwd else None, **mask))
                    done(name)
                    continue
                conv_in = acts['conv_in'][i]
                if own == 's12':
                    dz_phys = dz if tm else dz.permute(0, 2, 3, 1)
                    if acts['conv_f16'].get(i) and self.conv_wrw_f16:
                        write(g[name + '/kernel'], lambda out: hip.conv_s12_wrw16(
                            dz_phys, conv_in.permute(0, 2, 3, 1), acts['conv_f16'][i], out=out,
                            time_major=tm, dbias=g[name + '/bias'] if fused_bwd else None,
                            **mask))
                    else:
                        write(g[name + '/kernel'], lambda out: hip.conv_s12_wrw(
                            dz_phys, conv_in.permute(0, 2, 3, 1), out=out, time_major=tm,
                            dbias=g[name + '/bias'] if fused_bwd else None, **mask))
                    if i > 0 and acts['conv_f16'].get(i):
                        dact = hip.conv_s12_bwd_data16(dz_phys, self._conv_packed16[i],
                                                       time_major=tm, **mask)
                    elif i > 0:
                        dact = hip.conv_s12_bwd_data(dz_phys, self._conv_packed[i],
                                                     time_major=tm, **mask)
                    done(name)
                    continue
                need_dx = i > 0
                dxp, dw, _ = torch.ops.aten.convolution_backward(
                    dz, conv_in, self._conv_kernel_cl(i), [p[name + '/bias'].shape[0]],
                    list(CONV_STRIDES[i]), [0, 0], [1, 1], False, [0, 0], 1,
                    [need_dx, True, False])
                if accumulate:
                    g[name + '/kernel'].add_(dw)
                else:
                    g[name + '/kernel'].copy_(dw)
                if need_dx:
                    dact = dxp[:, :, pt0:dxp.shape[2] - pt1, pf0:dxp.shape[3] - pf1] \
                        .permute(0, 2, 3, 1).contiguous()
                done(name)
        else:
            if side is not main:
                main.wait_stream(side)
            dact = dy.reshape(rows, -1)
            for i in range(2, -1, -1):
                name = 'dense{}'.format(i)
                dz = hip.bias_act_bwd(acts['dense_out'][i], dact.contiguous(), cfg.relu_cutoff,
                                      cfg.dense_dropout_rate if training else 0.0,
                                      g[name + '/bias'])
                write(g[name + '/kernel'],
                      lambda out: torch.mm(acts['dense_in'][i].t(), dz, out=out))
                if i > 0:
                    dact = torch.mm(dz, p[name + '/kernel'].t())
                done(name)
        if side is not main:
            main.wait_stream(side)

    def forward_backward(self, features, feature_len, labels, reduce_hook=None, check=True,
                         accumulate=False, mwer=None, originals=None):
        logits, seq_length = self.inference_fn(features, feature_len, training=True)
        if mwer:
            loss = self.mwer_loss_fn(logits, seq_length, labels, originals=originals,
                                     check=check, **mwer)
        else:
            loss = self.loss_fn(logits, seq_length, labels, check=check)
        if accumulate:
            self.backward(reduce_hook, accumulate=True)
        else:
            self.backward(reduce_hook)
        return loss

    def step_guard(self):
        acts, cfg = self._acts, self.cfg
        words = (0, 0)
        if acts is not None and hip.rnn_persistent_supported(cfg.cell, acts['t_out'],
                                                             acts['batch'], cfg.num_units_rnn):
            words = hip.rnn_timeout_words(cfg.cell, acts['rnn_ws'], acts['t_out'], acts['batch'],
                                          cfg.num_units_rnn)
        return hip.step_guard(self.last_status, self.last_per_utterance_loss, words)

    @property
    def grad_norm_names(self):
        return [name for name, _, _ in self.arena.layer_slices]

    def grad_norms(self, grad_scale=1.0, max_norm=0.0, skip=None):
        if self._grad_norm_state is None:
            slices = self.arena.layer_slices
            offsets = torch.tensor([slices[0][1]] + [stop for _, _, stop in slices],
                                   dtype=torch.int64, device=self.device)
            workspace = torch.empty(
                max(hip.grad_norm_workspace_bytes(self.arena.size, len(slices)), 256),
                dtype=torch.uint8, device=self.device)
            out = torch.zeros(len(slices) + 2, dtype=torch.float32, device=self.device)
            self._grad_norm_state = (offsets, workspace, out)
        offsets, workspace, out = self._grad_norm_state
        return hip.grad_norm(self.arena.grad, offsets, grad_scale, max_norm, skip=skip, out=out,
                             workspace=workspace)

    def apply_gradients(self, learning_rate=1e-5, beta1=0.9, beta2=0.999, epsilon=1e-8,
                        grad_scale=1.0, skip=None, grad_factor=None, ema_decay=0.0):
        a = self.arena
        if ema_decay > 0.0 and a.ema is None:
            raise hip.CtcAsrError('apply_gradients: ema_decay needs a model built with ema=True.')
        alpha = ema_alpha_at(ema_decay, self.step_count) if ema_decay > 0.0 else None
        self.step_count += 1
        if alpha is None:
            hip.adam_step(a.param, a.grad, a.m, a.v, self.step_count, learning_rate, beta1, beta2,
                          epsilon, grad_scale, skip=skip, grad_factor=grad_factor)
        else:
            hip.adam_step(a.param, a.grad, a.m, a.v, self.step_count, learning_rate, beta1, beta2,
                          epsilon, grad_scale, skip=skip, grad_factor=grad_factor, ema=a.ema,
                          ema_alpha=alpha)

    @contextlib.contextmanager
    def ema_weights(self):
        a = self.arena
        if a.ema is None:
            raise hip.CtcAsrError('ema_weights: the model was built without an average.')

        def swap():
            scratch = a.param.clone()
            a.param.copy_(a.ema)
            a.ema.copy_(scratch)
            a.touch()

        swap()
        try:
            yield self
        finally:
            swap()

    def model_fn(self, features, labels, mode, learning_rate=1e-5, adam=(0.9, 0.999, 1e-8)):
        if mode not in ('train', 'eval', 'infer'):
            raise RuntimeError('Invalid mode.')
        logits, seq_length = self.inference_fn(features['spectrogram'],
                                               features['spectrogram_length'],
                                               training=(mode == 'train'))
        self.check_rnn_error()
        if mode == 'infer':
            decoded, plaintext, _ = self.decode_fn(logits, seq_length, None)
            return {'decoded': decoded, 'plaintext': plaintext}
        loss = self.loss_fn(logits, seq_length, labels)
        if mode == 'train':
            self.backward()
            self.apply_gradients(learning_rate, *adam)
        originals = features['label_plaintext']
        decoded, plaintext, summary = self.decode_fn(
            logits, seq_length, np.array([t.encode('utf-8') if isinstance(t, str) else t
                                          for t in originals], dtype=object))
        score = self.error_counts_fn if self.gpu_metrics else self.error_rates_fn
        _, mean_ed, _, wer = score(labels, [t.decode('utf-8') if isinstance(t, bytes) else t
                                            for t in originals], decoded, plaintext)[:4]
        return {'loss': loss, 'decoded': decoded, 'plaintext': plaintext, 'summary': summary,
                'mean_edit_distance': mean_ed, 'word_error_rate': wer}

    def decode_fn(self, logits, seq_len, originals=None, beam_width=None, greedy=False,
                  scorer=None):
        beam_width = self.cfg.beam_width if beam_width is None else beam_width
        if greedy:
            out, out_len = hip.ctc_greedy_decode(logits, seq_len)
        elif scorer is not None:
            out, out_len, _ = hip.ctc_beam_decode_lm(logits, seq_len, beam_width, scorer)
        else:
            out, out_len, _ = hip.ctc_beam_decode(logits, seq_len, beam_width)
        return self._decoded_to_text(out.cpu().numpy(), out_len.cpu().numpy(), originals)

    @staticmethod
    def _decoded_to_text(out, out_len, originals):
        decoded = [out[b, :out_len[b]].tolist() for b in range(out.shape[0])]
        return CTCModel._lists_to_text(decoded, originals)

    @staticmethod
    def _lists_to_text(decoded, originals):
        width = max([len(d) for d in decoded] + [0])
        dense = np.zeros((len(decoded), width), dtype=np.int32)
        for b, row in enumerate(decoded):
            dense[b, :len(row)] = row
        plaintext, summary = metrics.dense_to_text(dense, originals if originals is not None
                                                   else np.array([], dtype=np.int32))
        return decoded, plaintext, summary

    def decode_group_size(self, num_steps, batch, beam_width=None, budget_bytes=48 << 30,
                          max_utterances=256, scorer=None):
        beam_width = self.cfg.beam_width if beam_width is None else beam_width
        sizer = hip.ctc_beam_workspace_bytes if scorer is None else \
            hip.ctc_beam_lm_workspace_bytes
        per_utt = max(1, sizer(num_steps, 1, self.cfg.num_classes, beam_width))
        utterances = max(batch, min(max_utterances, budget_bytes // per_utt))
        return max(1, int(utterances // batch))

    def decode_many(self, batches, beam_width=None, scorer=None):
        beam_width = self.cfg.beam_width if beam_width is None else beam_width
        if not batches:
            return []
        steps = max(int(logits.shape[0]) for logits, _, _ in batches)
        total = sum(int(logits.shape[1]) for logits, _, _ in batches)
        classes = int(batches[0][0].shape[2])
        joint = torch.zeros((steps, total, classes), dtype=torch.float32, device=self.device)
        lengths = torch.empty(total, dtype=torch.int32, device=self.device)
        start = 0
        for logits, seq_len, _ in batches:
            stop = start + int(logits.shape[1])
            joint[:logits.shape[0], start:stop] = logits
            lengths[start:stop] = seq_len
            start = stop
        if scorer is not None:
            out, out_len, _ = hip.ctc_beam_decode_lm(joint, lengths, beam_width, scorer)
        else:
            out, out_len, _ = hip.ctc_beam_decode(joint, lengths, beam_width)
        out, out_len = out.cpu().numpy(), out_len.cpu().numpy()
        results, start = [], 0
        for logits, _, originals in batches:
            stop = start + int(logits.shape[1])
# ... 147 lines not shown
```

include/ctcasr.h:

```cpp
#ifndef CTCASR_H_
#define CTCASR_H_

#include <stddef.h>
#include <stdint.h>

#ifdef __cplusplus
extern "C" {
#endif

#define CTCASR_ABI_VERSION 8

enum {
    CTCASR_OK = 0,
    CTCASR_ERR_BAD_ARGUMENT = -1,
    CTCASR_ERR_UNSUPPORTED = -2,
    CTCASR_ERR_WORKSPACE = -3,
    CTCASR_ERR_LAUNCH = -4,
    CTCASR_ERR_TIMEOUT = -5
};

enum {
    CTCASR_CELL_RNN_RELU = 0,
    CTCASR_CELL_RNN_TANH = 1,
    CTCASR_CELL_LSTM = 2,
// ... 3 lines not shown
typedef void *ctcasr_stream_t;

int ctcasr_abi_version(void);
#define CTCASR_BUILD_PROBE_WRONG_RESULTS 1u
#define CTCASR_BUILD_NONDEFAULT_TUNING   2u
unsigned ctcasr_build_flags(void);
int ctcasr_set_option(const char *name, int value);
int ctcasr_rnn_kernel_events(int launches[2], double total_ms[2]);
const char *ctcasr_error_string(int code);

int ctcasr_log_softmax_fwd(const float *x, float *y, int rows, int C, ctcasr_stream_t stream);
int ctcasr_log_softmax_bwd(const float *y, const float *dy, float *dx, int rows, int C,
                           ctcasr_stream_t stream);

size_t ctcasr_ctc_loss_workspace_bytes(int T, int B, int C, int max_label_len);
int ctcasr_ctc_loss_fwd_bwd(const float *logits, const int32_t *labels,
                            const int32_t *label_offsets, const int32_t *seq_len, int T, int B,
                            int C, int blank, int max_label_len, float grad_scale, float *loss,
                            float *grad_logits, int32_t *status, void *workspace,
                            size_t workspace_bytes, ctcasr_stream_t stream);

int ctcasr_ctc_greedy_decode(const float *logits, const int32_t *seq_len, int T, int B, int C,
                             int blank, int32_t *out, int32_t *out_len, ctcasr_stream_t stream);

size_t ctcasr_ctc_beam_workspace_bytes(int T, int B, int C, int beam_width);
int ctcasr_ctc_beam_decode(const float *logits, const int32_t *seq_len, int T, int B, int C,
                           int blank, int beam_width, int norm_mode, int32_t *out,
                           int32_t *out_len, float *logp, void *workspace,
                           size_t workspace_bytes, ctcasr_stream_t stream);

size_t ctcasr_ctc_beam_lm_workspace_bytes(int T, int B, int C, int beam_width);
int ctcasr_ctc_beam_decode_lm(const float *logits, const int32_t *seq_len, int T, int B, int C,
                              int blank, int beam_width, int norm_mode, const int32_t *lm_next,
                              const float *lm_score, const float *lm_final, int lm_states,
                              int32_t *out, int32_t *out_len, float *logp, void *workspace,
                              size_t workspace_bytes, ctcasr_stream_t stream);

size_t ctcasr_ctc_beam_nbest_workspace_bytes(int T, int B, int C, int beam_width);
int ctcasr_ctc_beam_decode_nbest(const float *logits, const int32_t *seq_len, int T, int B, int C,
                                 int blank, int beam_width, int norm_mode, int top_paths,
                                 const int32_t *lm_next, const float *lm_score,
                                 const float *lm_final, int lm_states, int32_t *out,
                                 int32_t *out_len, float *logp, int32_t *n_paths, void *workspace,
                                 size_t workspace_bytes, ctcasr_stream_t stream);

size_t ctcasr_ctc_score_workspace_bytes(int T, int B, int C, int H, int max_label_len);
int ctcasr_ctc_score(const float *logits, const int32_t *seq_len, int T, int B, int C, int blank,
                     const int32_t *labels, const int32_t *label_offsets, const int32_t *utt,
                     int H, int max_label_len, float *score, int32_t *status, void *workspace,
                     size_t workspace_bytes, ctcasr_stream_t stream);

size_t ctcasr_ctc_mwer_workspace_bytes(int T, int B, int C, int N, int max_label_len);
int ctcasr_ctc_mwer(const float *logits, const int32_t *seq_len, int T, int B, int C, int blank,
                    const int32_t *labels, const int32_t *label_offsets, const int32_t *n_hyps,
                    const float *risk, int N, int max_label_len, float scale, int accumulate,
                    float *grad, float *expected_risk, float *score, float *posterior,
                    int32_t *status, void *workspace, size_t workspace_bytes,
                    ctcasr_stream_t stream);

size_t ctcasr_ctc_align_workspace_bytes(int T, int B, int C, int max_label_len);
int ctcasr_ctc_align(const float *logits, const int32_t *labels, const int32_t *label_offsets,
                     const int32_t *seq_len, int T, int B, int C, int blank, int max_label_len,
                     int32_t *path, float *score, float *frame_logp, int32_t *status,
                     void *workspace, size_t workspace_bytes, ctcasr_stream_t stream);

#define CTCASR_ALIGN_LONG_TILE_STATES 1024
#define CTCASR_ALIGN_LONG_TILE_FRAMES 256
size_t ctcasr_ctc_align_long_workspace_bytes(int64_t T, int C, int64_t L, int tile_frames);
int ctcasr_ctc_align_long(const float *logits, const int32_t *labels, int64_t T, int C, int blank,
                          int64_t L, int tile_frames, int32_t *path, double *score,
                          float *frame_logp, float *logp, int32_t *status, void *workspace,
                          size_t workspace_bytes, ctcasr_stream_t stream);

size_t ctcasr_ctc_search_workspace_bytes(int T, int B, int C);
int ctcasr_ctc_search(const float *logits, const int32_t *seq_len, int T, int B, int C, int blank,
                      const int32_t *labels, const int32_t *label_offsets, int P, int max_label_len,
                      const double *min_score, const int32_t *pair_utt, const int32_t *pair_phrase,
                      int H, int max_hits, int32_t *hits, double *hit_score, int32_t *n_hits,
                      double *best_score, int32_t *best_span, double *end_score,
                      int32_t *end_start, int32_t *status, void *workspace, size_t workspace_bytes,
                      ctcasr_stream_t stream);

size_t ctcasr_edit_distance_workspace_bytes(int B, int max_hyp_len, int max_ref_len);
int ctcasr_edit_distance(const int32_t *hyp, const int32_t *hyp_offsets, const int32_t *hyp_len,
                         const int32_t *ref, const int32_t *ref_offsets, const int32_t *ref_len,
                         int B, int max_hyp_len, int max_ref_len, int32_t *distance,
                         int32_t *substitutions, int32_t *deletions, int32_t *insertions,
                         int32_t *status, void *workspace, size_t workspace_bytes,
                         ctcasr_stream_t stream);

size_t ctcasr_rnn_gru_drec_offset(int T, int B, int H);
size_t ctcasr_rnn_reserve_bytes(int cell, int T, int B, int H);
size_t ctcasr_rnn_workspace_bytes(int cell, int T, int B, int H);
int ctcasr_rnn_fwd(int cell, const float *xw, const float *xw_bias, const float *w_hh,
                   const float *b_hh_n, const int32_t *seq_len, int T, int B, int H, float *y,
                   void *reserve, void *workspace, size_t workspace_bytes, ctcasr_stream_t stream);
#define CTCASR_RNN_DEFAULT 0
#define CTCASR_RNN_HALF_CHIP 1
#define CTCASR_RNN_WHOLE_CHIP 2
#define CTCASR_RNN_ONE_BARRIER 4
#define CTCASR_RNN_F16 16
#define CTCASR_RNN_XCD_SPLIT 32
#define CTCASR_RNN_STAGGER 64
#define CTCASR_RNN_KPAIR 128
#define CTCASR_RNN_TICKET(ticket) ((int)(((unsigned)(ticket) & 0xFFFFFFu) << 8))
int ctcasr_rnn_fwd_steps(int cell, const float *xw, const float *xw_bias, const float *w_hh,
                         const float *b_hh_n, const int32_t *seq_len, int T, int B, int H,
                         float *y, void *y_pieces, void *reserve, void *workspace,
                         size_t workspace_bytes, int step_begin, int step_end, int flags,
                         ctcasr_stream_t stream);
int ctcasr_rnn_fwd_f16_supported(int cell, int T, int B, int H, int flags);
int ctcasr_rnn_persistent_supported(int cell, int T, int B, int H);
int ctcasr_rnn_poll_error(void *workspace, size_t workspace_bytes, int cell, int T, int B,
                          int H, ctcasr_stream_t stream);
int ctcasr_rnn_resident_gate(void *workspace, size_t workspace_bytes, int cell, int T, int B,
                             int H, unsigned ticket, int max_wait_us, ctcasr_stream_t stream);
int ctcasr_rnn_bwd(int cell, const float *dy, const float *y, const float *w_hh_t,
                   const float *b_hh_n, const int32_t *seq_len, int T, int B, int H,
                   const void *reserve, float *dxw, float *dbias, void *workspace,
                   size_t workspace_bytes, ctcasr_stream_t stream);
int ctcasr_rnn_bwd_steps(int cell, const float *dy, const float *y, const float *w_hh_t,
                         const float *b_hh_n, const int32_t *seq_len, int T, int B, int H,
                         const void *reserve, float *dxw, float *dbias, uint32_t *colmax,
                         void *workspace, size_t workspace_bytes, int step_begin, int step_end,
                         int flags, ctcasr_stream_t stream);
int ctcasr_rnn_bwd_f16_supported(int cell, int T, int B, int H, int flags);
int ctcasr_rnn_f16_recurrence(int cell, int T, int B, int H, int flags, int backward, int ragged);

int ctcasr_bias_act_fwd(float *y, const float *bias, int64_t rows, int cols, float cutoff,
                        float dropout_rate, uint64_t seed, ctcasr_stream_t stream);
int ctcasr_bias_act_bwd(const float *y, const float *dy, float *dz, float *dbias, int64_t rows,
                        int cols, float cutoff, float dropout_rate, ctcasr_stream_t stream);
int ctcasr_dropout(const float *in, float *out, int64_t n, float dropout_rate, uint64_t seed,
                   ctcasr_stream_t stream);
int ctcasr_colsum_accumulate(const float *dz, float *dbias, int64_t rows, int cols,
                             ctcasr_stream_t stream);

int ctcasr_conv_s12_supported(int freq_in, int cout);
int ctcasr_conv_s12_pack_weights(const float *w, float *packed, int cout, ctcasr_stream_t stream);
size_t ctcasr_conv_s12_pack16_bytes(int cout);
int ctcasr_conv_s12_pack_weights16(const float *w, void *packed16, int cout,
                                   ctcasr_stream_t stream);
int ctcasr_conv_s12_fwd16(const float *x, float x_scale, const void *packed16, const float *bias,
                          float *y, int B, int T, int freq_in, int cout, float relu_cutoff,
                          int y_time_major, ctcasr_stream_t stream);
int ctcasr_conv_s12_bwd_data16(const float *dz, const void *packed16, float *dx, int B, int T,
                               int freq_in, int cout, int dz_time_major, const float *act,
                               float relu_cutoff, ctcasr_stream_t stream);
size_t ctcasr_conv_s12_wrw16_workspace_bytes(int B, int T, int freq_in, int cout);
int ctcasr_conv_s12_wrw16(const float *dz, const float *x, float x_scale, float *dw, int B, int T,
                          int freq_in, int cout, int dz_time_major, const float *act,
                          float relu_cutoff, float *dbias, void *workspace,
                          size_t workspace_bytes, ctcasr_stream_t stream);
int ctcasr_conv_s12_fwd(const float *x, const float *packed, const float *bias, float *y, int B,
                        int T, int freq_in, int cout, float relu_cutoff, int y_time_major,
                        ctcasr_stream_t stream);
int ctcasr_conv_s12_bwd_data(const float *dz, const float *packed, float *dx, int B, int T,
                             int freq_in, int cout, int dz_time_major, const float *act,
                             float relu_cutoff, ctcasr_stream_t stream);
size_t ctcasr_conv_s12_wrw_workspace_bytes(int B, int T, int freq_in, int cout);
int ctcasr_conv_s12_wrw(const float *dz, const float *x, float *dw, int B, int T, int freq_in,
                        int cout, int dz_time_major, const float *act, float relu_cutoff,
                        float *dbias, void *workspace, size_t workspace_bytes,
                        ctcasr_stream_t stream);

int ctcasr_conv0_fwd(const float *x, const float *w, const float *bias, float *y, int B, int T,
                     float relu_cutoff, ctcasr_stream_t stream);
size_t ctcasr_conv0_wrw_workspace_bytes(int B, int T);
int ctcasr_conv0_wrw(const float *dz, const float *x, float *dw, int B, int T, const float *act,
                     float relu_cutoff, float *dbias, void *workspace, size_t workspace_bytes,
                     ctcasr_stream_t stream);

size_t ctcasr_conv0_pack16_bytes(void);
int ctcasr_conv0_pack_weights16(const float *w, void *packed16, ctcasr_stream_t stream);
int ctcasr_conv0_fwd16(const float *x, const void *packed16, const float *bias, float *y, int B,
                       int T, float relu_cutoff, ctcasr_stream_t stream);
size_t ctcasr_conv0_wrw16_workspace_bytes(int B, int T);
int ctcasr_conv0_wrw16(const float *dz, const float *x, float *dw, int B, int T, const float *act,
                       float relu_cutoff, float *dbias, void *workspace, size_t workspace_bytes,
                       ctcasr_stream_t stream);

int ctcasr_transpose_batched(const float *in, float *out, int batch, int rows, int cols,
                             ctcasr_stream_t stream);

#define CTCASR_SPLIT_MAX_BLOCKS 6
int ctcasr_split_bf16(const float *x, int64_t rows, int cols, int64_t ld_x, const int *order,
                      int blocks, void *out, int64_t ld_out, int64_t block_stride,
                      ctcasr_stream_t stream);

int ctcasr_split_f16(const float *x, int64_t rows, int cols, int64_t ld_x, float scale,
                     const int *order, int blocks, void *out, int64_t ld_out,
                     int64_t block_stride, ctcasr_stream_t stream);

int ctcasr_colmax_scale(const float *x, int64_t rows, int cols, int64_t ld_x, void *workspace,
                        float *scale, float *inv_scale, ctcasr_stream_t stream);
int ctcasr_colscale_from_max(const uint32_t *max_bits, int cols, float *scale, float *inv_scale,
                             ctcasr_stream_t stream);
int ctcasr_split_f16_cols(const float *x, int64_t rows, int cols, int64_t ld_x,
                          const float *col_scale, float scale, const int *order, int blocks,
                          void *out, int64_t ld_out, int64_t block_stride, ctcasr_stream_t stream);
int ctcasr_split_f16_rows(const float *x, int64_t rows, int cols, int64_t ld_x, const int *order,
                          int blocks, void *out, int64_t ld_out, int64_t block_stride,
                          float *inv_scale, ctcasr_stream_t stream);
int ctcasr_rescale_rows(const float *t, int64_t ld_t, const float *row_factor, float alpha,
                        float *out, int64_t ld_out, int64_t rows, int cols, int accumulate,
                        ctcasr_stream_t stream);

int ctcasr_gemm_split_nt(const float *a, int64_t lda, const float *b, int64_t ldb, float *c,
                         int64_t ldc, int m, int n, int k, int accumulate, ctcasr_stream_t stream);
int ctcasr_gemm_split_tn(const float *a, int64_t lda, const float *b, int64_t ldb, float *c,
                         int64_t ldc, int m, int n, int k, int accumulate, ctcasr_stream_t stream);

size_t ctcasr_dgrad16_packed_bytes(int n);
int ctcasr_dgrad16_published_offsets(int T, int B, int hidden, size_t *exchange,
                                     size_t *inverse_scales);
int ctcasr_dgrad16_pack_weights(const float *w_ih, int64_t ld_w, int hidden, int n, float scale,
                                void *packed, ctcasr_stream_t stream);
int ctcasr_dgrad16_supported(int cell, int T, int B, int hidden);
int ctcasr_dgrad16_blockscaled(void *workspace, int T, int B, int hidden, const void *packed,
                               float scale, int n, float *dx, int64_t ld_dx, int t_lo, int t_hi,
                               int dir_lo, int dir_hi, int accumulate, ctcasr_stream_t stream);

size_t ctcasr_wgrad16_packed_bytes(int stages, int cols);
size_t ctcasr_wgrad16_sync_ints(int m, int nx, int ny);
int ctcasr_wgrad16_pack(const float *x, int64_t ld_x, int64_t rows_total, int cols, int64_t row0,
                        int stages, const float *col_scale, float scale, void *packed,
                        ctcasr_stream_t stream);
int ctcasr_wgrad16_gemm(const void *d_packed, int m, int stages, const float *inv_scale,
                        const void *x_packed, int x_stage0, int nx, float x_scale, float *dw_x,
                        int64_t ld_x, const void *y_packed, int y_stage0, int ny, float y_scale,
                        float *dw_y, int64_t ld_y, int parts, int32_t *sync, ctcasr_stream_t stream);

int ctcasr_adam_step(float *param, const float *grad, float *m, float *v, int64_t n, float lr,
                     float beta1, float beta2, float epsilon, int64_t step, float grad_scale,
                     const int32_t *skip, ctcasr_stream_t stream);
int ctcasr_step_guard(const int32_t *ctc_status, const float *per_utterance_loss, int batch,
                      const uint32_t *timeout_word0, const uint32_t *timeout_word1,
                      const int32_t *wgrad_word, int32_t *skip, ctcasr_stream_t stream);
int ctcasr_adam_step_clipped(float *param, const float *grad, float *m, float *v, int64_t n,
                             float lr, float beta1, float beta2, float epsilon, int64_t step,
                             float grad_scale, const int32_t *skip, const float *grad_factor,
                             ctcasr_stream_t stream);
int ctcasr_adam_step_ema(float *param, const float *grad, float *m, float *v, float *ema,
                         int64_t n, float lr, float beta1, float beta2, float epsilon,
                         int64_t step, float grad_scale, const int32_t *skip,
                         const float *grad_factor, float ema_alpha, ctcasr_stream_t stream);

#define CTCASR_GRAD_NORM_CHUNK 8192
#define CTCASR_GRAD_NORM_MAX_SEGMENTS 64
size_t ctcasr_grad_norm_workspace_bytes(int64_t n, int segments);
int ctcasr_grad_norm(const float *grad, int64_t n, const int64_t *seg_offsets, int segments,
                     float grad_scale, float max_norm, float *norms, float *clip_factor,
                     int32_t *skip, void *workspace, size_t workspace_bytes,
                     ctcasr_stream_t stream);
size_t ctcasr_rnn_timeout_word_offset(int cell, int T, int B, int H, int block);
int ctcasr_occupy_cus(int workgroups, int busy_us, ctcasr_stream_t stream);
int ctcasr_collective_traffic(int workgroups, int busy_us, float *a, const float *b,
                              int64_t scratch_floats, int64_t payload_bytes,
                              ctcasr_stream_t stream);
int ctcasr_absmax(const float *x, int64_t n, uint32_t *max_bits, ctcasr_stream_t stream);

int ctcasr_features_num_frames(int num_samples);
size_t ctcasr_features_tables_bytes(void);
int ctcasr_features_init_tables(void *tables, int sampling_rate, ctcasr_stream_t stream);
size_t ctcasr_features_workspace_bytes(int B, int max_samples);
int ctcasr_features(const int16_t *pcm, const int32_t *num_samples, int B, int max_samples,
                    int feature_type, int normalization, int drop_every_second_frame,
                    const void *tables, float *out, int out_frames, int32_t *out_len,
                    void *workspace, size_t workspace_bytes, ctcasr_stream_t stream);

#define CTCASR_SPEC_AUGMENT_MAX_MASKS 16
int ctcasr_spec_augment(float *features, const int32_t *lengths, int B, int out_frames,
                        uint64_t seed, int n_freq, int freq_width, int n_time, int time_width,
                        int time_permille, int32_t *intervals, ctcasr_stream_t stream);
int ctcasr_resample_num_samples(int num_samples, int percent);
int ctcasr_speed_perturb(const int16_t *pcm, const int32_t *num_samples, const int32_t *percent,
                         int B, int max_in, int16_t *out, int max_out, int32_t *out_samples,
                         ctcasr_stream_t stream);

#define CTCASR_NOISE_MIX_CHUNK 8192
#define CTCASR_NOISE_MIX_MIN_SNR_DB (-20)
#define CTCASR_NOISE_MIX_MAX_SNR_DB 60
size_t ctcasr_noise_mix_workspace_bytes(int B);
int ctcasr_noise_mix(const int16_t *pcm, const int32_t *num_samples, int B, int max_samples,
                     const int16_t *bank, const int64_t *clip_offsets, int num_clips,
                     uint64_t seed, int snr_lo_db, int snr_hi_db, int prob_permille,
                     int16_t *out, int32_t *draws, int64_t *powers, float *gain,
                     void *workspace, size_t workspace_bytes, ctcasr_stream_t stream);

#define CTCASR_REVERB_CHUNK 2048
#define CTCASR_REVERB_TAP_BLOCK 32
#define CTCASR_REVERB_TAP_ALIGN 8
#define CTCASR_REVERB_MAX_TAPS 8192
int ctcasr_reverb(const int16_t *pcm, const int32_t *num_samples, int B, int max_samples,
                  const int16_t *taps, const int64_t *rir_offsets, const int32_t *rir_delay,
                  const float *rir_scale, int num_rirs, uint64_t seed, int prob_permille,
                  int16_t *out, int32_t *draws, ctcasr_stream_t stream);

#define CTCASR_VAD_HOP 160
#define CTCASR_VAD_LEVELS 160
#define CTCASR_VAD_CHUNK 40960
int ctcasr_vad_energy(const int16_t *pcm, int64_t n, int64_t *energy, uint32_t *hist,
                      ctcasr_stream_t stream);
int ctcasr_gather_segments(const int16_t *pcm, int64_t n, const int64_t *seg_start,
                           const int32_t *seg_len, int B, int max_samples, int16_t *out,
                           int32_t *num_samples, ctcasr_stream_t stream);

#define CTCASR_RESAMPLE_MAX_TABLE 16640
#define CTCASR_PCM_S16 0
#define CTCASR_PCM_U8 1
#define CTCASR_PCM_S32 2
#define CTCASR_PCM_F32 3
int ctcasr_resample_plan(int rate_in, int rate_out, int *M, int *L, int *radius, int *taps);
int ctcasr_resample_chunk(int rate_in, int rate_out);
int64_t ctcasr_resample_out_samples(int64_t n, int rate_in, int rate_out);
size_t ctcasr_resample_table_bytes(int rate_in, int rate_out);
int ctcasr_resample_table(int rate_in, int rate_out, float *table, ctcasr_stream_t stream);
int ctcasr_resample(const void *in, int format, int channels, int64_t n, int rate_in, int rate_out,
                    const float *table, int16_t *out, int64_t n_out, int32_t *status,
                    ctcasr_stream_t stream);

#define CTCASR_SEQ_BN_ROWS 64
size_t ctcasr_seq_bn_workspace_bytes(int64_t rows, int C);
int ctcasr_seq_bn_fwd(const float *x, const int32_t *lengths, int T, int B, int C,
                      const float *gamma, const float *beta, float *running_mean,
                      float *running_var, double decay, double eps, float *y, float *mean,
                      float *rstd, void *workspace, size_t workspace_bytes,
                      ctcasr_stream_t stream);
int ctcasr_seq_bn_infer(const float *x, const int32_t *lengths, int T, int B, int C,
                        const float *gamma, const float *beta, const float *running_mean,
                        const float *running_var, double eps, float *y, ctcasr_stream_t stream);
int ctcasr_seq_bn_bwd(const float *dy, const float *x, const int32_t *lengths, int T, int B, int C,
                      const float *mean, const float *rstd, const float *gamma, float *dgamma,
// ... 8 lines not shown
```

Measured before the change: 6686.

## Pack conv weight-gradient inputs and run backward prologue early on side stream

Splits the conv weight-gradient entry points so the fp16 packing of the layer input x runs during the forward pass, on a side stream, into a retained workspace. The backward pass then waits on an event and reuses the packed buffer. The grad-zeroing and w_hh transposes also move into an early prologue on the side stream, overlapping the loss computation. The torch isfinite/where input poison check becomes a single custom kernel. In exchange, per-layer workspaces stay alive from forward to backward, which raises memory use and adds event synchronisation.

Measured after the change: 6762, median of 5. 1.1% higher.

```diff
diff --git a/ctc_asr_amd/csrc/conv16.hip b/ctc_asr_amd/csrc/conv16.hip
--- a/ctc_asr_amd/csrc/conv16.hip
+++ b/ctc_asr_amd/csrc/conv16.hip
@@ -723,12 +723,27 @@
     return wrw16_workspace(B, T, freq_in, cout).total;
 }
 
-extern "C" int ctcasr_conv_s12_wrw16(const float *dz, const float *x, float x_scale, float *dw,
-                                     int B, int T, int freq_in, int cout, int dz_time_major,
-                                     const float *act, float relu_cutoff, float *dbias,
-                                     void *workspace, size_t workspace_bytes,
-                                     ctcasr_stream_t stream) {
-    if (!dz || !x || !dw || B <= 0 || T <= 0 || (act && relu_cutoff <= 0.f) || !(x_scale > 0.f))
+extern "C" int ctcasr_conv_s12_wrw16_pack_x(const float *x, float x_scale, int B, int T,
+                                            int freq_in, int cout, void *workspace,
+                                            size_t workspace_bytes, ctcasr_stream_t stream) {
+    if (!x || B <= 0 || T <= 0 || !(x_scale > 0.f)) return CTCASR_ERR_BAD_ARGUMENT;
+    if (!covered16(freq_in, cout)) return CTCASR_ERR_UNSUPPORTED;
+    const Wrw16Workspace w = wrw16_workspace(B, T, freq_in, cout);
+    if (!workspace || workspace_bytes < w.total) return CTCASR_ERR_WORKSPACE;
+    u32x4 *x16 = reinterpret_cast<u32x4 *>(reinterpret_cast<char *>(workspace) + w.x16);
+    const int nblk = (B + 7) / 8;
+    const long per_utt = (long)T * freq_in * C16_CIN, xcells = (long)nblk * per_utt;
+    wrw16_pack_x_kernel<<<(unsigned)((xcells + 255) / 256), 256, 0, (hipStream_t)stream>>>(
+        x, x_scale, x16, B, per_utt, xcells);
+    return ctcasr_launch_status();
+}
+
+extern "C" int ctcasr_conv_s12_wrw16_packed(const float *dz, float x_scale, float *dw, int B, int T,
+                                            int freq_in, int cout, int dz_time_major,
+                                            const float *act, float relu_cutoff, float *dbias,
+                                            void *workspace, size_t workspace_bytes,
+                                            ctcasr_stream_t stream) {
+    if (!dz || !dw || B <= 0 || T <= 0 || (act && relu_cutoff <= 0.f) || !(x_scale > 0.f))
         return CTCASR_ERR_BAD_ARGUMENT;
     if (!covered16(freq_in, cout)) return CTCASR_ERR_UNSUPPORTED;
     const Wrw16Workspace w = wrw16_workspace(B, T, freq_in, cout);
@@ -736,16 +751,13 @@
     hipStream_t s = (hipStream_t)stream;
     char *base = reinterpret_cast<char *>(workspace);
     unsigned *max_bits = reinterpret_cast<unsigned *>(base + w.max_bits);
-    u32x4 *x16 = reinterpret_cast<u32x4 *>(base + w.x16);
+    const u32x4 *x16 = reinterpret_cast<const u32x4 *>(base + w.x16);
     u32x4 *dz16 = reinterpret_cast<u32x4 *>(base + w.dz16);
     float *partial = reinterpret_cast<float *>(base + w.partial);
     const int fo = freq_in / 2, nblk = (B + 7) / 8;
     if (hipMemsetAsync(max_bits, 0, 512, s) != hipSuccess) return CTCASR_ERR_LAUNCH;
     const long cells4 = (long)B * T * fo * cout / 4;
     wrw16_colmax_kernel<<<240, 256, 0, s>>>(dz, act, relu_cutoff, cells4, cout, max_bits, dbias);
-    const long per_utt = (long)T * freq_in * C16_CIN, xcells = (long)nblk * per_utt;
-    wrw16_pack_x_kernel<<<(unsigned)((xcells + 255) / 256), 256, 0, s>>>(x, x_scale, x16, B,
-                                                                        per_utt, xcells);
     const long dcells = (long)nblk * T * fo * cout;
     wrw16_pack_dz_kernel<<<(unsigned)((dcells + 255) / 256), 256, 0, s>>>(
         dz, act, relu_cutoff, max_bits, dz16, B, T, fo * cout, cout, dz_time_major, dcells);
@@ -770,6 +782,20 @@
     return ctcasr_launch_status();
 }
 
+extern "C" int ctcasr_conv_s12_wrw16(const float *dz, const float *x, float x_scale, float *dw,
+                                     int B, int T, int freq_in, int cout, int dz_time_major,
+                                     const float *act, float relu_cutoff, float *dbias,
+                                     void *workspace, size_t workspace_bytes,
+                                     ctcasr_stream_t stream) {
+    if (!dz || !x || !dw || B <= 0 || T <= 0 || (act && relu_cutoff <= 0.f) || !(x_scale > 0.f))
+        return CTCASR_ERR_BAD_ARGUMENT;
+    const int rc = ctcasr_conv_s12_wrw16_pack_x(x, x_scale, B, T, freq_in, cout, workspace,
+                                                workspace_bytes, stream);
+    if (rc != CTCASR_OK) return rc;
+    return ctcasr_conv_s12_wrw16_packed(dz, x_scale, dw, B, T, freq_in, cout, dz_time_major, act,
+                                        relu_cutoff, dbias, workspace, workspace_bytes, stream);
+}
+
 namespace {
 
 constexpr int Z0_KT = 11, Z0_KF = 41, Z0_FI = 80, Z0_FO = 40, Z0_TT = 16;
@@ -1118,30 +1144,44 @@
     return z0_workspace(B, T).total;
 }
 
-extern "C" int ctcasr_conv0_wrw16(const float *dz, const float *x, float *dw, int B, int T,
-                                  const float *act, float relu_cutoff, float *dbias,
-                                  void *workspace, size_t workspace_bytes,
-                                  ctcasr_stream_t stream) {
-    if (!dz || !x || !dw || B <= 0 || T <= 0 || (act && relu_cutoff <= 0.f))
+extern "C" int ctcasr_conv0_wrw16_pack_x(const float *x, int B, int T, void *workspace,
+                                         size_t workspace_bytes, ctcasr_stream_t stream) {
+    if (!x || B <= 0 || T <= 0) return CTCASR_ERR_BAD_ARGUMENT;
+    const Z0Workspace w = z0_workspace(B, T);
+    if (!workspace || workspace_bytes < w.total) return CTCASR_ERR_WORKSPACE;
+    hipStream_t s = (hipStream_t)stream;
+    char *base = reinterpret_cast<char *>(workspace);
+    unsigned *x_bits = reinterpret_cast<unsigned *>(base + 256);
+    u32x4 *x16 = reinterpret_cast<u32x4 *>(base + w.x16);
+    const int nblk = (B + 7) / 8;
+    if (hipMemsetAsync(base + 256, 0, 256, s) != hipSuccess) return CTCASR_ERR_LAUNCH;
+    const long n_x = (long)B * T * Z0_FI;
+    conv16_absmax_kernel<<<512, 256, 0, s>>>(x, (int)n_x, x_bits);
+    const long per_utt = (long)T * Z0_FI, xcells = (long)nblk * per_utt;
+    conv0_pack_x_kernel<<<(unsigned)((xcells + 255) / 256), 256, 0, s>>>(x, x_bits, x16, B, per_utt,
+                                                                        xcells);
+    return ctcasr_launch_status();
+}
+
+extern "C" int ctcasr_conv0_wrw16_packed(const float *dz, float *dw, int B, int T,
+                                         const float *act, float relu_cutoff, float *dbias,
+                                         void *workspace, size_t workspace_bytes,
+                                         ctcasr_stream_t stream) {
+    if (!dz || !dw || B <= 0 || T <= 0 || (act && relu_cutoff <= 0.f))
         return CTCASR_ERR_BAD_ARGUMENT;
     const Z0Workspace w = z0_workspace(B, T);
     if (!workspace || workspace_bytes < w.total) return CTCASR_ERR_WORKSPACE;
     hipStream_t s = (hipStream_t)stream;
     char *base = reinterpret_cast<char *>(workspace);
     unsigned *ch_bits = reinterpret_cast<unsigned *>(base);
-    unsigned *x_bits = reinterpret_cast<unsigned *>(base + 256);
-    u32x4 *x16 = reinterpret_cast<u32x4 *>(base + w.x16);
+    const unsigned *x_bits = reinterpret_cast<const unsigned *>(base + 256);
+    const u32x4 *x16 = reinterpret_cast<const u32x4 *>(base + w.x16);
     u32x4 *dz16 = reinterpret_cast<u32x4 *>(base + w.dz16);
     float *partial = reinterpret_cast<float *>(base + w.partial);
     const int t_out = (T + 1) / 2, nblk = (B + 7) / 8;
-    if (hipMemsetAsync(base, 0, 512, s) != hipSuccess) return CTCASR_ERR_LAUNCH;
+    if (hipMemsetAsync(base, 0, 256, s) != hipSuccess) return CTCASR_ERR_LAUNCH;
     const long cells4 = (long)B * t_out * Z0_FO * 32 / 4;
     wrw16_colmax_kernel<<<240, 256, 0, s>>>(dz, act, relu_cutoff, cells4, 32, ch_bits, dbias);
-    const long n_x = (long)B * T * Z0_FI;
-    conv16_absmax_kernel<<<512, 256, 0, s>>>(x, (int)n_x, x_bits);
-    const long per_utt = (long)T * Z0_FI, xcells = (long)nblk * per_utt;
-    conv0_pack_x_kernel<<<(unsigned)((xcells + 255) / 256), 256, 0, s>>>(x, x_bits, x16, B, per_utt,
-                                                                        xcells);
     const long dcells = (long)nblk * t_out * Z0_FO * 32;
     wrw16_pack_dz_kernel<<<(unsigned)((dcells + 255) / 256), 256, 0, s>>>(
         dz, act, relu_cutoff, ch_bits, dz16, B, t_out, Z0_FO * 32, 32, 0, dcells);
@@ -1155,3 +1195,15 @@
                                                                   w.parts);
     return ctcasr_launch_status();
 }
+
+extern "C" int ctcasr_conv0_wrw16(const float *dz, const float *x, float *dw, int B, int T,
+                                  const float *act, float relu_cutoff, float *dbias,
+                                  void *workspace, size_t workspace_bytes,
+                                  ctcasr_stream_t stream) {
+    if (!dz || !x || !dw || B <= 0 || T <= 0 || (act && relu_cutoff <= 0.f))
+        return CTCASR_ERR_BAD_ARGUMENT;
+    const int rc = ctcasr_conv0_wrw16_pack_x(x, B, T, workspace, workspace_bytes, stream);
+    if (rc != CTCASR_OK) return rc;
+    return ctcasr_conv0_wrw16_packed(dz, dw, B, T, act, relu_cutoff, dbias, workspace,
+                                     workspace_bytes, stream);
+}
diff --git a/ctc_asr_amd/csrc/elementwise.hip b/ctc_asr_amd/csrc/elementwise.hip
--- a/ctc_asr_amd/csrc/elementwise.hip
+++ b/ctc_asr_amd/csrc/elementwise.hip
@@ -90,6 +90,16 @@
 }
 
 __global__ void __launch_bounds__(256)
+input_poison_kernel(const float *__restrict__ x, int64_t per_utt, float *__restrict__ poison) {
+    const float *row = x + (int64_t)blockIdx.y * per_utt;
+    bool bad = false;
+    for (int64_t i = (int64_t)blockIdx.x * 256 + threadIdx.x; i < per_utt;
+         i += (int64_t)gridDim.x * 256)
+        bad |= !(fabsf(row[i]) <= 3.402823466e38f);
+    if (bad) poison[blockIdx.y] = __uint_as_float(0x7FC00000u);
+}
+
+__global__ void __launch_bounds__(256)
 transpose_kernel(const float *__restrict__ in, float *__restrict__ out, int rows, int cols) {
     __shared__ float tile[32][33];
     const size_t base = (size_t)blockIdx.z * rows * cols;
@@ -299,6 +309,21 @@
                       (hipStream_t)stream);
 }
 
+extern "C" int ctcasr_input_poison(const float *x, int B, int64_t per_utt, float *poison,
+                                   ctcasr_stream_t stream) {
+    if (!x || !poison || B < 0 || B > 65535 || per_utt < 0) return CTCASR_ERR_BAD_ARGUMENT;
+    if (B == 0) return CTCASR_OK;
+    hipStream_t s = (hipStream_t)stream;
+    if (hipMemsetAsync(poison, 0, sizeof(float) * (size_t)B, s) != hipSuccess)
+        return CTCASR_ERR_LAUNCH;
+    if (per_utt == 0) return CTCASR_OK;
+    int64_t chunks = (2048 + B - 1) / B;
+    const int64_t most = (per_utt + 4095) / 4096;
+    if (chunks > most) chunks = most;
+    input_poison_kernel<<<dim3((unsigned)chunks, (unsigned)B), 256, 0, s>>>(x, per_utt, poison);
+    return ctcasr_launch_status();
+}
+
 extern "C" int ctcasr_colsum_accumulate(const float *dz, float *dbias, int64_t rows, int cols,
                                         ctcasr_stream_t stream) {
     if (!dz || !dbias || rows < 0 || cols <= 0) return CTCASR_ERR_BAD_ARGUMENT;
diff --git a/ctc_asr_amd/hip.py b/ctc_asr_amd/hip.py
--- a/ctc_asr_amd/hip.py
+++ b/ctc_asr_amd/hip.py
@@ -118,6 +118,13 @@
     'ctcasr_conv_s12_wrw16_workspace_bytes': (_c_sz, [_c_int] * 4),
     'ctcasr_conv_s12_wrw16': (_c_int, [_c_p, _c_p, _c_f, _c_p] + [_c_int] * 5 +
                               [_c_p, _c_f, _c_p, _c_p, _c_sz, _c_p]),
+    'ctcasr_conv_s12_wrw16_pack_x': (_c_int, [_c_p, _c_f] + [_c_int] * 4 + [_c_p, _c_sz, _c_p]),
+    'ctcasr_conv_s12_wrw16_packed': (_c_int, [_c_p, _c_f, _c_p] + [_c_int] * 5 +
+                                     [_c_p, _c_f, _c_p, _c_p, _c_sz, _c_p]),
+    'ctcasr_conv0_wrw16_pack_x': (_c_int, [_c_p, _c_int, _c_int, _c_p, _c_sz, _c_p]),
+    'ctcasr_conv0_wrw16_packed': (_c_int, [_c_p, _c_p, _c_int, _c_int, _c_p, _c_f, _c_p, _c_p,
+                                            _c_sz, _c_p]),
+    'ctcasr_input_poison': (_c_int, [_c_p, _c_int, _c_i64, _c_p, _c_p]),
     'ctcasr_conv_s12_bwd_data': (_c_int, [_c_p, _c_p, _c_p] + [_c_int] * 5 + [_c_p, _c_f, _c_p]),
     'ctcasr_conv_s12_wrw_workspace_bytes': (_c_sz, [_c_int] * 4),
     'ctcasr_conv_s12_wrw': (_c_int, [_c_p] * 3 + [_c_int] * 5 + [_c_p, _c_f, _c_p] +
@@ -1452,9 +1459,36 @@
     return out
 
 
+def conv_s12_wrw16_workspace_bytes(batch, frames, freq_in, cout):
+    return load().ctcasr_conv_s12_wrw16_workspace_bytes(int(batch), int(frames), int(freq_in),
+                                                        int(cout))
+
+
+def conv0_wrw16_workspace_bytes(batch, frames):
+    return load().ctcasr_conv0_wrw16_workspace_bytes(int(batch), int(frames))
+
+
+@_on_tensor_device
+def conv_s12_wrw16_pack_x(x, x_scale, cout, workspace=None):
+    batch, frames, freq, cin = _conv_dims('conv_s12_wrw16_pack_x', 'x', x, 4)
+    if cin != 32 or not load().ctcasr_conv_s12_wrw16_workspace_bytes(batch, frames, freq,
+                                                                       int(cout)):
+        raise CtcAsrError('conv_s12_wrw16_pack_x: unsupported layer shape {} / cout {}'.format(
+            tuple(x.shape), cout))
+    x_scale = _conv_scale('conv_s12_wrw16_pack_x', x_scale)
+    need = load().ctcasr_conv_s12_wrw16_workspace_bytes(batch, frames, freq, int(cout))
+    if workspace is None or workspace.numel() < need:
+        workspace = _workspace(need, x.device)
+    _check(load().ctcasr_conv_s12_wrw16_pack_x(_dev(x, name='x'), x_scale, batch, frames, freq,
+                                               int(cout), _dev(workspace, torch.uint8, 'workspace'),
+                                               workspace.numel(), _stream()),
+           'conv_s12_wrw16_pack_x')
+    return workspace
+
+
 @_on_tensor_device
 def conv_s12_wrw16(dz, x, x_scale, out=None, time_major=False, act=None, relu_cutoff=0.0,
-                   dbias=None):
+                   dbias=None, packed=None):
     batch, frames, freq_out, cout = _conv_s12_dz('conv_s12_wrw16', dz, time_major)
     if tuple(x.shape) != (batch, frames, 2 * freq_out, 32):
         raise CtcAsrError('conv_s12_wrw16: unsupported layer shape {} / {}'.format(
@@ -1464,9 +1498,19 @@
     _expect_numel('conv_s12_wrw16', 'out', out, cout * 32 * 11 * 21)
     out = torch.empty((cout, 32, 11, 21), dtype=torch.float32, device=x.device) if out is None \
         else out
-    workspace = _workspace(load().ctcasr_conv_s12_wrw16_workspace_bytes(batch, frames,
-                                                                        2 * freq_out, cout),
-                           x.device)
+    need = load().ctcasr_conv_s12_wrw16_workspace_bytes(batch, frames, 2 * freq_out, cout)
+    if packed is not None:
+        if packed.numel() < need:
+            raise CtcAsrError('conv_s12_wrw16: packed holds {} bytes, {} needed.'.format(
+                packed.numel(), need))
+        with _Timed('conv_s12_wrw'):
+            _check(load().ctcasr_conv_s12_wrw16_packed(
+                _dev(dz, name='dz'), x_scale, _dev(out, name='dw'), batch, frames, 2 * freq_out,
+                cout, 1 if time_major else 0, _dev(act, name='act'), float(relu_cutoff),
+                _dev(dbias, name='dbias'), _dev(packed, torch.uint8, 'packed'), packed.numel(),
+                _stream()), 'conv_s12_wrw16')
+        return out
+    workspace = _workspace(need, x.device)
     with _Timed('conv_s12_wrw'):
         _check(load().ctcasr_conv_s12_wrw16(_dev(dz, name='dz'), _dev(x, name='x'),
                                             x_scale, _dev(out, name='dw'), batch, frames,
@@ -1530,7 +1574,19 @@
 
 
 @_on_tensor_device
-def conv0_wrw16(dz, x, out=None, act=None, relu_cutoff=0.0, dbias=None):
+def conv0_wrw16_pack_x(x, workspace=None):
+    batch, frames = _conv0_x('conv0_wrw16_pack_x', x)
+    need = load().ctcasr_conv0_wrw16_workspace_bytes(batch, frames)
+    if workspace is None or workspace.numel() < need:
+        workspace = _workspace(need, x.device)
+    _check(load().ctcasr_conv0_wrw16_pack_x(_dev(x, name='x'), batch, frames,
+                                            _dev(workspace, torch.uint8, 'workspace'),
+                                            workspace.numel(), _stream()), 'conv0_wrw16_pack_x')
+    return workspace
+
+
+@_on_tensor_device
+def conv0_wrw16(dz, x, out=None, act=None, relu_cutoff=0.0, dbias=None, packed=None):
     batch, frames = _conv0_x('conv0_wrw16', x)
     if tuple(dz.shape) != (batch, (frames + 1) // 2, 40, 32):
         raise CtcAsrError('conv0_wrw16 covers x [B,T,80], dz [B,ceil(T/2),40,32] only.')
@@ -1538,7 +1594,18 @@
     _expect_numel('conv0_wrw16', 'out', out, 32 * 11 * 41)
     out = torch.empty((32, 1, 11, 41), dtype=torch.float32, device=x.device) if out is None \
         else out
-    workspace = _workspace(load().ctcasr_conv0_wrw16_workspace_bytes(batch, frames), x.device)
+    need = load().ctcasr_conv0_wrw16_workspace_bytes(batch, frames)
+    if packed is not None:
+        if packed.numel() < need:
+            raise CtcAsrError('conv0_wrw16: packed holds {} bytes, {} needed.'.format(
+                packed.numel(), need))
+        with _Timed('conv0_wrw'):
+            _check(load().ctcasr_conv0_wrw16_packed(
+                _dev(dz, name='dz'), _dev(out, name='dw'), batch, frames, _dev(act, name='act'),
+                float(relu_cutoff), _dev(dbias, name='dbias'),
+                _dev(packed, torch.uint8, 'packed'), packed.numel(), _stream()), 'conv0_wrw16')
+        return out
+    workspace = _workspace(need, x.device)
     with _Timed('conv0_wrw'):
         _check(load().ctcasr_conv0_wrw16(_dev(dz, name='dz'), _dev(x, name='x'),
                                          _dev(out, name='dw'), batch, frames,
@@ -1546,6 +1613,19 @@
                                          _dev(dbias, name='dbias'),
                                          _dev(workspace, torch.uint8, 'workspace'),
                                          workspace.numel(), _stream()), 'conv0_wrw16')
+    return out
+
+
+@_on_tensor_device
+def input_poison(x, out=None):
+    batch = x.shape[0]
+    _expect_numel('input_poison', 'out', out, batch)
+    out = torch.empty(batch, dtype=torch.float32, device=x.device) if out is None else out
+    if x.numel() == 0:
+        return out.zero_()
+    if batch:
+        _check(load().ctcasr_input_poison(_dev(x, name='x'), batch, x.numel() // batch,
+                                          _dev(out, name='poison'), _stream()), 'input_poison')
     return out
 
 
diff --git a/ctc_asr_amd/model.py b/ctc_asr_amd/model.py
--- a/ctc_asr_amd/model.py
+++ b/ctc_asr_amd/model.py
@@ -390,6 +390,7 @@
         self._w_split, self._w_split_ready, self._w_split_bufs = {}, None, {}
         self._w_guard = None
         self._side_stream = None
+        self._wrw_ws = {}
         self.early_hooks = False
         self.rnn_bwd_flags = int(os.environ.get('CTCASR_RNN_BWD_FLAGS', str(hip.RNN_DEFAULT)))
         self.gpu_metrics = os.environ.get('CTCASR_GPU_METRICS', '1') == '1'
@@ -569,6 +570,42 @@
             self._w_split_ready = torch.cuda.Event()
             self._w_split_ready.record(side)
 
+    def _side(self):
+        if self._side_stream is None:
+            self._side_stream = torch.cuda.Stream(self.device)
+        return self._side_stream
+
+    def _pack_wrw_early(self, acts, layer, pack, nbytes):
+        if not self.overlap_wgrad:
+            return
+        ws = self._wrw_ws.get(layer)
+        if ws is None or ws.numel() < nbytes:
+            ws = self._wrw_ws[layer] = torch.empty(nbytes, dtype=torch.uint8, device=self.device)
+        main, side = torch.cuda.current_stream(self.device), self._side()
+        ready = torch.cuda.Event()
+        ready.record(main)
+        with torch.cuda.stream(side):
+            side.wait_event(ready)
+            pack(ws)
+            packed = torch.cuda.Event()
+            packed.record(side)
+        acts.setdefault('wrw_packed', {})[layer] = (ws, packed)
+
+    def _backward_prologue_early(self, ready, accumulate):
+        acts = self._acts
+        if acts is None or ready is None:
+            return
+        side = self._side()
+        with torch.cuda.stream(side):
+            side.wait_event(ready)
+            if not accumulate:
+                self.arena.grad.zero_()
+            for i in range(self.cfg.num_layers_rnn):
+                hip.transpose_batched(self.arena.p['rnn{}/w_hh'.format(i)], out=self._w_hh_t[i])
+            done = torch.cuda.Event()
+            done.record(side)
+        acts['bwd_prologue'] = (done, bool(accumulate))
+
     def _weight_split(self, name, backward=False, acts=None):
         pieces, ready = (self._w_split, self._w_split_ready) if acts is None else \
             (acts['w_split'], acts['w_split_ready'])
@@ -599,8 +636,7 @@
         sequences = sequences.to(self.device, torch.float32).contiguous()
         batch, frames, _ = sequences.shape
         acts = {'training': training, 'batch': batch, 'conv_f16': {}}
-        acts['input_poison'] = torch.where(
-            torch.isfinite(sequences).view(batch, -1).all(dim=1), 0.0, float('nan')).to(torch.float32)
+        acts['input_poison'] = hip.input_poison(sequences)
         self._prepare_weight_splits(cfg.output_time(frames) * batch, training, batch)
         if cfg.used_model == 'ds2':
             x = sequences.unsqueeze(1).contiguous(memory_format=torch.channels_last)
@@ -629,6 +665,9 @@
                         'fp16x3' if self.conv_f16 else 'fp32'
                     conv_in.append(None)
                     acts['features'] = sequences
+                    if training and self.conv_f16 and self.conv_wrw_f16:
+                        self._pack_wrw_early(acts, 0, lambda ws: hip.conv0_wrw16_pack_x(
+                            sequences, ws), hip.conv0_wrw16_workspace_bytes(batch, frames))
                 elif own_kind[i] == 's12':
                     kernel = p['conv{}/kernel'.format(i)]
                     last_time_major = fused and i == layers - 1
@@ -637,6 +676,12 @@
                     if x_scale is not None:
                         self._conv_packed16[i] = hip.conv_s12_pack_weights16(
                             kernel, self._conv_packed16.get(i))
+                        if training and self.conv_wrw_f16:
+                            self._pack_wrw_early(
+                                acts, i, lambda ws, x=x, x_scale=x_scale, cout=kernel.shape[0]:
+                                hip.conv_s12_wrw16_pack_x(x.permute(0, 2, 3, 1), x_scale, cout, ws),
+                                hip.conv_s12_wrw16_workspace_bytes(
+                                    batch, x.shape[2], x.shape[3], kernel.shape[0]))
                         y = hip.conv_s12_fwd16(x.permute(0, 2, 3, 1), x_scale,
                                                self._conv_packed16[i], kernel.shape[0],
                                                p['conv{}/bias'.format(i)], relu_cutoff=cutoff,
@@ -1117,7 +1162,13 @@
             if reduce_hook is not None:
                 reduce_hook(layer, *slices[layer])
 
-        if not accumulate:
+        prologue = acts.pop('bwd_prologue', None)
+        if prologue is not None:
+            if prologue[1] != bool(accumulate):
+                raise RuntimeError('backward(accumulate={}) behind a prologue for accumulate={}.'
+                                   .format(bool(accumulate), prologue[1]))
+            torch.cuda.current_stream(self.device).wait_event(prologue[0])
+        elif not accumulate:
             self.arena.grad.zero_()
 
         def write(view, fn):
@@ -1164,8 +1215,9 @@
             for tensor in tensors:
                 tensor.record_stream(side)
 
-        for i in range(cfg.num_layers_rnn):
-            hip.transpose_batched(p['rnn{}/w_hh'.format(i)], out=self._w_hh_t[i])
+        if prologue is None:
+            for i in range(cfg.num_layers_rnn):
+                hip.transpose_batched(p['rnn{}/w_hh'.format(i)], out=self._w_hh_t[i])
 
         write(g['logits/kernel'], lambda out: torch.mm(acts['dense4'].t(), dlogits, out=out))
         hip.colsum_accumulate(dlogits, g['logits/bias'])
@@ -1514,6 +1566,10 @@
                 if own == 'conv0':
                     wrw0 = hip.conv0_wrw16 if (self.conv_f16 and self.conv_wrw_f16) \
                         else hip.conv0_wrw
+                    early = acts.get('wrw_packed', {}).get(i) if wrw0 is hip.conv0_wrw16 else None
+                    if early is not None:
+                        main.wait_event(early[1])
+                        mask = dict(mask, packed=early[0])
                     write(g[name + '/kernel'], lambda out: wrw0(
                         dz.permute(0, 2, 3, 1), acts['features'], out=out,
                         dbias=g[name + '/bias'] if fused_bwd else None, **mask))
@@ -1523,10 +1579,15 @@
                 if own == 's12':
                     dz_phys = dz if tm else dz.permute(0, 2, 3, 1)
                     if acts['conv_f16'].get(i) and self.conv_wrw_f16:
+                        early = acts.get('wrw_packed', {}).get(i)
+                        packed = None
+                        if early is not None:
+                            main.wait_event(early[1])
+                            packed = early[0]
                         write(g[name + '/kernel'], lambda out: hip.conv_s12_wrw16(
                             dz_phys, conv_in.permute(0, 2, 3, 1), acts['conv_f16'][i], out=out,
                             time_major=tm, dbias=g[name + '/bias'] if fused_bwd else None,
-                            **mask))
+                            packed=packed, **mask))
                     else:
                         write(g[name + '/kernel'], lambda out: hip.conv_s12_wrw(
                             dz_phys, conv_in.permute(0, 2, 3, 1), out=out, time_major=tm,
@@ -1571,7 +1632,12 @@
 
     def forward_backward(self, features, feature_len, labels, reduce_hook=None, check=True,
                          accumulate=False, mwer=None, originals=None):
+        ready = None
+        if self.overlap_wgrad:
+            ready = torch.cuda.Event()
+            ready.record(torch.cuda.current_stream(self.device))
         logits, seq_length = self.inference_fn(features, feature_len, training=True)
+        self._backward_prologue_early(ready, accumulate)
         if mwer:
             loss = self.mwer_loss_fn(logits, seq_length, labels, originals=originals,
                                      check=check, **mwer)
diff --git a/include/ctcasr.h b/include/ctcasr.h
--- a/include/ctcasr.h
+++ b/include/ctcasr.h
@@ -179,6 +179,13 @@
                           int freq_in, int cout, int dz_time_major, const float *act,
                           float relu_cutoff, float *dbias, void *workspace,
                           size_t workspace_bytes, ctcasr_stream_t stream);
+int ctcasr_conv_s12_wrw16_pack_x(const float *x, float x_scale, int B, int T, int freq_in,
+                                 int cout, void *workspace, size_t workspace_bytes,
+                                 ctcasr_stream_t stream);
+int ctcasr_conv_s12_wrw16_packed(const float *dz, float x_scale, float *dw, int B, int T,
+                                 int freq_in, int cout, int dz_time_major, const float *act,
+                                 float relu_cutoff, float *dbias, void *workspace,
+                                 size_t workspace_bytes, ctcasr_stream_t stream);
 int ctcasr_conv_s12_fwd(const float *x, const float *packed, const float *bias, float *y, int B,
                         int T, int freq_in, int cout, float relu_cutoff, int y_time_major,
                         ctcasr_stream_t stream);
@@ -206,6 +213,14 @@
 int ctcasr_conv0_wrw16(const float *dz, const float *x, float *dw, int B, int T, const float *act,
                        float relu_cutoff, float *dbias, void *workspace, size_t workspace_bytes,
                        ctcasr_stream_t stream);
+int ctcasr_conv0_wrw16_pack_x(const float *x, int B, int T, void *workspace,
+                              size_t workspace_bytes, ctcasr_stream_t stream);
+int ctcasr_conv0_wrw16_packed(const float *dz, float *dw, int B, int T, const float *act,
+                              float relu_cutoff, float *dbias, void *workspace,
+                              size_t workspace_bytes, ctcasr_stream_t stream);
+
+int ctcasr_input_poison(const float *x, int B, int64_t per_utt, float *poison,
+                        ctcasr_stream_t stream);
 
 int ctcasr_transpose_batched(const float *in, float *out, int batch, int rows, int cols,
                              ctcasr_stream_t stream);
```
